# Shreyas911/MITgcm

Measured on AMD Instinct MI355X. Metric: model-days/wallclock-sec, higher is better.
Workload: dtype f64; 1 GPU; BASELINE config 2, verification/global_ocean.90x40x15 as verified: 90x40x15 global lat-lon ocean, 1 tile of 90x40 (OL=3) on 1 GPU, restarted from the committed pickup at nIter0=36000; r* coordinate with non-linear free surface (UPDATE_CG2D every step), JMD95P, GM/Redi gkw91, CD scheme, biharmonic + harmonic viscosity, quasi-hydrostatic + NH metric + 3-D Coriolis, implicit vertical diffusion, IVDC,; tiles_per_gpu=1, parallelism=replicas1, cg2d=single-GPU kernel

## Files before the change

mitgcm_amd/csrc/common.h:

```cpp
#pragma once
#include <hip/hip_runtime.h>
#include <stdint.h>
#include <stdlib.h>

namespace mgcm {

struct Dims {
  int sNx, sNy, OLx, OLy, Nr, nSx, nSy, nTiles;
  int t0, nT;
  int nx, ny;
  long n2, n3;
  long N2all, N3all;
};

#define MG_F2D_LIST(X) X(dxF) X(dyF) X(dxG) X(dyG) X(dxC) X(dyC) X(dxV) X(dyU) X(rA) X(rAw) X(rAs) X(recip_dxF) \
    X(recip_dyF) X(recip_dxC) X(recip_dyC) X(recip_dxV) X(recip_dyU) X(recip_rA) X(recip_rAw) X(recip_rAs) \
    X(fCori) X(Bo_surf) X(recip_Bo) X(tanPhiAtU) X(tanPhiAtV) X(maskInC) X(SST) X(lambdaThetaClimRelax) X(aW2d) \
    X(aS2d) X(aC2d) X(pW) X(pS) X(pC) X(etaN) X(fu) X(fv) X(etaH) X(surfaceForcingT) X(surfaceForcingS) \
    X(cg2d_b) X(cg2d_x) X(Qnet) X(EmPmR) X(SSS) X(lambdaSaltClimRelax) X(etaNm1) X(fCoriCos) X(recip_Rcol) \
    X(rSurfW) X(rSurfS) X(rLowW) X(rLowS) X(Ro_surf) X(R_low) X(rStarFacC) X(rStarFacW) X(rStarFacS) \
    X(rStarExpC) X(rStarExpW) X(rStarExpS) X(rStarDhCDt) X(rStarDhWDt) X(rStarDhSDt) X(PmEpR) X(dEtaHdt) \
    X(maskInW) X(maskInS) X(fCoriG) X(recip_rAz) X(recip_dxG) X(recip_dyG) X(etaHnm1) X(cg2d_r) X(cg2d_s) X(cg2d_q) \
    X(cg2d_min) X(cg2d_y) X(cg2d_v) X(EmPmRnext)
#define MG_F3D_LIST(X) X(hFacC) X(hFacW) X(hFacS) X(recip_hFacC) X(recip_hFacW) X(recip_hFacS) X(maskC) X(maskW) \
    X(maskS) X(uVel) X(vVel) X(wVel) X(theta) X(salt) X(gU) X(gV) X(guNm1) X(gvNm1) X(rhoInSitu) X(IVDConvCount) \
    X(gtNm1) X(thetaNext) X(gTscr) X(cpScr) X(phiHydC) X(saltNext) X(gsNm1) X(advScr1) X(advScr2) X(gAdv) \
    X(sigmaR) X(Kwx) X(Kwy) X(Kwz) X(Kux) X(Kvy) X(uVelD) X(vVelD) X(uNM1) X(vNM1) X(cdU) X(cdV) X(h0FacC) \
    X(h0FacW) X(h0FacS) X(totPhiHyd) X(alphaRho) X(del2u) X(del2v) X(dWtC) X(dWtU) X(dWtV) X(Kuz) X(Kvz) \
    X(GM_PsiX) X(GM_PsiY) X(gtNm2) X(gsNm2)
#define MG_ENUM2(n) F2_##n,
#define MG_ENUM3(n) F3_##n,
enum F2Id { MG_F2D_LIST(MG_ENUM2) F2_COUNT };
enum F3Id { MG_F3D_LIST(MG_ENUM3) F3_COUNT };
#undef MG_ENUM2
#undef MG_ENUM3

struct Params {
  double deltaTMom, deltaTFreeSurf, deltaTClock, abEps, rhoConst, gBaro;
  double viscAhD, viscAhZ, viscA4D, viscA4Z, viscAr, sideDragFactor;
  double freeSurfFac, implicSurfPress, implicDiv2DFlow, rkSign;
  double afFacMom, vfFacMom, pfFacMom, cfFacMom, foFacMom, mtFacMom;
  double cg2dNorm, cg2dTolerance_sq;
  int momAdvection, momViscosity, momForcing, useCoriolis, no_slip_sides, no_slip_bottom;
  int selectCoriScheme, momForcingOutAB, momDissip_In_AB, implicitViscosity;
  int cg2dMaxIters, cg2dUseMinResSol, cg2dNormaliseRHS, nIter0;
  int cg2dUseFMA;
  int useSRCGSolver;
  int cg2dRefOrder;
  double gravity, gravitySign, rhoNil, tAlpha, sBeta, ivdc_kappa, diffKhT, diffKrT, deltaTtracer;
  double recip_rSphere;
  int exactConserv, tempStepping, tempAdvection, tempForcing, implicitDiffusion, tempAdvScheme;
  int metricSphere;
  double diffKhS, diffKrS;
  int saltStepping, saltAdvection, saltForcing, saltAdvScheme, multiDimAdvection, momStepping;
  int multiDimCompressible;
  int eosType;
  int allowFreezing, useRealFreshWaterFlux, useCDscheme, useGMRedi, periodicExternalForcing, nForcRec;
  double HeatCapacity_Cp, convertFW2Salt, temp_EvPrRn, salt_EvPrRn, rCD, epsAB_CD;
  double externForcingPeriod, externForcingCycle;
  double GM_background_K, GM_isopycK, GM_skewflx, GM_maxSlope, GM_Kmin_horiz, GM_Small_Number, GM_slopeSqCutoff;
  int GM_AdvForm, GM_ExtraDiag;
  int nonlinFreeSurf, select_rStar, quasiHydrostatic, useNHMTerms, select3dCoriScheme, selectP_inEOS_Zc;
  int storePhiHyd4Phys;
  double hFacInf;
  int vectorInvariantMomentum, selectVortScheme, selectKEscheme, upwindShear, cubeCorners;
  int staggerTimeStep, tracForcingOutAB;
  double alph_AB, beta_AB;
  int useAB3;
};

struct Fields {
  const double *drF, *drC, *recip_drF, *recip_drC, *rF, *rC, *tRef, *sRef;
  const double *dxF, *dyF, *dxG, *dyG, *dxC, *dyC, *dxV, *dyU, *rA, *rAw, *rAs;
  const double *recip_dxF, *recip_dyF, *recip_dxC, *recip_dyC, *recip_dxV, *recip_dyU;
  const double *recip_rA, *recip_rAw, *recip_rAs, *fCori, *Bo_surf, *recip_Bo;
  const double *tanPhiAtU, *tanPhiAtV, *maskInC, *lambdaThetaClimRelax;
  double *SST;
  double *hFacC, *hFacW, *hFacS, *recip_hFacC, *recip_hFacW, *recip_hFacS;
  const double *maskC, *maskW, *maskS;
  double *aW2d, *aS2d, *aC2d, *pW, *pS, *pC;
  double *uVel, *vVel, *wVel, *theta, *salt, *etaN;
  double *gU, *gV, *guNm1, *gvNm1;
  double *fu, *fv;
  double *etaH, *surfaceForcingT, *rhoInSitu, *IVDConvCount, *gtNm1;
  double *thetaNext, *gTscr, *cpScr;
  double *phiHydC;
  double *saltNext, *gsNm1, *surfaceForcingS;
  double *gtNm2, *gsNm2;
  double *advScr1, *advScr2, *gAdv;
  const double *pRef4EOS;
  const double *forcRec;
  double *Qnet, *EmPmR, *SSS, *lambdaSaltClimRelax, *etaNm1;
  double *sigmaR, *Kwx, *Kwy, *Kwz, *Kux, *Kvy;
  double *Kuz, *Kvz, *GM_PsiX, *GM_PsiY;
  double *uVelD, *vVelD, *uNM1, *vNM1, *cdU, *cdV;
  const double *h0FacC, *h0FacW, *h0FacS;
  const double *fCoriCos, *recip_Rcol, *rSurfW, *rSurfS, *rLowW, *rLowS, *Ro_surf, *R_low;
  const double *phiRefC;
  double *totPhiHyd, *alphaRho, *del2u, *del2v;
  double *rStarFacC, *rStarFacW, *rStarFacS, *rStarExpC, *rStarExpW, *rStarExpS;
  double *rStarDhCDt, *rStarDhWDt, *rStarDhSDt, *PmEpR, *dEtaHdt;
  double *etaHnm1;
  const double *maskInW, *maskInS;
  double *dWtC, *dWtU, *dWtV;
  const double *fCoriG, *recip_rAz, *recip_dxG, *recip_dyG;
  const int *tileFace, *tileEdge;
  double *cg2d_b, *cg2d_x;
  double *cg2d_r, *cg2d_s, *cg2d_q;
  double *cg2d_min;
  double *cg2d_y, *cg2d_v;
  double *EmPmRnext;
  double *a2, *a3;
};
typedef __attribute__((address_space(1))) double mg_gdouble;
#define AR2(x, q) ((mg_gdouble *)f.a2)[(long)F2_##x * d.N2all + (q)]
#define AR3(x, q) ((mg_gdouble *)f.a3)[(long)F3_##x * d.N3all + (q)]

#define MG_I2(d, i, j, t) \
  ((long)((i) + (d).OLx - 1) + (long)((j) + (d).OLy - 1) * (d).nx + (long)(t) * (d).n2)
#define MG_I3(d, i, j, k, t)                                                                \
  ((long)((i) + (d).OLx - 1) + (long)((j) + (d).OLy - 1) * (d).nx + (long)((k) - 1) * (d).n2 + \
   (long)(t) * (d).n3)

#define MG_NXCD 8
__device__ __forceinline__ int mg_xcd_block() {
  const int b = (int)blockIdx.x, n = (int)gridDim.x;
  const int x = b % MG_NXCD, per = n / MG_NXCD, rem = n % MG_NXCD;
  return x * per + (x < rem ? x : rem) + b / MG_NXCD;
}
#define MG_PLANE(i0, ni, j0, nj, zvar)                                                  \
  int i, j, zvar;                                                                       \
  {                                                                                     \
    const int np_ = (ni) * (nj), nb_ = (np_ + (int)blockDim.x - 1) / (int)blockDim.x; \
    const int lb_ = mg_xcd_block();                                                     \
    const int q_ = (lb_ % nb_) * (int)blockDim.x + (int)threadIdx.x;                    \
    zvar = lb_ / nb_;                                                                   \
    if (q_ >= np_) return;                                                              \
    i = (i0) + q_ % (ni);                                                               \
    j = (j0) + q_ / (ni);                                                               \
  }
#define MG_PLANE_LB(i0, ni, j0, nj, zvar, LB)                                           \
  int i, j, zvar;                                                                       \
  {                                                                                     \
    const int np_ = (ni) * (nj), nb_ = (np_ + (int)blockDim.x - 1) / (int)blockDim.x; \
    const int lb_ = (LB);                                                               \
    const int q_ = (lb_ % nb_) * (int)blockDim.x + (int)threadIdx.x;                    \
    zvar = lb_ / nb_;                                                                   \
    if (q_ >= np_) return;                                                              \
    i = (i0) + q_ % (ni);                                                               \
    j = (j0) + q_ / (ni);                                                               \
  }
#define MG_PLANE_THREADS 256

__host__ __device__ inline int mg_col_kp(int Nr) { int kp = 1; while (kp < Nr) kp <<= 1; return kp; }
#define MG_COLS(i0, ni, j0, nj, Nr)                                                    \
  const int KP_ = mg_col_kp(Nr), NC_ = 256 / KP_;                                        \
  const int cc = (int)threadIdx.x % NC_, kk = (int)threadIdx.x / NC_;                   \
  const long col_ = (long)mg_xcd_block() * NC_ + cc;                                    \
  const long npl_ = (long)(ni) * (nj);                                                  \
  const bool valid = col_ < npl_ * d.nT;                                                \
  const int t = d.t0 + (int)(valid ? col_ / npl_ : 0);                                  \
  const int i = (i0) + (int)((valid ? col_ % npl_ : 0) % (ni));                         \
  const int j = (j0) + (int)((valid ? col_ % npl_ : 0) / (ni));
inline unsigned mg_col_blocks(int ni, int nj, int nT, int Nr) {
  const int nc = 256 / mg_col_kp(Nr);
  return (unsigned)(((long)ni * nj * nT + nc - 1) / nc);
}
#define MG_COLF(i0, ni, j0, nj, NCv)                                                   \
  const int NC_ = (NCv), KW_ = 256 / NC_;                                              \
  const int cc = (int)threadIdx.x % NC_, kk = (int)threadIdx.x / NC_;                  \
  const long col_ = (long)mg_xcd_block() * NC_ + cc;                                   \
  const long npl_ = (long)(ni) * (nj);                                                 \
  const bool valid = col_ < npl_ * d.nT;                                               \
  const int t = d.t0 + (int)(valid ? col_ / npl_ : 0);                                 \
  const int i = (i0) + (int)((valid ? col_ % npl_ : 0) % (ni));                        \
  const int j = (j0) + (int)((valid ? col_ % npl_ : 0) / (ni));
#define MG_COLF_LB(i0, ni, j0, nj, NCv, LB)                                            \
  const int NC_ = (NCv), KW_ = 256 / NC_;                                              \
  const int cc = (int)threadIdx.x % NC_, kk = (int)threadIdx.x / NC_;                  \
  const long col_ = (long)(LB) * NC_ + cc;                                             \
  const long npl_ = (long)(ni) * (nj);                                                 \
  const bool valid = col_ < npl_ * d.nT;                                               \
  const int t = d.t0 + (int)(valid ? col_ / npl_ : 0);                                 \
  const int i = (i0) + (int)((valid ? col_ % npl_ : 0) % (ni));                        \
  const int j = (j0) + (int)((valid ? col_ % npl_ : 0) / (ni));
#define MG_COLF_K(kvar) for (int kvar = kk + 1; kvar <= d.Nr; kvar += KW_)
inline int mg_colf_nc(long ncols, int Nr, int nArr) {
  (void)ncols; (void)Nr; (void)nArr;
  return 16;
}
inline size_t mg_colf_lds(int Nr, int nc, int nArr) { return (size_t)nArr * Nr * nc * sizeof(double); }
#define MG_ALLOW_LDS(kern)                                                                              \
  do {                                                                                                  \
    static const bool set_ = (hipFuncSetAttribute((const void *)(kern),                                 \
                                                  hipFuncAttributeMaxDynamicSharedMemorySize, 160 * 1024) == hipSuccess); \
    (void)set_;                                                                                         \
  } while (0)
inline unsigned mg_colf_blocks(long ncols, int nc) { return (unsigned)((ncols + nc - 1) / nc); }
enum { MG_FUSE_SFP = 1, MG_FUSE_ETA = 2, MG_FUSE_PHI = 4, MG_FUSE_END = 8, MG_FUSE_PHYS = 16, MG_FUSE_ETAA = 32,
       MG_FUSE_TREX = 64, MG_FUSE_DT = 128, MG_FUSE_ETAX = 256, MG_FUSE_TCG = 512, MG_FUSE_OPE = 1024,
       MG_FUSE_RING = 2048, MG_FUSE_RINGP = 4096, MG_FUSE_ENDS = 8192, MG_FUSE_PIPE = 16384 };
inline bool mg_fuse_on(int bit) {
  const int mask = getenv("MGCM_STEP_FUSE") ? atoi(getenv("MGCM_STEP_FUSE"))
                                            : MG_FUSE_SFP | MG_FUSE_PHI | MG_FUSE_END | MG_FUSE_DT | MG_FUSE_ETAX |
                                                MG_FUSE_OPE | MG_FUSE_RING | MG_FUSE_RINGP | MG_FUSE_ENDS | MG_FUSE_PIPE;
  return (mask & bit) != 0;
}
inline bool mg_hfuse(int bit, long nx, long ny, long nT, long Nr) {
  return mg_fuse_on(bit) && nx * ny * nT * Nr <= (1L << 21);
}
inline unsigned mg_plane_blocks(int ni, int nj, int nz) {
  return (unsigned)(((ni) * (nj) + MG_PLANE_THREADS - 1) / MG_PLANE_THREADS * (nz));
}

__device__ __forceinline__ void sfp_rhs_column(const Dims &d, const Params &p, const Fields &f, long q, bool inner,
                                               const double *sE, const double *sW, const double *sN, const double *sS,
                                               int NC_, int cc) {
  if (p.useCDscheme) f.etaNm1[q] = f.etaN[q];
  f.cg2d_x[q] = f.Bo_surf[q] * f.etaN[q];
  double b = 0.0;
  if (inner) {
    if (p.useRealFreshWaterFlux) {
      const double tmpFac = p.freeSurfFac * (1.0 / p.rhoConst) * p.implicDiv2DFlow;
      b = tmpFac * f.rA[q] * f.EmPmR[q] / p.deltaTMom * f.maskInC[q];
    }
    for (int k2 = d.Nr; k2 >= 1; k2--) {
      const int s2 = (k2 - 1) * NC_ + cc;
      b = b + sE[s2] - sW[s2];
      b = b + sN[s2] - sS[s2];
    }
    b = b - p.freeSurfFac * f.rA[q] / p.deltaTMom / p.deltaTFreeSurf * (p.exactConserv ? f.etaH[q] : f.etaN[q]);
  }
  f.cg2d_b[q] = b;
}

struct TracerArgs {
  const double *tr;
  double *trNext;
  double *gNm1;
  double *scr;
  double *cp;
  const double *sfc;
  double diffKh, diffKr, dT;
  int advection, multiDim, useAB, forcing;
  int limiter;
  int scheme;
  double *gNm2;
};

#define MG_XMAX 8
struct XFields {
  double *p[MG_XMAX];
  int nz[MG_XMAX];
  int n;
};

__device__ __forceinline__ void exchange_multi_body(const Dims &d, const XFields &x, const long *__restrict__ map,
                                                    int nHalo, int *ctr, int hb, int k, int fi) {
  const int h = hb * (int)blockDim.x + (int)threadIdx.x;
  if (ctr && h == 0 && k == 0 && fi == 0) { ctr[0] += 1; ctr[1] += 1; }
  if (h >= nHalo || fi >= x.n || k >= x.nz[fi]) return;
  const long dst = map[2 * h], src = map[2 * h + 1];
  const long dt = dst / d.n2, dl = dst % d.n2, st = src / d.n2, sl = src % d.n2;
  const long lvl = (long)d.n2 * x.nz[fi];
  double *a = x.p[fi];
  a[dt * lvl + (long)k * d.n2 + dl] = a[st * lvl + (long)k * d.n2 + sl];
}

__device__ __forceinline__ void exchange_mixed_body(const Dims &d, double *u, double *v, int nzUV,
                                                    const long *__restrict__ uvMap, int nU, int nV, const XFields &x,
                                                    const long *__restrict__ map, int nHalo, int *ctr, int hb, int k,
                                                    int z) {
  const int h = hb * (int)blockDim.x + (int)threadIdx.x;
  if (ctr && h == 0 && k == 0 && z == 0) { ctr[0] += 1; ctr[1] += 1; }
  if (z == 0) {
    if (h >= nU + nV || k >= nzUV) return;
    const long dst = uvMap[2 * h], code = uvMap[2 * h + 1];
    const long N2 = d.n2 * d.nTiles, s = (code > 0 ? code : -code) - 1;
    const long n3 = d.n2 * nzUV, lvl = (long)k * d.n2;
    auto at = [&](long g) -> long { return (g / d.n2) * n3 + lvl + g % d.n2; };
    const double val = s < N2 ? u[at(s)] : v[at(s - N2)];
    (h < nU ? u : v)[at(dst)] = code > 0 ? val : -val;
    return;
  }
  const int fi = z - 1;
  if (h >= nHalo || fi >= x.n || k >= x.nz[fi]) return;
  const long dst = map[2 * h], src = map[2 * h + 1];
  const long dt = dst / d.n2, dl = dst % d.n2, st = src / d.n2, sl = src % d.n2;
  const long lvl = (long)d.n2 * x.nz[fi];
  double *a = x.p[fi];
  a[dt * lvl + (long)k * d.n2 + dl] = a[st * lvl + (long)k * d.n2 + sl];
}

struct MwgTables {
  const int *ownG;
  const int *ownC;
  const unsigned *ownNb;
  const unsigned *ownExp;
  const int *ringG;
  const unsigned *ringNb;
  const int *impC;
  const int *impG;
  const int *nImp;
  int G, IMAX, SZ;
  int nExp;
  int pinned;
  int sys;
  int partsPerTile;
  int exclusive;
  unsigned *ctr;
  unsigned *epoch;
  unsigned long long *part;
  unsigned long long *xs;
  size_t hsBytes;
  int ref;
  int nTiles;
  const int *ownN;
  unsigned long long *refc;
};

struct MonSpec {
  const double *arr, *hfac, *mask, *area, *dr;
  int nz, arr3d, hf3d;
};
constexpr int MON_NF = 6, MON_NV = 6;
struct MonSpecs {
  MonSpec s[MON_NF];
  double mean[MON_NF];
};

struct SolveRecord {
  double firstResidual, lastResidual, minResidualSq, rhsMax, sumRHS;
  int numIters, nIterMin;
};

}
```

mitgcm_amd/csrc/kernels_dyn.hip:

```cpp
#include <cstdlib>

#include "common.h"
#include "phys.h"
#include <cstring>
#include <cstdio>
#include <type_traits>

namespace mgcm {

__device__ __forceinline__ double hfacz(const Dims &d, const Fields &f, int i, int j, int k, int t) {
  if (i < 2 - d.OLx || j < 2 - d.OLy) return 0.0;
  double h = fmin(f.hFacW[MG_I3(d, i, j, k, t)], f.hFacW[MG_I3(d, i, j - 1, k, t)]);
  h = fmin(f.hFacS[MG_I3(d, i, j, k, t)], h);
  h = fmin(f.hFacS[MG_I3(d, i - 1, j, k, t)], h);
  return h;
}

__device__ __forceinline__ double h0facz(const Dims &d, const Params &p, const Fields &f, int i, int j, int k, int t) {
  if (!(p.momViscosity && p.no_slip_sides && p.nonlinFreeSurf > 0)) return hfacz(d, f, i, j, k, t);
  if (i < 2 - d.OLx || j < 2 - d.OLy) return 0.0;
  return fmin(fmin(f.h0FacW[MG_I3(d, i, j, k, t)], f.h0FacW[MG_I3(d, i, j - 1, k, t)]),
              fmin(f.h0FacS[MG_I3(d, i, j, k, t)], f.h0FacS[MG_I3(d, i - 1, j, k, t)]));
}

__device__ __forceinline__ void del2uv_body(const Dims &d, const Params &p, const Fields &f, int lb) {
  MG_PLANE_LB(1 - d.OLx, d.nx, 1 - d.OLy, d.ny, z, lb)
  const int t = d.t0 + z / d.Nr, k = z % d.Nr + 1;
  const long q3 = MG_I3(d, i, j, k, t);
  if (i < 2 - d.OLx || i > d.sNx + d.OLx - 1 || j < 2 - d.OLy || j > d.sNy + d.OLy - 1) {
    f.del2u[q3] = 0.0;
    f.del2v[q3] = 0.0;
    return;
  }
  const double drF = f.drF[k - 1];
#define U(ii, jj) f.uVel[MG_I3(d, ii, jj, k, t)]
#define V(ii, jj) f.vVel[MG_I3(d, ii, jj, k, t)]
#define G2(a, ii, jj) f.a[MG_I2(d, ii, jj, t)]
#define G3(a, ii, jj) f.a[MG_I3(d, ii, jj, k, t)]
  {
    auto fz = [&](int ii) { return drF * G3(hFacC, ii, j) * G2(dyF, ii, j) * G2(recip_dxF, ii, j) * (U(ii + 1, j) - U(ii, j)) * 1.0; };
    auto fm = [&](int jj) {
      return drF * hfacz(d, f, i, jj, k, t) * G2(dxV, i, jj) * G2(recip_dyU, i, jj) * (U(i, jj) - U(i, jj - 1));
    };
    double v4 = f.recip_drF[k - 1] * G3(recip_hFacW, i, j) * G2(recip_rAw, i, j) *
                (fz(i) - fz(i - 1) + fm(j + 1) - fm(j)) * G3(maskW, i, j);
    if (p.no_slip_sides) {
      const double hS = G3(h0FacW, i, j) - h0facz(d, p, f, i, j, k, t);
      const double hN = G3(h0FacW, i, j) - h0facz(d, p, f, i, j + 1, k, t);
      v4 = v4 - G3(recip_hFacW, i, j) * G2(recip_rAw, i, j) *
                    (hS * G2(dxV, i, j) * G2(recip_dyU, i, j) + hN * G2(dxV, i, j + 1) * G2(recip_dyU, i, j + 1)) * U(i, j) *
                    p.sideDragFactor * G3(maskW, i, j);
    }
    f.del2u[q3] = v4;
  }
  {
    auto fz = [&](int ii) {
      return drF * hfacz(d, f, ii, j, k, t) * G2(dyU, ii, j) * G2(recip_dxV, ii, j) * (V(ii, j) - V(ii - 1, j)) * 1.0;
    };
    auto fm = [&](int jj) { return drF * G3(hFacC, i, jj) * G2(dxF, i, jj) * G2(recip_dyF, i, jj) * (V(i, jj + 1) - V(i, jj)); };
    double v4 = f.recip_drF[k - 1] * G3(recip_hFacS, i, j) * G2(recip_rAs, i, j) *
                (fz(i + 1) - fz(i) + fm(j) - fm(j - 1)) * G3(maskS, i, j);
    if (p.no_slip_sides) {
      const double hW = G3(h0FacS, i, j) - h0facz(d, p, f, i, j, k, t);
      const double hE = G3(h0FacS, i, j) - h0facz(d, p, f, i + 1, j, k, t);
      v4 = v4 - G3(recip_hFacS, i, j) * G2(recip_rAs, i, j) *
                    (hW * G2(dyU, i, j) * G2(recip_dxV, i, j) + hE * G2(dyU, i + 1, j) * G2(recip_dxV, i + 1, j)) * V(i, j) *
                    p.sideDragFactor * G3(maskS, i, j);
    }
    f.del2v[q3] = v4;
  }
#undef U
#undef V
#undef G2
#undef G3
}
__global__ void __launch_bounds__(256) k_del2uv(Dims d, Params p, Fields f) { del2uv_body(d, p, f, mg_xcd_block()); }

template <bool PHYS = false>
__device__ __forceinline__ void phi_hyd_body(const Dims &d, const Params &p, const Fields &f, int nc, int lb,
                                             const int *iterPtr = nullptr) {
  extern __shared__ __attribute__((aligned(16))) double lds[];
  MG_COLF_LB(PHYS ? 1 - d.OLx : -1, PHYS ? d.nx : d.sNx + 3, PHYS ? 1 - d.OLy : -1, PHYS ? d.ny : d.sNy + 3, nc, lb)
  const int Nr = d.Nr, NS = Nr * NC_;
  double *sM = lds, *sP = lds + NS, *sPh = lds + 2 * NS, *sC = lds + 3 * NS, *sU = lds + 4 * NS, *sV = lds + 5 * NS;
  const bool qh = p.quasiHydrostatic && (p.select3dCoriScheme >= 1 || p.useNHMTerms);
  const bool rstar = p.nonlinFreeSurf > 0 && p.select_rStar > 0;
  const bool inPhi = !PHYS || (i >= -1 && i <= d.sNx + 1 && j >= -1 && j <= d.sNy + 1);
  const bool ring = inPhi && i >= 0 && j >= 0;
  const double recip_rhoConst = 1.0 / p.rhoConst;
  const long q2 = MG_I2(d, i, j, t);
  if (valid) MG_COLF_K(k) {
    const int me = (k - 1) * NC_ + cc;
    double dRlocM = 0.5 * f.drC[k - 1];
    if (k == 1) dRlocM = f.rF[0] - f.rC[0];
    const double dRlocP = (k == Nr) ? (f.rC[k - 1] - f.rF[k]) : 0.5 * f.drC[k];
    const long q3 = MG_I3(d, i, j, k, t);
    double a;
    if constexpr (PHYS) a = oceanic_phys_point(d, p, f, iterPtr, i, j, k, t);
    else a = f.rhoInSitu[q3];
    if (qh) {
      const double scalingFactor = p.rhoConst * p.gravitySign * (1.0 / p.gravity);
      const double u0 = f.uVel[q3], u1 = f.uVel[MG_I3(d, i + 1, j, k, t)];
      const double v0 = f.vVel[q3], v1 = f.vVel[MG_I3(d, i, j + 1, k, t)];
      double gW = 0.0;
      if (p.select3dCoriScheme >= 1) gW = f.fCoriCos[q2] * (1.0 * 0.5 * (u0 + u1) - 0.0 * 0.5 * (v0 + v1));
      if (p.useNHMTerms) gW = gW + ((u0 * u0 + u1 * u1) + (v0 * v0 + v1 * v1)) * 0.5 * p.recip_rSphere;
      a = a + scalingFactor * gW;
    }
    if (rstar && inPhi) f.alphaRho[q3] = a;
    sM[me] = dRlocM * p.gravity * a * recip_rhoConst;
    sP[me] = dRlocP * p.gravity * a * recip_rhoConst;
    if (rstar) {
      const double drF = f.drF[k - 1];
      sC[me] = f.rStarDhCDt[q2] * drF * f.h0FacC[q3] * f.rA[q2];
      if (ring) {
        sU[me] = f.rStarDhWDt[q2] * drF * f.h0FacW[q3] * f.rAw[q2];
        sV[me] = f.rStarDhSDt[q2] * drF * f.h0FacS[q3] * f.rAs[q2];
      }
    }
  }
  __syncthreads();
  if (valid && kk == 0) {
    double phF = 0.0;
    for (int k2 = 1; k2 <= Nr; k2++) {
      const int s2 = (k2 - 1) * NC_ + cc;
      const double phC = phF + sM[s2];
      phF = phC + sP[s2];
      sPh[s2] = phC;
    }
    if (rstar) {
      auto d0 = [&](long r) { return f.rStarDhCDt[r] * (f.Ro_surf[r] - f.R_low[r]) * f.rA[r]; };
      double c = d0(q2);
      double u = ring ? 0.5 * (d0(q2 - 1) + c) : 0.0, v = ring ? 0.5 * (d0(q2 - d.nx) + c) : 0.0;
      for (int k2 = 1; k2 <= Nr; k2++) {
        const int s2 = (k2 - 1) * NC_ + cc;
        const double cc2 = sC[s2];
        sC[s2] = c;
        c = c - cc2;
        if (ring) {
          const double uu = sU[s2], vv = sV[s2];
          sU[s2] = u;
          sV[s2] = v;
          u = u - uu;
          v = v - vv;
        }
      }
    }
  }
  __syncthreads();
  if (valid) MG_COLF_K(k) {
    const int me = (k - 1) * NC_ + cc;
    const long q3 = MG_I3(d, i, j, k, t);
    if (rstar && inPhi) {
      f.dWtC[q3] = sC[me];
      if (ring) { f.dWtU[q3] = sU[me]; f.dWtV[q3] = sV[me]; }
    }
    if (ring) {
      const double phC = sPh[me];
      f.phiHydC[q3] = phC;
      if (p.storePhiHyd4Phys) {
        double tot;
        if (rstar && p.nonlinFreeSurf >= 4) {
          const double dPhiRef = (f.Ro_surf[q2] - f.rC[k - 1]) * p.gravity;
          tot = phC * f.rStarFacC[q2] + fmax(dPhiRef, 0.0) * (f.rStarFacC[q2] - 1.0) + 0.0;
        } else {
          tot = phC + f.Bo_surf[q2] * f.etaN[q2] + 0.0;
        }
        f.totPhiHyd[q3] = tot;
      }
    }
  }
}
__global__ void __launch_bounds__(256) k_phi_hyd(Dims d, Params p, Fields f, int nc) {
  phi_hyd_body(d, p, f, nc, mg_xcd_block());
}
constexpr int PHI_CH = 10;
template <bool RS, bool QH, int NRC = 0>
__device__ __forceinline__ void phi_flat_body(const Dims &d, const Params &p, const Fields &f, int lb) {
  constexpr int o = RS ? 1 : 0;
  const int W = d.sNx + 2 + o, H = d.sNy + 2 + o;
  const long col = (long)lb * 256 + threadIdx.x, npl = (long)W * H;
  if (col >= npl * d.nT) return;
  const int t = d.t0 + (int)(col / npl), r = (int)(col % npl);
  const int i = r % W - o, j = r / W - o;
  const bool ring = i >= 0 && j >= 0;
  const int Nr = NRC > 0 ? NRC : d.Nr;
  constexpr int CH = (RS || QH) ? 5 : PHI_CH;
  const double recip_rhoConst = 1.0 / p.rhoConst;
  const double scalingFactor = p.rhoConst * p.gravitySign * (1.0 / p.gravity);
  const long q2 = MG_I2(d, i, j, t);
  double c = 0.0, u = 0.0, v = 0.0, dCdt = 0.0, dWdt = 0.0, dSdt = 0.0, rA = 0.0, rAw = 0.0, rAs = 0.0;
  if (RS) {
    auto d0 = [&](long rr) { return f.rStarDhCDt[rr] * (f.Ro_surf[rr] - f.R_low[rr]) * f.rA[rr]; };
    c = d0(q2);
    u = ring ? 0.5 * (d0(q2 - 1) + c) : 0.0;
    v = ring ? 0.5 * (d0(q2 - d.nx) + c) : 0.0;
    dCdt = f.rStarDhCDt[q2]; rA = f.rA[q2];
    if (ring) { dWdt = f.rStarDhWDt[q2]; dSdt = f.rStarDhSDt[q2]; rAw = f.rAw[q2]; rAs = f.rAs[q2]; }
  }
  const bool tot = p.storePhiHyd4Phys && ring;
  const bool totR = RS && p.nonlinFreeSurf >= 4;
  const double bEta = tot && !totR ? f.Bo_surf[q2] * f.etaN[q2] : 0.0;
  const double fac = tot && totR ? f.rStarFacC[q2] : 0.0, roS = tot && totR ? f.Ro_surf[q2] : 0.0;
  const double fCos = QH ? f.fCoriCos[q2] : 0.0;
  double phF = 0.0;
  auto chunk = [&](const int k0) {
    double a[CH], u0[CH], u1[CH], v0[CH], v1[CH], hC[CH], hW[CH], hS[CH], dM[CH], dP[CH];
#pragma unroll
    for (int cc = 0; cc < CH; cc++) {
      const int k = k0 + cc <= Nr ? k0 + cc : Nr;
      const long q3 = MG_I3(d, i, j, k, t);
      a[cc] = f.rhoInSitu[q3];
      if constexpr (NRC > 0) {
        dM[cc] = (k == 1) ? f.rF[0] - f.rC[0] : 0.5 * f.drC[k - 1];
        dP[cc] = (k == Nr) ? (f.rC[k - 1] - f.rF[k]) : 0.5 * f.drC[k];
      }
      if (QH) {
        u0[cc] = f.uVel[q3]; u1[cc] = f.uVel[MG_I3(d, i + 1, j, k, t)];
        v0[cc] = f.vVel[q3]; v1[cc] = f.vVel[MG_I3(d, i, j + 1, k, t)];
      }
      if (RS) {
        hC[cc] = f.h0FacC[q3];
        if (ring) { hW[cc] = f.h0FacW[q3]; hS[cc] = f.h0FacS[q3]; }
      }
    }
#pragma unroll
    for (int cc = 0; cc < CH; cc++) {
      const int k = k0 + cc;
      if (k > Nr) continue;
      const long q3 = MG_I3(d, i, j, k, t);
      double dRlocM, dRlocP;
      if constexpr (NRC > 0) {
        dRlocM = dM[cc];
        dRlocP = dP[cc];
      } else {
        dRlocM = 0.5 * f.drC[k - 1];
        if (k == 1) dRlocM = f.rF[0] - f.rC[0];
        dRlocP = (k == Nr) ? (f.rC[k - 1] - f.rF[k]) : 0.5 * f.drC[k];
      }
      double al = a[cc];
      if (QH) {
        double gW = 0.0;
        if (p.select3dCoriScheme >= 1) gW = fCos * (1.0 * 0.5 * (u0[cc] + u1[cc]) - 0.0 * 0.5 * (v0[cc] + v1[cc]));
        if (p.useNHMTerms)
          gW = gW + ((u0[cc] * u0[cc] + u1[cc] * u1[cc]) + (v0[cc] * v0[cc] + v1[cc] * v1[cc])) * 0.5 * p.recip_rSphere;
        al = al + scalingFactor * gW;
      }
      if (RS) f.alphaRho[q3] = al;
      const double sM = dRlocM * p.gravity * al * recip_rhoConst;
      const double sP = dRlocP * p.gravity * al * recip_rhoConst;
      const double phC = phF + sM;
      phF = phC + sP;
      if (RS) {
        const double drF = f.drF[k - 1];
        const double cc2 = dCdt * drF * hC[cc] * rA;
        f.dWtC[q3] = c;
        c = c - cc2;
        if (ring) {
          const double uu = dWdt * drF * hW[cc] * rAw, vv = dSdt * drF * hS[cc] * rAs;
          f.dWtU[q3] = u;
          f.dWtV[q3] = v;
          u = u - uu;
          v = v - vv;
        }
      }
      if (ring) {
        f.phiHydC[q3] = phC;
        if (tot) {
          if (totR) {
            const double dPhiRef = (roS - f.rC[k - 1]) * p.gravity;
            f.totPhiHyd[q3] = phC * fac + fmax(dPhiRef, 0.0) * (fac - 1.0) + 0.0;
          } else {
            f.totPhiHyd[q3] = phC + bEta + 0.0;
          }
        }
      }
    }
  };
  if constexpr (NRC > 0) {
#pragma unroll
    for (int k0 = 1; k0 <= NRC; k0 += CH) chunk(k0);
  } else {
    for (int k0 = 1; k0 <= Nr; k0 += CH) chunk(k0);
  }
}
template <bool RS, bool QH, int NRC = 0>
__global__ void __launch_bounds__(256) k_phi_flat(Dims d, Params p, Fields f) {
  phi_flat_body<RS, QH, NRC>(d, p, f, mg_xcd_block());
}

inline bool phi_flat_on(const Params &p) {
  const char *e = getenv("MGCM_PHI_FLAT");
  const int v = e ? atoi(e) : 1;
  if (v == 0 || v == 2) return v == 2;
  const bool rs = p.nonlinFreeSurf > 0 && p.select_rStar > 0;
  const bool qh = p.quasiHydrostatic && (p.select3dCoriScheme >= 1 || p.useNHMTerms);
  return !rs && !qh;
}
inline int phi_flat_blocks(const Dims &d, const Params &p) {
  const int o = (p.nonlinFreeSurf > 0 && p.select_rStar > 0) ? 1 : 0;
  return (int)(((long)(d.sNx + 2 + o) * (d.sNy + 2 + o) * d.nT + 255) / 256);
}
__global__ void __launch_bounds__(256) k_phys_phi(Dims d, Params p, Fields f, int nc, const int *iterPtr) {
  phi_hyd_body<true>(d, p, f, nc, mg_xcd_block(), iterPtr);
}
__global__ void __launch_bounds__(256) k_phi_del2(Dims d, Params p, Fields f, int nc, int nbPhi) {
  const int lb = mg_xcd_block();
  if (lb < nbPhi) phi_hyd_body(d, p, f, nc, lb);
  else del2uv_body(d, p, f, lb - nbPhi);
}


template <class A> __device__ __forceinline__ int vi_tile_face(const A &, const Fields &f, int t) { return f.tileFace[t]; }
template <class A> __device__ __forceinline__ int vi_tile_edge(const A &, const Fields &f, int t) { return f.tileEdge[t]; }
template <class A> __device__ __forceinline__ double vi_rdrC(const A &, const Fields &f, int kk) { return f.recip_drC[kk - 1]; }
template <class A> __device__ __forceinline__ double vi_rdrF(const A &, const Fields &f, int kk) { return f.recip_drF[kk - 1]; }
template <class A> __device__ __forceinline__ double vi_drF(const A &, const Fields &f, int kk) { return f.drF[kk - 1]; }
// ... 2028 lines not shown
```

mitgcm_amd/csrc/kernels_rstar.hip:

```cpp
#include "common.h"
#include "phys.h"
#include "ucg2d.h"

namespace mgcm {

__device__ __forceinline__ double eta_exch(const Dims &d, const Fields &f, const long *srcOf, long q, int fromX) {
  const long sq = srcOf[q];
  if (sq >= 0) return f.cg2d_b[sq];
  const long l = q % d.n2;
  const int i = (int)(l % d.nx) - d.OLx + 1, j = (int)(l / d.nx) - d.OLy + 1;
  if (i >= 1 && i <= d.sNx && j >= 1 && j <= d.sNy) return f.cg2d_b[q];
  return fromX ? f.recip_Bo[q] * f.cg2d_x[q] : f.etaN[q];
}

template <bool FUSE>
__device__ __forceinline__ void calc_r_star_body(const Dims &d, const Params &p, const Fields &f,
                                                 const long *__restrict__ srcOf, int lb, int fromX, int empNext = 0) {
  const long q = (long)lb * blockDim.x + threadIdx.x;
  if (q >= d.n2 * d.nTiles) return;
  const int t = (int)(q / d.n2);
  if (t < d.t0 || t >= d.t0 + d.nT) return;
  if constexpr (FUSE) {
    if (p.nonlinFreeSurf > 0 && p.useRealFreshWaterFlux) f.PmEpR[q] = -f.EmPmR[q];
    if (empNext) f.EmPmR[q] = f.EmPmRnext[q];
    const double x = eta_exch(d, f, srcOf, q, fromX);
    f.etaHnm1[q] = f.etaH[q];
    f.etaN[q] = x;
    f.etaH[q] = x;
  }
  const long sq = srcOf[q], r = sq >= 0 ? sq : q;
  const long l = r % d.n2;
  const int i = (int)(l % d.nx) - d.OLx + 1, j = (int)(l / d.nx) - d.OLy + 1;
  auto eta = [&](long qq) { return FUSE ? eta_exch(d, f, srcOf, qq, fromX) : f.etaH[qq]; };
  const double oc = f.rStarFacC[q], ow = f.rStarFacW[q], os = f.rStarFacS[q];
  double fc = oc, fw = ow, fs = os;
  if (i >= 0 && i <= d.sNx + 1 && j >= 0 && j <= d.sNy + 1)
    fc = (f.maskInC[r] != 0.0) ? (eta(r) + f.Ro_surf[r] - f.R_low[r]) * f.recip_Rcol[r] : 1.0;
  const long rv = p.cubeCorners ? q : r;
  const long lv = rv % d.n2;
  const int iv = (int)(lv % d.nx) - d.OLx + 1, jv = (int)(lv / d.nx) - d.OLy + 1;
  if (iv >= 1 && iv <= d.sNx + 1 && jv >= 1 && jv <= d.sNy) {
    if (f.maskInW[rv] != 0.0) {
      const double tmp = f.rSurfW[rv] - f.rLowW[rv];
      fw = (0.5 * (eta(rv - 1) * f.rA[rv - 1] + eta(rv) * f.rA[rv]) * f.recip_rAw[rv] + tmp) / tmp;
    } else {
      fw = 1.0;
    }
  }
  if (iv >= 1 && iv <= d.sNx && jv >= 1 && jv <= d.sNy + 1) {
    if (f.maskInS[rv] != 0.0) {
      const double tmp = f.rSurfS[rv] - f.rLowS[rv];
      fs = (0.5 * (eta(rv - d.nx) * f.rA[rv - d.nx] + eta(rv) * f.rA[rv]) * f.recip_rAs[rv] + tmp) / tmp;
    } else {
      fs = 1.0;
    }
  }
  f.rStarFacC[q] = fc;
  f.rStarFacW[q] = fw;
  f.rStarFacS[q] = fs;
  f.rStarDhCDt[q] = (fc - oc) / p.deltaTFreeSurf;
  f.rStarDhWDt[q] = (fw - ow) / p.deltaTFreeSurf;
  f.rStarDhSDt[q] = (fs - os) / p.deltaTFreeSurf;
  f.rStarExpC[q] = fc / oc;
  f.rStarExpW[q] = fw / ow;
  f.rStarExpS[q] = fs / os;
}
template <bool FUSE>
__global__ void __launch_bounds__(256) k_calc_r_star(Dims d, Params p, Fields f, const long *__restrict__ srcOf, int fromX) {
  calc_r_star_body<FUSE>(d, p, f, srcOf, (int)blockIdx.x, fromX);
}
template <bool FUSE>
__global__ void __launch_bounds__(256) k_rstar_exch(Dims d, Params p, Fields f, const long *__restrict__ srcOf, int nbR,
                                                    XFields x, const long *__restrict__ map, int nHalo, int *ctr, int nbX,
                                                    int nzMax, int fromX, int empNext) {
  const int b = (int)blockIdx.x;
  if (b < nbR) { calc_r_star_body<FUSE>(d, p, f, srcOf, b, fromX, empNext); return; }
  const int r = b - nbR;
  exchange_multi_body(d, x, map, nHalo, ctr, r % nbX, (r / nbX) % nzMax, r / (nbX * nzMax));
}

template <bool FUSE>
__global__ void __launch_bounds__(256) k_rstar_exmix(Dims d, Params p, Fields f, const long *__restrict__ srcOf, int nbR,
                                                     int fromX, double *u, double *v, int nzUV,
                                                     const long *__restrict__ uvMap, int nU, int nV, XFields x,
                                                     const long *__restrict__ map, int nHalo, int nbH, int nzMax) {
  const int b = (int)blockIdx.x;
  if (b < nbR) { calc_r_star_body<FUSE>(d, p, f, srcOf, b, fromX); return; }
  const int r = b - nbR;
  exchange_mixed_body(d, u, v, nzUV, uvMap, nU, nV, x, map, nHalo, nullptr, r % nbH, (r / nbH) % nzMax, r / (nbH * nzMax));
}

template <bool SFP, bool PH>
__global__ void __launch_bounds__(256) k_update_r_star_cg2d_a(Dims d, Params p, Fields f, int nc, int opIn,
                                                              const long *__restrict__ srcOf, int nbPc,
                                                              const int *iterPtr, int nbPh) {
  extern __shared__ __attribute__((aligned(16))) double lds[];
  int lb = mg_xcd_block();
  if constexpr (PH) {
    if (lb < nbPh) { phys_hoist_body(d, p, f, iterPtr, srcOf, lb); return; }
    lb -= nbPh;
  }
  if (lb < nbPc) { ucg2d_p_point(d, p, f, srcOf, lb); return; }
  lb -= nbPc;
  MG_COLF_LB(1 - d.OLx, d.nx, 1 - d.OLy, d.ny, nc, lb)
  const int NS = d.Nr * NC_;
  double *sW = lds, *sS = lds + NS;
  double *fE = lds + 2 * NS, *fW = lds + 3 * NS, *fN = lds + 4 * NS, *fS = lds + 5 * NS;
  const long q = MG_I2(d, i, j, t);
  const bool op = opIn && p.nonlinFreeSurf > 2 && i >= 1 && i <= d.sNx + 1 && j >= 1 && j <= d.sNy + 1;
  const bool inner = i >= 1 && i <= d.sNx && j >= 1 && j <= d.sNy;
  if (valid) {
    const double fc = f.rStarFacC[q], fw = f.rStarFacW[q], fs = f.rStarFacS[q];
    double fwE = 0.0, fsN = 0.0;
    if (SFP && inner) { fwE = f.rStarFacW[MG_I2(d, i + 1, j, t)]; fsN = f.rStarFacS[MG_I2(d, i, j + 1, t)]; }
    MG_COLF_K(k) {
      const long q3 = MG_I3(d, i, j, k, t);
      const double hC = f.h0FacC[q3] * fc, hW = f.h0FacW[q3] * fw, hS = f.h0FacS[q3] * fs;
      f.hFacC[q3] = hC;
      f.hFacW[q3] = hW;
      f.hFacS[q3] = hS;
      if (f.maskC[q3] != 0.0) f.recip_hFacC[q3] = 1.0 / hC;
      if (f.maskW[q3] != 0.0) f.recip_hFacW[q3] = 1.0 / hW;
      if (f.maskS[q3] != 0.0) f.recip_hFacS[q3] = 1.0 / hS;
      const int me = (k - 1) * NC_ + cc;
      if (op) {
        double faceArea = f.dyG[q] * f.drF[k - 1] * hW;
        sW[me] = faceArea * f.recip_dxC[q];
        faceArea = f.dxG[q] * f.drF[k - 1] * hS;
        sS[me] = faceArea * f.recip_dyC[q];
      }
      if (SFP) {
        if (p.useCDscheme) {
          f.uNM1[q3] = f.uVel[q3];
          f.vNM1[q3] = f.vVel[q3];
        }
        if (inner) {
          const double drF = f.drF[k - 1];
          const long qE = MG_I3(d, i + 1, j, k, t), qN = MG_I3(d, i, j + 1, k, t);
          fE[me] = f.dyG[MG_I2(d, i + 1, j, t)] * drF * (f.h0FacW[qE] * fwE) * f.gU[qE] / p.deltaTMom;
          fW[me] = f.dyG[q] * drF * hW * f.gU[q3] / p.deltaTMom;
          fN[me] = f.dxG[MG_I2(d, i, j + 1, t)] * drF * (f.h0FacS[qN] * fsN) * f.gV[qN] / p.deltaTMom;
          fS[me] = f.dxG[q] * drF * hS * f.gV[q3] / p.deltaTMom;
        }
      }
    }
  }
  __syncthreads();
  if (!valid || kk != 0) return;
  if (opIn && p.nonlinFreeSurf > 2) {
    double aW = 0.0, aS = 0.0;
    if (op) {
      for (int k = 1; k <= d.Nr; k++) {
        const int me = (k - 1) * NC_ + cc;
        aW = aW + sW[me];
        aS = aS + sS[me];
      }
      aW = aW * p.cg2dNorm * p.implicSurfPress * p.implicDiv2DFlow;
      aS = aS * p.cg2dNorm * p.implicSurfPress * p.implicDiv2DFlow;
    }
    f.aW2d[q] = aW;
    f.aS2d[q] = aS;
  }
  if (SFP) sfp_rhs_column(d, p, f, q, inner, fE, fW, fN, fS, NC_, cc);
}

__global__ void __launch_bounds__(256) k_update_cg2d_p(Dims d, Params p, Fields f, const long *__restrict__ srcOf) {
  ucg2d_p_point(d, p, f, srcOf, (int)blockIdx.x);
}

hipError_t launch_calc_r_star(const Dims &d, const Params &p, const Fields &f, const long *srcOf, hipStream_t s,
                              bool fuseEtaH, int fromX) {
  const long n = d.n2 * d.nTiles;
  hipLaunchKernelGGL(fuseEtaH ? k_calc_r_star<true> : k_calc_r_star<false>, dim3((unsigned)((n + 255) / 256)), dim3(256),
                     0, s, d, p, f, srcOf, fromX);
  return hipGetLastError();
}

hipError_t launch_rstar_exch(const Dims &d, const Params &p, const Fields &f, const long *srcOf, bool fuseEtaH,
                             const XFields &x, const long *map, int nHalo, int *ctr, hipStream_t s, int fromX, int empNext) {
  const long n = d.n2 * d.nTiles;
  const int nbR = (int)((n + 255) / 256);
  int nzMax = 1;
  for (int q = 0; q < x.n; q++) nzMax = x.nz[q] > nzMax ? x.nz[q] : nzMax;
  const int nbX = ((nHalo > 0 ? nHalo : 1) + 255) / 256;
  const unsigned nb = (unsigned)(nbR + nbX * nzMax * (x.n > 0 ? x.n : 1));
  hipLaunchKernelGGL(fuseEtaH ? k_rstar_exch<true> : k_rstar_exch<false>, dim3(nb), dim3(256), 0, s, d, p, f, srcOf, nbR, x,
                     map, nHalo, ctr, nbX, nzMax, fromX, fuseEtaH ? empNext : 0);
  return hipGetLastError();
}

hipError_t launch_rstar_exmix(const Dims &d, const Params &p, const Fields &f, const long *srcOf, bool fuseEtaH, int fromX,
                              double *u, double *v, int nzUV, const long *uvMap, int nU, int nV, const XFields &x,
                              const long *map, int nHalo, hipStream_t s) {
  const long n = d.n2 * d.nTiles;
  const int nbR = (int)((n + 255) / 256);
  int nzMax = nzUV;
  for (int q = 0; q < x.n; q++) nzMax = x.nz[q] > nzMax ? x.nz[q] : nzMax;
  const int nh = (nU + nV) > nHalo ? nU + nV : nHalo;
  const int nbH = ((nh > 0 ? nh : 1) + 255) / 256;
  const unsigned nb = (unsigned)(nbR + nbH * nzMax * (1 + x.n));
  hipLaunchKernelGGL(fuseEtaH ? k_rstar_exmix<true> : k_rstar_exmix<false>, dim3(nb), dim3(256), 0, s, d, p, f, srcOf, nbR,
                     fromX, u, v, nzUV, uvMap, nU, nV, x, map, nHalo, nbH, nzMax);
  return hipGetLastError();
}

hipError_t launch_update_r_star_cg2d(const Dims &d, const Params &p, const Fields &f, const long *srcOf, hipStream_t s,
                                     bool sfp, bool opEarly, bool pcHere, const int *iterPtr) {
  const long n = d.n2 * d.nTiles;
  const unsigned nb = (unsigned)((n + 255) / 256);
  const long ncol = (long)d.nx * d.ny * d.nT;
  const int nArr = sfp ? 6 : 2;
  const int nc = mg_colf_nc(ncol, d.Nr, nArr);
  auto kPlain = k_update_r_star_cg2d_a<false, false>, kSfp = k_update_r_star_cg2d_a<true, false>,
       kSfpPhys = k_update_r_star_cg2d_a<true, true>;
  MG_ALLOW_LDS(kPlain);
  MG_ALLOW_LDS(kSfp);
  const int nbPc = (opEarly && pcHere && p.nonlinFreeSurf > 2) ? (int)nb : 0;
  if (iterPtr) {
    if (!sfp) return hipErrorInvalidValue;
    MG_ALLOW_LDS(kSfpPhys);
    const int nbPh = phys_hoist_blocks(d);
    hipLaunchKernelGGL(kSfpPhys, dim3(mg_colf_blocks(ncol, nc) + (unsigned)(nbPc + nbPh)), dim3(256),
                       mg_colf_lds(d.Nr, nc, nArr), s, d, p, f, nc, opEarly ? 0 : 1, srcOf, nbPc, iterPtr, nbPh);
  } else
    hipLaunchKernelGGL(sfp ? kSfp : kPlain, dim3(mg_colf_blocks(ncol, nc) + (unsigned)nbPc), dim3(256),
                       mg_colf_lds(d.Nr, nc, nArr), s, d, p, f, nc, opEarly ? 0 : 1, srcOf, nbPc, (const int *)nullptr, 0);
  if (p.nonlinFreeSurf > 2 && !opEarly) hipLaunchKernelGGL(k_update_cg2d_p, dim3(nb), dim3(256), 0, s, d, p, f, srcOf);
  return hipGetLastError();
}

}
```

mitgcm_amd/csrc/kernels_step.hip:

```cpp
#include "kernels_dyn.hip"
#include "kernels_thermo.hip"
#include "ucg2d.h"

namespace mgcm {

template <bool GM>
__global__ void __launch_bounds__(256) k_dt_front(Dims d, Params p, Fields f, TracerArgs aT, TracerArgs aS,
                                                  const int *iterPtr, int nc, int nbPhi, int nbDel, int nbTr) {
  int lb = mg_xcd_block();
  if (lb < nbPhi) { phi_hyd_body(d, p, f, nc, lb); return; }
  lb -= nbPhi;
  if (lb < nbDel) { del2uv_body(d, p, f, lb); return; }
  lb -= nbDel;
  if (lb < nbTr) tracer_rhs_body_br<GM>(d, p, f, aT, iterPtr, lb);
  else tracer_rhs_body_br<GM>(d, p, f, aS, iterPtr, lb - nbTr);
}

__global__ void __launch_bounds__(256) k_dt_back(Dims d, Params p, Fields f, TracerArgs aT, TracerArgs aS,
                                                 const int *iterPtr, int nc, int nbMom, int nbImp) {
  int lb = mg_xcd_block();
  if (lb < nbMom) {
    if (lb & 1) mom_step_point<false, 2>(d, p, f, iterPtr, lb >> 1);
    else mom_step_point<false, 1>(d, p, f, iterPtr, lb >> 1);
    return;
  }
  lb -= nbMom;
  if (lb < nbImp) tracer_impl_body<false>(d, p, f, aT, nc, lb);
  else tracer_impl_body<false>(d, p, f, aS, nc, lb - nbImp);
}

static int dt_long_first() {
  const char *e = getenv("MGCM_DT_LAYOUT");
  return !(e && atoi(e) == 4);
}
__global__ void __launch_bounds__(256) k_dt_l1(Dims d, Params p, Fields f, int nc, int nbGm, int nbPhi, int nbOp, int lf) {
  int lb = mg_xcd_block();
  if (lf) {
    if (lb < nbPhi) { phi_hyd_body(d, p, f, nc, lb); return; }
    lb -= nbPhi;
    if (lb < nbOp) { ucg2d_op_point(d, p, f, lb); return; }
    lb -= nbOp;
    if (lb < nbGm) { gm_tensor_body(d, p, f, lb); return; }
    del2uv_body(d, p, f, lb - nbGm);
    return;
  }
  if (lb < nbOp) { ucg2d_op_point(d, p, f, lb); return; }
  lb -= nbOp;
  if (lb < nbGm) { gm_tensor_body(d, p, f, lb); return; }
  lb -= nbGm;
  if (lb < nbPhi) { phi_hyd_body(d, p, f, nc, lb); return; }
  del2uv_body(d, p, f, lb - nbPhi);
}
static void phi_frame(const Dims &d, const Params &p, int &nc, int &nArr, int &nb);
template <bool RS, bool QH>
__global__ void __launch_bounds__(256) k_dt_l1f(Dims d, Params p, Fields f, int nbGm, int nbPhi, int nbOp) {
  int lb = mg_xcd_block();
  if (lb < nbOp) { ucg2d_op_point(d, p, f, lb); return; }
  lb -= nbOp;
  if (lb < nbGm) { gm_tensor_body(d, p, f, lb); return; }
  lb -= nbGm;
  if (lb < nbPhi) { phi_flat_body<RS, QH>(d, p, f, lb); return; }
  del2uv_body(d, p, f, lb - nbPhi);
}
static void launch_l1(const Dims &d, const Params &p, const Fields &f, int nbDel, hipStream_t s, int nbOp = 0,
                      bool gm = true) {
  const int nbGm = gm ? (int)mg_plane_blocks(d.nx - 2, d.ny - 2, d.nT * d.Nr) : 0;
  if (phi_flat_on(p)) {
    const bool rs = p.nonlinFreeSurf > 0 && p.select_rStar > 0;
    const bool qh = p.quasiHydrostatic && (p.select3dCoriScheme >= 1 || p.useNHMTerms);
    auto kern = rs ? (qh ? k_dt_l1f<true, true> : k_dt_l1f<true, false>)
                   : (qh ? k_dt_l1f<false, true> : k_dt_l1f<false, false>);
    const int nbPhi = phi_flat_blocks(d, p);
    hipLaunchKernelGGL(kern, dim3((unsigned)(nbOp + nbGm + nbPhi + nbDel)), dim3(256), 0, s, d, p, f, nbGm, nbPhi,
                       nbOp);
    return;
  }
  int nc, nArr, nbPhi;
  phi_frame(d, p, nc, nArr, nbPhi);
  MG_ALLOW_LDS(k_dt_l1);
  hipLaunchKernelGGL(k_dt_l1, dim3((unsigned)(nbOp + nbGm + nbPhi + nbDel)), dim3(256), mg_colf_lds(d.Nr, nc, nArr), s, d, p,
                     f, nc, nbGm, nbPhi, nbOp, dt_long_first());
}
template <bool GM, bool FF4>
__global__ void __launch_bounds__(256) k_dt_l2(Dims d, Params p, Fields f, TracerArgs aT, TracerArgs aS,
                                               const int *iterPtr, int nbMom, int nbTr, const long *__restrict__ srcOf,
                                               int nbPc, int nbOp, int lf) {
  int lb = mg_xcd_block();
  if (lf) {
    if (lb < 2 * nbTr) {
      if (lb < nbTr) tracer_rhs_body_br<GM>(d, p, f, aT, iterPtr, lb);
      else tracer_rhs_body_br<GM>(d, p, f, aS, iterPtr, lb - nbTr);
      return;
    }
    lb -= 2 * nbTr;
  }
  if (lb < nbPc) { ucg2d_p_point(d, p, f, srcOf, lb); return; }
  lb -= nbPc;
  if (lb < nbOp) { ucg2d_op_point(d, p, f, lb); return; }
  lb -= nbOp;
  if (lb < nbMom) {
    if constexpr (FF4) mom_ff4_body(d, p, f, iterPtr, lb);
    else if (lb & 1) mom_step_point<false, 2>(d, p, f, iterPtr, lb >> 1);
    else mom_step_point<false, 1>(d, p, f, iterPtr, lb >> 1);
    return;
  }
  lb -= nbMom;
  if (lb < nbTr) tracer_rhs_body_br<GM>(d, p, f, aT, iterPtr, lb);
  else tracer_rhs_body_br<GM>(d, p, f, aS, iterPtr, lb - nbTr);
}
__global__ void __launch_bounds__(256) k_dt_l3(Dims d, Params p, Fields f, TracerArgs aT, TracerArgs aS,
                                               const int *iterPtr, int nc, int nbCd, int nbImp, const long *__restrict__ srcOf,
                                               int nbPc, int lf) {
  int lb = mg_xcd_block();
  if (lf) {
    if (lb < 2 * nbImp) {
      if (lb < nbImp) tracer_impl_body<false>(d, p, f, aT, nc, lb);
      else tracer_impl_body<false>(d, p, f, aS, nc, lb - nbImp);
      return;
    }
    lb -= 2 * nbImp;
    if (lb < nbPc) { ucg2d_p_point(d, p, f, srcOf, lb); return; }
    cd_scheme_body(d, p, f, iterPtr, lb - nbPc);
    return;
  }
  if (lb < nbPc) { ucg2d_p_point(d, p, f, srcOf, lb); return; }
  lb -= nbPc;
  if (lb < nbCd) { cd_scheme_body(d, p, f, iterPtr, lb); return; }
  lb -= nbCd;
  if (lb < nbImp) tracer_impl_body<false>(d, p, f, aT, nc, lb);
  else tracer_impl_body<false>(d, p, f, aS, nc, lb - nbImp);
}
bool dyn_thermo_takes_gm(const Params &p) {
  const char *e = getenv("MGCM_DT_LAYOUT");
  return p.useGMRedi && p.useCDscheme && !(p.implicitViscosity) && !(e && atoi(e) == 2);
}

bool dyn_thermo_fusable(const Dims &d, const Params &p, const TracerArgs &aT, const TracerArgs &aS) {
  return mg_hfuse(MG_FUSE_DT, d.nx, d.ny, d.nT, d.Nr) && p.momStepping && p.tempStepping && p.saltStepping &&
         p.useGMRedi && p.implicitDiffusion && !aT.multiDim && !aS.multiDim && !p.vectorInvariantMomentum &&
         aT.scr != aS.scr && aT.scheme == 2 && aS.scheme == 2 && !p.useAB3;
}

static void phi_frame(const Dims &d, const Params &p, int &nc, int &nArr, int &nb) {
  const long ncol = (long)(d.sNx + 3) * (d.sNy + 3) * d.nT;
  nArr = (p.nonlinFreeSurf > 0 && p.select_rStar > 0) ? 6 : 3;
  nc = mg_colf_nc(ncol, d.Nr, nArr);
  nb = (int)mg_colf_blocks(ncol, nc);
}

bool gm_phi_fusable(const Dims &d, const Params &p) {
  return mg_hfuse(MG_FUSE_DT, d.nx, d.ny, d.nT, d.Nr) && p.useGMRedi && p.momStepping;
}
hipError_t launch_gm_phi(const Dims &d, const Params &p, const Fields &f, hipStream_t s, bool op) {
  launch_l1(d, p, f, phi_del2_fused(d, p) ? (int)mg_plane_blocks(d.nx, d.ny, d.nT * d.Nr) : 0, s, op ? ucg2d_blocks(d) : 0);
  return hipGetLastError();
}

template <bool GM>
__global__ void __launch_bounds__(256) k_tr_rhs_pair(Dims d, Params p, Fields f, TracerArgs aT, TracerArgs aS,
                                                     const int *iterPtr, int nbTr) {
  const int lb = mg_xcd_block();
  if (lb < nbTr) tracer_rhs_body<GM>(d, p, f, aT, iterPtr, lb);
  else tracer_rhs_body<GM>(d, p, f, aS, iterPtr, lb - nbTr);
}
__global__ void __launch_bounds__(256) k_tr_impl_pair(Dims d, Params p, Fields f, TracerArgs aT, TracerArgs aS, int nc,
                                                      int nbImp) {
  const int lb = mg_xcd_block();
  if (lb < nbImp) tracer_impl_body<false>(d, p, f, aT, nc, lb);
  else tracer_impl_body<false>(d, p, f, aS, nc, lb - nbImp);
}
bool tracer_hpair_ok(const Dims &d, const Params &p, const TracerArgs &aT, const TracerArgs &aS) {
  return mg_hfuse(MG_FUSE_DT, d.nx, d.ny, d.nT, d.Nr) && p.tempStepping && p.saltStepping && p.implicitDiffusion &&
         !aT.multiDim && !aS.multiDim && aT.scr != aS.scr && !tracer_march_on(d);
}
hipError_t launch_tracer_hpair(const Dims &d, const Params &p, const Fields &f, const TracerArgs &aT, const TracerArgs &aS,
                               const int *iterPtr, hipStream_t s) {
  const int nbTr = (int)mg_plane_blocks(d.sNx, d.sNy, d.nT * d.Nr);
  if (p.useGMRedi) hipLaunchKernelGGL(k_tr_rhs_pair<true>, dim3((unsigned)(2 * nbTr)), dim3(256), 0, s, d, p, f, aT, aS,
                                      iterPtr, nbTr);
  else hipLaunchKernelGGL(k_tr_rhs_pair<false>, dim3((unsigned)(2 * nbTr)), dim3(256), 0, s, d, p, f, aT, aS, iterPtr, nbTr);
  const long ncol = (long)d.sNx * d.sNy * d.nT;
  const int nc = mg_colf_nc(ncol, d.Nr, 3);
  const int nbImp = (int)mg_colf_blocks(ncol, nc);
  MG_ALLOW_LDS(k_tr_impl_pair);
  hipLaunchKernelGGL(k_tr_impl_pair, dim3((unsigned)(2 * nbImp)), dim3(256), mg_colf_lds(d.Nr, nc, 3), s, d, p, f, aT, aS, nc,
                     nbImp);
  return hipGetLastError();
}

hipError_t launch_dyn_thermo(const Dims &d, const Params &p, const Fields &f, const TracerArgs &aT, const TracerArgs &aS,
                             const int *iterPtr, hipStream_t s, const long *srcOf, bool gmHere) {
  const dim3 blk(256);
  int ncPhi, nArrPhi, nbPhi;
  phi_frame(d, p, ncPhi, nArrPhi, nbPhi);
  const int nbDel = del2_needed(p) ? (int)mg_plane_blocks(d.nx, d.ny, d.nT * d.Nr) : 0;
  const int nbTr = (int)mg_plane_blocks(d.sNx, d.sNy, d.nT * d.Nr);
  if (dyn_thermo_takes_gm(p)) {
    const int nbU = srcOf ? ucg2d_blocks(d) : 0;
    const int nbOp1 = 0, nbPc2 = 0, nbOp2 = nbU, nbPc3 = nbU;
    launch_l1(d, p, f, nbDel, s, nbOp1, gmHere);
    const bool ff4 = mom_ff4_on(true);
    const int nbMom = ff4 ? mom_ff4_blocks(d) : 2 * (int)mg_plane_blocks(d.nx, d.ny, d.nT * d.Nr);
    auto l2 = ff4 ? k_dt_l2<true, true> : k_dt_l2<true, false>;
    hipLaunchKernelGGL(l2, dim3((unsigned)(nbPc2 + nbOp2 + nbMom + 2 * nbTr)), blk, 0, s, d, p, f, aT, aS, iterPtr, nbMom, nbTr,
                       srcOf, nbPc2, nbOp2, dt_long_first());
    const long ncolTr = (long)d.sNx * d.sNy * d.nT;
    const int ncTr = mg_colf_nc(ncolTr, d.Nr, 3);
    const int nbImp = (int)mg_colf_blocks(ncolTr, ncTr);
    const int nbCd = (int)mg_plane_blocks(d.nx - 2, d.ny - 2, d.nT * d.Nr);
    MG_ALLOW_LDS(k_dt_l3);
    hipLaunchKernelGGL(k_dt_l3, dim3((unsigned)(nbPc3 + nbCd + 2 * nbImp)), blk, mg_colf_lds(d.Nr, ncTr, 3), s, d, p, f, aT,
                       aS, iterPtr, ncTr, nbCd, nbImp, srcOf, nbPc3, dt_long_first());
    return hipGetLastError();
  }
  if (srcOf || !gmHere) return hipErrorInvalidValue;
  MG_ALLOW_LDS(k_dt_front<true>);
  hipLaunchKernelGGL(k_dt_front<true>, dim3((unsigned)(nbPhi + nbDel + 2 * nbTr)), blk,
                     mg_colf_lds(d.Nr, ncPhi, nArrPhi), s, d, p, f, aT, aS, iterPtr, ncPhi, nbPhi, nbDel, nbTr);
  const int nbMom = 2 * (int)mg_plane_blocks(d.nx, d.ny, d.nT * d.Nr);
  const long ncolTr = (long)d.sNx * d.sNy * d.nT;
  const int ncTr = mg_colf_nc(ncolTr, d.Nr, 3);
  const int nbImp = (int)mg_colf_blocks(ncolTr, ncTr);
  MG_ALLOW_LDS(k_dt_back);
  hipLaunchKernelGGL(k_dt_back, dim3((unsigned)(nbMom + 2 * nbImp)), blk, mg_colf_lds(d.Nr, ncTr, 3), s, d, p, f, aT, aS,
                     iterPtr, ncTr, nbMom, nbImp);
  const hipError_t e = hipGetLastError();
  if (e != hipSuccess) return e;
  return launch_mom_tail(d, p, f, iterPtr, s);
}

}
```

mitgcm_amd/csrc/model.hip:

```cpp
#include <hip/hip_runtime.h>

#include <cmath>
#include <cstdarg>
#include <cstdio>
#include <cstdlib>
#include <cstring>
#include <algorithm>
#include <map>
#include <utility>
#include <string>
#include <vector>

#include "../../include/mitgcm_amd.h"
#include "cg2d.h"

namespace mgcm {
static std::vector<std::pair<uintptr_t, uintptr_t>> g_hostReg;
void mg_host_ranges_set(const uintptr_t *lo, const uintptr_t *hi, size_t n) {
  g_hostReg.clear();
  for (size_t i = 0; i < n; i++) g_hostReg.push_back({lo[i], hi[i]});
  std::sort(g_hostReg.begin(), g_hostReg.end());
}
hipError_t mg_host_copy(void *dst, const void *src, size_t bytes, hipMemcpyKind kind, hipStream_t s) {
  if (g_hostReg.empty() || bytes == 0) return hipMemcpyAsync(dst, src, bytes, kind, s);
  const uintptr_t h = (uintptr_t)(kind == hipMemcpyHostToDevice ? src : dst), end = h + bytes;
  size_t off = 0;
  while (h + off < end) {
    const uintptr_t cur = h + off;
    uintptr_t cut = end;
    for (const auto &r : g_hostReg) {
      if (r.first > cur && r.first < cut) cut = r.first;
      if (r.second > cur && r.second < cut) cut = r.second;
    }
    const hipError_t e = hipMemcpyAsync((char *)dst + off, (const char *)src + off, cut - cur, kind, s);
    if (e != hipSuccess) return e;
    off += cut - cur;
  }
  return hipSuccess;
}
}

namespace mgcm {
hipError_t launch_mom_step(const Dims &, const Params &, const Fields &, const int *, hipStream_t, bool ring = true);
bool mom_ring_separable(const Dims &, const Params &);
hipError_t launch_mom_ring(const Dims &, const Params &, const Fields &, const int *, hipStream_t);
hipError_t launch_phi_hyd(const Dims &, const Params &, const Fields &, hipStream_t);
bool phys_phi_fusable(const Dims &, const Params &);
hipError_t launch_phys_phi(const Dims &, const Params &, const Fields &, const int *, hipStream_t);
hipError_t launch_sfp_rhs(const Dims &, const Params &, const Fields &, hipStream_t);
hipError_t launch_exchange(const Dims &, double *, const long *, int, int, hipStream_t);
hipError_t launch_cgd(const Dims &, const Params &, const Fields &, int, double, double *, hipStream_t);
hipError_t launch_cgd_record(SolveRecord *, const int *, double, double, double, double, int, double, int, hipStream_t);
hipError_t launch_field_pack(double *, const long *, long, double *, int, hipStream_t);
hipError_t launch_correction(const Dims &, const Params &, const Fields &, hipStream_t);
hipError_t launch_bump_counter(int *, int, hipStream_t);
hipError_t launch_exchange_multi(const Dims &, const XFields &, const long *, int, int *, hipStream_t);
hipError_t launch_exchange_uv(const Dims &, double *, double *, const long *, int, int, int, hipStream_t);
hipError_t launch_exchange_mixed(const Dims &, double *, double *, int, const long *, int, int, const XFields &,
                                 const long *, int, int *, hipStream_t);
hipError_t launch_exchange_uv_pairs(const Dims &, double *const *, double *const *, int, const long *, int, int,
                                   hipStream_t);
hipError_t launch_exch_eta(const Dims &, const Params &, const Fields &, const long *, bool, int, hipStream_t,
                           int fromX = 0);
hipError_t launch_corr_cont(const Dims &, const Params &, const Fields &, int, hipStream_t, const long *etaSrc = nullptr,
                            bool gmNext = false);
hipError_t launch_calc_r_star(const Dims &, const Params &, const Fields &, const long *, hipStream_t, bool fuseEtaH = false,
                              int fromX = 0);
hipError_t launch_rstar_exmix(const Dims &, const Params &, const Fields &, const long *, bool, int, double *, double *, int,
                              const long *, int, int, const XFields &, const long *, int, hipStream_t);
hipError_t launch_rstar_exch(const Dims &, const Params &, const Fields &, const long *, bool, const XFields &, const long *,
                             int, int *, hipStream_t, int fromX = 0, int empNext = 0);
hipError_t launch_update_r_star_cg2d(const Dims &, const Params &, const Fields &, const long *, hipStream_t, bool sfp = false,
                                     bool opEarly = false, bool pcHere = false, const int *iterPtr = nullptr);
hipError_t launch_halo_pack(const Dims &, const XFields &, const long *, long, double *, int, hipStream_t);
hipError_t launch_oceanic_phys(const Dims &, const Params &, const Fields &, const int *, hipStream_t, bool gm = true,
                               bool *ringDone = nullptr);
hipError_t launch_tracer_step(const Dims &, const Params &, const Fields &, const TracerArgs &, const int *, hipStream_t,
                              bool impl = true);
bool dyn_thermo_fusable(const Dims &, const Params &, const TracerArgs &, const TracerArgs &);
hipError_t launch_dyn_thermo(const Dims &, const Params &, const Fields &, const TracerArgs &, const TracerArgs &, const int *,
                             hipStream_t, const long *srcOf = nullptr, bool gmHere = true);
bool dyn_thermo_takes_gm(const Params &);
hipError_t launch_gm_tensor(const Dims &, const Params &, const Fields &, hipStream_t);
hipError_t launch_hfac_snapshot(const Dims &, const Fields &, double *, hipStream_t);
Fields hfac_snapshot_fields(const Dims &, const Fields &, double *);
bool gm_phi_fusable(const Dims &, const Params &);
hipError_t launch_gm_phi(const Dims &, const Params &, const Fields &, hipStream_t, bool op = false);
bool tracer_hpair_ok(const Dims &, const Params &, const TracerArgs &, const TracerArgs &);
hipError_t launch_tracer_hpair(const Dims &, const Params &, const Fields &, const TracerArgs &, const TracerArgs &,
                               const int *, hipStream_t);
hipError_t launch_mon_stats(const Dims &, const MonSpecs &, int, double *, int, hipStream_t);
}

using namespace mgcm;

static thread_local std::string g_err;
static int set_err(const char *fmt, ...) {
  char buf[1024];
  va_list ap;
  va_start(ap, fmt);
  vsnprintf(buf, sizeof buf, fmt, ap);
  va_end(ap);
  g_err = buf;
  return -1;
}
#define HIPCHK(x)                                                                              \
  do {                                                                                         \
    hipError_t e_ = (x);                                                                       \
    if (e_ != hipSuccess) return set_err("%s:%d %s: %s", __FILE__, __LINE__, #x, hipGetErrorString(e_)); \
  } while (0)

enum FieldKind { F1D, F2D, F3D, FREC };
#define MG_MAXREC 12
struct FieldDesc {
  const char *name;
  FieldKind kind;
  size_t off;
};

#define FD(n, k) {#n, k, offsetof(Fields, n)}
static const FieldDesc FIELDS[] = {
    FD(drF, F1D), FD(drC, F1D), FD(recip_drF, F1D), FD(recip_drC, F1D), FD(rF, F1D), FD(rC, F1D), FD(tRef, F1D), FD(sRef, F1D), FD(pRef4EOS, F1D), FD(phiRefC, F1D),
#define FD2(n) FD(n, F2D),
#define FD3(n) FD(n, F3D),
    MG_F2D_LIST(FD2)
    MG_F3D_LIST(FD3)
#undef FD2
#undef FD3
    FD(forcRec, FREC),
};
#undef FD

struct PDesc {
  const char *name;
  size_t off;
  bool isint;
};
#define PD(n) {#n, offsetof(Params, n), false}
#define PI_(n) {#n, offsetof(Params, n), true}
static const PDesc PARAMS[] = {
    PD(deltaTMom), PD(deltaTFreeSurf), PD(deltaTClock), PD(abEps), PD(alph_AB), PD(beta_AB), PI_(useAB3), PD(rhoConst), PD(gBaro), PD(viscAhD), PD(viscAhZ),
    PD(viscA4D), PD(viscA4Z), PD(viscAr), PD(sideDragFactor), PD(freeSurfFac), PD(implicSurfPress),
    PD(implicDiv2DFlow), PD(rkSign), PD(afFacMom), PD(vfFacMom), PD(pfFacMom), PD(cfFacMom), PD(foFacMom),
    PD(mtFacMom), PD(cg2dNorm), PD(cg2dTolerance_sq),
    PI_(momAdvection), PI_(momViscosity), PI_(momForcing), PI_(useCoriolis), PI_(no_slip_sides),
    PI_(no_slip_bottom), PI_(selectCoriScheme), PI_(momForcingOutAB), PI_(momDissip_In_AB),
    PI_(implicitViscosity), PI_(cg2dMaxIters), PI_(cg2dUseMinResSol), PI_(cg2dNormaliseRHS), PI_(nIter0), PI_(cg2dUseFMA), PI_(useSRCGSolver), PI_(cg2dRefOrder),
    PD(gravity), PD(gravitySign), PD(rhoNil), PD(tAlpha), PD(sBeta), PD(ivdc_kappa), PD(diffKhT), PD(diffKrT),
    PD(deltaTtracer), PI_(exactConserv), PI_(tempStepping), PI_(tempAdvection), PI_(tempForcing),
    PI_(implicitDiffusion), PI_(tempAdvScheme), PI_(saltStepping), PI_(saltAdvection), PI_(saltForcing),
    PI_(saltAdvScheme), PD(diffKhS), PD(diffKrS), PI_(multiDimAdvection), PI_(multiDimCompressible), PI_(momStepping),
    PI_(eosType), PI_(allowFreezing), PI_(useRealFreshWaterFlux), PI_(useCDscheme), PI_(useGMRedi),
    PI_(periodicExternalForcing), PI_(nForcRec), PD(HeatCapacity_Cp), PD(convertFW2Salt), PD(temp_EvPrRn),
    PD(salt_EvPrRn), PD(rCD), PD(epsAB_CD), PD(externForcingPeriod), PD(externForcingCycle), PD(GM_background_K),
    PD(GM_isopycK), PD(GM_skewflx), PD(GM_maxSlope), PD(GM_Kmin_horiz), PD(GM_Small_Number), PD(GM_slopeSqCutoff),
    PI_(GM_AdvForm), PI_(GM_ExtraDiag),
    PI_(nonlinFreeSurf), PI_(select_rStar), PI_(quasiHydrostatic), PI_(useNHMTerms), PI_(select3dCoriScheme),
    PI_(selectP_inEOS_Zc), PI_(storePhiHyd4Phys), PD(hFacInf),
    PI_(vectorInvariantMomentum), PI_(selectVortScheme), PI_(selectKEscheme), PI_(upwindShear),
    PI_(staggerTimeStep), PI_(tracForcingOutAB),
};
#undef PD
#undef PI_

enum Kern { K_MOM, K_RHS, K_CG2D, K_EXCH, K_ETA, K_CORR, K_CONT, K_PHYS, K_TEMP, K_RSTAR, K_PHI, K_N };
static const char *KNAMES[K_N] = {"mom_step",   "sfp_rhs",    "cg2d",         "exchange",  "eta_update",
                                  "correction", "continuity", "oceanic_phys", "temp_step", "r_star", "phi_hyd"};

struct mgcm_model {
  Dims d{};
  Params p{};
  Fields f{};
  int device = 0;
  hipStream_t stream = nullptr;
  hipStream_t ownStream = nullptr;
  hipStream_t stream2 = nullptr;
  hipEvent_t evFork = nullptr, evJoin = nullptr;
  hipEvent_t evSnap = nullptr;
  double *snapH = nullptr;
  hipStream_t stream3 = nullptr;
  hipEvent_t evEta0 = nullptr, evEta1 = nullptr;
  hipEvent_t evHand = nullptr;
  bool overlap = true;
  std::vector<void *> allocs;
  std::map<std::string, double> extra;
  long *d_halo = nullptr;
  long *d_srcOf = nullptr;
  int nHalo = 0;
  long *d_haloAll = nullptr;
  int nHaloAll = 0;
  std::vector<long> h_halo;
  enum class Cg2dSolver { Bxy = 3, Mwg = 4, BlockRef = 5, MwgRef = 6 };
  Cg2dSolver solver = Cg2dSolver::Bxy;
  bool useMwg() const { return solver == Cg2dSolver::Mwg || solver == Cg2dSolver::MwgRef; }
  int nPts = 0;
  unsigned *d_nbr = nullptr;
  int *d_gofs = nullptr;
  unsigned *d_nbx = nullptr;
  int *d_blkx = nullptr;
  int nBlkX = 0;
  int bxyVar = -1;
  int *d_slot2 = nullptr;
  std::vector<int> h_dropG;
  int *d_dropG = nullptr;
  int nDropBlk = 0;
  bool noCompact = false;
  int *h_guard = nullptr;
  int *d_guard = nullptr;
  bool latlonTopology = true;
  MwgTables mwg{};
  std::vector<void *> mwgAllocs;
  void *mwgShared = nullptr;
  void *mwgBlock = nullptr;
  std::vector<int> mwgPlan;
  bool uvMap = false;
  std::vector<long> h_uv[2];
  long *d_uv[2] = {nullptr, nullptr};
  int nUvU[2] = {0, 0}, nUvV[2] = {0, 0};
  long *d_uvAll[2] = {nullptr, nullptr};
  int nUvUAll[2] = {0, 0}, nUvVAll[2] = {0, 0};
  struct UvPre { const long *map = nullptr; int nU = 0, nV = 0; } uvPre[2][2];
  int *d_tileInfo = nullptr;
  double *exchBuf[2] = {nullptr, nullptr};
  long exchCap = 0;
  bool useGraph = true;
  hipGraphExec_t graphExec[2][4][3] = {};
  hipGraphExec_t graph1Exec[2][4][2] = {};
  double *graph1Tr[2][4][2][4] = {};
  bool ovlAuto = false, ovlDecided = false;
  float ovlMs[2] = {0.f, 0.f};
  hipEvent_t ovlEv[2] = {nullptr, nullptr};
  double *thetaA = nullptr, *saltA = nullptr;
  int stepLayout = 0;
  int shardFork = 0;
// ... 811 lines not shown
    dst[i] = field_ptr(m, fd);
    total += counts[i];
    maxc = std::max(maxc, counts[i]);
  }
  HIPCHK(hipSetDevice(m->device));
  const size_t bytes = (size_t)(2 + 2 * n + total) * sizeof(double);
  if (m->stCap < bytes) {
    HIPCHK(hipStreamSynchronize(m->stream));
    if (m->stCopy) HIPCHK(hipStreamSynchronize(m->stCopy));
    else HIPCHK(hipStreamCreateWithFlags(&m->stCopy, hipStreamNonBlocking));
    for (int q = 0; q < 2; q++) {
      if (m->stHost[q]) HIPCHK(hipHostFree(m->stHost[q]));
      if (m->stDev[q]) HIPCHK(hipFree(m->stDev[q]));
      m->stHost[q] = nullptr;
      m->stDev[q] = nullptr;
      HIPCHK(hipHostMalloc((void **)&m->stHost[q], bytes, hipHostMallocDefault));
      HIPCHK(hipMalloc((void **)&m->stDev[q], bytes));
      if (!m->stEv[q]) HIPCHK(hipEventCreateWithFlags(&m->stEv[q], hipEventDisableTiming));
      if (!m->stCopied[q]) HIPCHK(hipEventCreateWithFlags(&m->stCopied[q], hipEventDisableTiming));
    }
    m->stCap = bytes;
  }
  const int q = m->stNext;
  m->stNext ^= 1;
  HIPCHK(hipEventSynchronize(m->stEv[q]));
  long *hdr = reinterpret_cast<long *>(m->stHost[q]);
  double *vals = reinterpret_cast<double *>(m->stHost[q]) + 2 + 2 * n;
  hdr[0] = n;
  long o = 0;
  for (int i = 0; i < n; i++) {
    hdr[1 + i] = reinterpret_cast<long>(dst[i]);
    hdr[1 + n + i] = o;
    memcpy(vals + o, hosts[i], counts[i] * sizeof(double));
    o += counts[i];
  }
  hdr[1 + 2 * n] = o;
  HIPCHK(hipMemcpyAsync(m->stDev[q], m->stHost[q], bytes, hipMemcpyHostToDevice, m->stCopy));
  HIPCHK(hipEventRecord(m->stCopied[q], m->stCopy));
  HIPCHK(hipStreamWaitEvent(m->stream, m->stCopied[q], 0));
  const unsigned gx = (unsigned)std::min<long>(64, (maxc + 255) / 256);
  hipLaunchKernelGGL(mgcm::k_put_scatter, dim3(gx, n), dim3(256), 0, m->stream, m->stDev[q]);
  HIPCHK(hipGetLastError());
  HIPCHK(hipEventRecord(m->stEv[q], m->stream));
  return 0;
}

int mgcm_put_async(mgcm_model *m, const char *name, const double *host, long count) {
  return mgcm_put_batch_async(m, 1, &name, &host, &count);
}

int mgcm_get(mgcm_model *m, const char *name, double *host, long count) {
  const FieldDesc *fd = find_field(name);
  if (!fd) return set_err("mgcm_get: unknown field %s", name);
  const long n = field_count(m, fd->kind);
  if (count > n || count <= 0) return set_err("mgcm_get: %s count %ld > %ld", name, count, n);
  HIPCHK(hipSetDevice(m->device));
  HIPCHK(mg_host_copy(host, field_ptr(m, fd), count * sizeof(double), hipMemcpyDeviceToHost, m->stream));
  HIPCHK(hipStreamSynchronize(m->stream));
  return 0;
}

double *mgcm_device_ptr(mgcm_model *m, const char *name) {
  const FieldDesc *fd = find_field(name);
  if (!fd) { set_err("mgcm_device_ptr: unknown field %s", name); return nullptr; }
  return field_ptr(m, fd);
}

int mgcm_set_halo_map(mgcm_model *m, const long *src_of_point, long count) {
  const long N2 = m->d.n2 * m->d.nTiles;
  if (count != N2) return set_err("mgcm_set_halo_map: count %ld != %ld", count, N2);
  m->h_halo.clear();
  build_latlon_halo(m);
  std::vector<long> ll = m->h_halo;
  m->h_halo.clear();
  for (long q = 0; q < N2; q++)
    if (src_of_point[q] >= 0 && src_of_point[q] != q) {
      m->h_halo.push_back(q);
      m->h_halo.push_back(src_of_point[q]);
    }
  m->latlonTopology = (ll == m->h_halo);
  m->ready = false;
  return 0;
}

int mgcm_set_uv_map(mgcm_model *m, const long *u1, const long *v1, const long *u0, const long *v0,
                    const int *tileFace, const int *tileEdge, long count) {
  const long N2 = m->d.n2 * m->d.nTiles;
  if (count != N2) return set_err("mgcm_set_uv_map: count %ld != %ld", count, N2);
  const long *src[2][2] = {{u0, v0}, {u1, v1}};
  for (int w = 0; w < 2; w++) {
    m->h_uv[w].assign((size_t)2 * N2, 0);
    for (int c = 0; c < 2; c++)
      for (long q = 0; q < N2; q++) {
        const long code = src[w][c][q];
        const long s = (code > 0 ? code : -code) - 1;
        if (code != 0 && (s < 0 || s >= 2 * N2)) return set_err("mgcm_set_uv_map: bad code %ld at %ld", code, q);
        m->h_uv[w][(size_t)c * N2 + q] = code;
      }
  }
  std::vector<int> info(2 * (size_t)m->d.nTiles);
  for (int t = 0; t < m->d.nTiles; t++) { info[t] = tileFace[t]; info[m->d.nTiles + t] = tileEdge[t]; }
  HIPCHK(hipSetDevice(m->device));
  if (m->d_tileInfo) (void)hipFree(m->d_tileInfo);
  HIPCHK(hipMalloc(&m->d_tileInfo, info.size() * sizeof(int)));
  HIPCHK(hipMemcpy(m->d_tileInfo, info.data(), info.size() * sizeof(int), hipMemcpyHostToDevice));
  m->f.tileFace = m->d_tileInfo;
  m->f.tileEdge = m->d_tileInfo + m->d.nTiles;
  m->p.cubeCorners = 1;
  m->uvMap = true;
  m->ready = false;
  drop_graphs(m);
  return 0;
}

static hipError_t uv_pre(mgcm_model *m, const Dims &d, double *u, double *v, int nz, int w, bool all = false) {
  const mgcm_model::UvPre &p = m->uvPre[all ? 1 : 0][w];
  return launch_exchange_uv(d, u, v, p.map, p.nU, p.nV, nz, m->stream);
}

static int exchange_uv(mgcm_model *m, double *u, double *v, int nz, bool withSigns) {
  if (!m->uvMap) {
    HIPCHK(launch_exchange(m->d, u, m->d_halo, m->nHalo, nz, m->stream));
    HIPCHK(launch_exchange(m->d, v, m->d_halo, m->nHalo, nz, m->stream));
    return 0;
  }
  const int w = withSigns ? 1 : 0;
  HIPCHK(uv_pre(m, m->d, u, v, nz, w));
  HIPCHK(launch_exchange_uv(m->d, u, v, m->d_uv[w], m->nUvU[w], m->nUvV[w], nz, m->stream));
  return 0;
}

static Dims all_tiles(const Dims &d) { Dims a = d; a.t0 = 0; a.nT = d.nTiles; return a; }

static hipError_t calc_r_star(mgcm_model *m, bool fuseEtaH = false, int fromX = 0, bool stagEx = false) {
  const Dims da = all_tiles(m->d);
  hipError_t e;
  if (stagEx) {
    XFields xw{};
    xw.p[0] = m->f.wVel; xw.nz[0] = m->d.Nr; xw.n = 1;
    e = uv_pre(m, m->d, m->f.uVel, m->f.vVel, m->d.Nr, 1);
    if (e != hipSuccess) return e;
    e = launch_rstar_exmix(da, m->p, m->f, m->d_srcOf, fuseEtaH, fromX, m->f.uVel, m->f.vVel, m->d.Nr, m->d_uv[1],
                           m->nUvU[1], m->nUvV[1], xw, m->d_halo, m->nHalo, m->stream);
  } else
    e = launch_calc_r_star(da, m->p, m->f, m->d_srcOf, m->stream, fuseEtaH, fromX);
  if (e != hipSuccess || !m->uvMap) return e;
  double *us[3] = {m->f.rStarFacW, m->f.rStarDhWDt, m->f.rStarExpW}, *vs[3] = {m->f.rStarFacS, m->f.rStarDhSDt,
                                                                                 m->f.rStarExpS};
  for (int q = 0; q < 3; q++)
    if ((e = uv_pre(m, da, us[q], vs[q], 1, 0, true)) != hipSuccess) return e;
  return launch_exchange_uv_pairs(da, us, vs, 3, m->d_uvAll[0], m->nUvUAll[0], m->nUvVAll[0], m->stream);
}
static hipError_t update_r_star_cg2d(mgcm_model *m, bool sfp = false, bool opEarly = false, bool pcHere = false,
                                     const int *physNext = nullptr) {
  return launch_update_r_star_cg2d(all_tiles(m->d), m->p, m->f, m->d_srcOf, m->stream, sfp, opEarly, pcHere, physNext);
}

int mgcm_init(mgcm_model *m) {
  auto ext = [&](const char *n, double dflt) { auto it = m->extra.find(n); return it == m->extra.end() ? dflt : it->second; };
  HIPCHK(hipSetDevice(m->device));
  if (!m->snapH && m->p.nonlinFreeSurf > 0 && m->p.select_rStar > 0 && (m->p.tempStepping || m->p.saltStepping)) {
    HIPCHK(hipMalloc(&m->snapH, 6 * (size_t)m->d.N3all * sizeof(double)));
    m->allocs.push_back(m->snapH);
  }
  if (upload_halo(m)) return -1;
  m->noCompact = false;
  m->nPts = m->d.nTiles * m->d.sNx * m->d.sNy;
  BxyChoice bxy;
  if (choose_bxy(m, bxy)) return -1;
  if (m->p.cg2dRefOrder) {
    if (m->p.useSRCGSolver) return set_err("mgcm_init: cg2dRefOrder with useSRCGSolver not implemented");
    m->solver = m->nPts > cg2d_ref_max_points() ? Cg2dSolver::MwgRef : Cg2dSolver::BlockRef;
  } else
    m->solver = (bxy.var < 0 || ext("cg2dForceMwg", 0.0) != 0.0) ? Cg2dSolver::Mwg : Cg2dSolver::Bxy;
  if (m->p.useSRCGSolver && m->solver == Cg2dSolver::BlockRef)
    return set_err("mgcm_init: useSRCGSolver (CG2D_SR) is implemented in the blocked single-workgroup and the "
                   "multi-workgroup CG2D only");
  clear_bxy(m);
  if (m->solver == Cg2dSolver::Bxy ? build_bxy(m, bxy) : m->solver == Cg2dSolver::BlockRef ? build_block(m) : build_mwg(m))
    return -1;
  if (!m->h_dropG.empty()) {
    const long n2a = m->d.n2 * m->d.nTiles;
    std::vector<double> eta((size_t)n2a);
    for (const char *nm : {"etaN", "etaH"}) {
      if (!strcmp(nm, "etaH") && m->p.nIter0 == 0) continue;
      HIPCHK(hipMemcpy(eta.data(), !strcmp(nm, "etaN") ? m->f.etaN : m->f.etaH, n2a * sizeof(double), hipMemcpyDeviceToHost));
      if (land_eta_check(m, nm, eta.data(), n2a)) return -1;
    }
  }
  if ((m->p.viscA4D != 0.0 || m->p.viscA4Z != 0.0) && (m->d.OLx < 3 || m->d.OLy < 3))
    return set_err("mgcm_init: biharmonic viscosity needs OLx, OLy >= 3 (del2u of the halo ring)");
  const bool rstar = m->p.nonlinFreeSurf > 0;
  if (rstar) {
    if (m->p.nonlinFreeSurf != 4 || m->p.select_rStar != 2)
      return set_err("mgcm_init: the non-linear free surface is implemented for nonlinFreeSurf=4, select_rStar=2 only");
    if (!m->p.exactConserv) return set_err("mgcm_init: nonlinFreeSurf needs exactConserv");
  }
  if (m->p.selectP_inEOS_Zc > 2) return set_err("mgcm_init: selectP_inEOS_Zc = 3 needs the non-hydrostatic pressure");
  if (m->p.selectP_inEOS_Zc == 2 && !m->p.storePhiHyd4Phys)
    return set_err("mgcm_init: selectP_inEOS_Zc = 2 needs storePhiHyd4Phys (set_parms.F:297)");
  if (m->p.implicitViscosity && (ext("momImplVertAdv", 0.0) != 0.0 || ext("selectImplicitDrag", 0.0) != 0.0))
    return set_err("mgcm_init: momImplVertAdv / selectImplicitDrag not implemented on the device");
  if (m->p.vectorInvariantMomentum) {
    if (m->d.OLx < 2 || m->d.OLy < 2) return set_err("mgcm_init: vector-invariant momentum needs OLx, OLy >= 2");
    if (m->p.viscA4D != 0.0 || m->p.viscA4Z != 0.0)
      return set_err("mgcm_init: biharmonic viscosity with vectorInvariantMomentum not implemented on the device");
    if (m->p.useNHMTerms || m->p.select3dCoriScheme > 0 || m->p.useCDscheme)
      return set_err("mgcm_init: NH metric / 3-D Coriolis / CD scheme with vectorInvariantMomentum not implemented");
    if (m->p.selectVortScheme < 0 || m->p.selectVortScheme > 3 || m->p.selectKEscheme < 0 || m->p.selectKEscheme > 3 ||
        m->p.selectCoriScheme < 0 || m->p.selectCoriScheme > 3)
      return set_err("mgcm_init: selectVortScheme/selectKEscheme/selectCoriScheme outside 0..3");
    auto e = m->extra.find("useAbsVorticity");
    if (e != m->extra.end() && e->second != 0.0) return set_err("mgcm_init: useAbsVorticity not implemented");
  }
  if (m->uvMap && m->p.useCDscheme) return set_err("mgcm_init: CD scheme on an EXCH2 topology not implemented");
  if (m->p.implicSurfPress != 1.0 || m->p.implicDiv2DFlow != 1.0)
    return set_err("mgcm_init: implicSurfPress/implicDiv2DFlow != 1 not supported yet");
  const bool sph = ext("usingSphericalPolarGrid", 0.0) != 0.0;
  m->p.metricSphere = sph && ext("selectMetricTerms", 1.0) >= 1.0;
  m->p.recip_rSphere = sph ? 1.0 / ext("rSphere", 6370.0e3) : 0.0;
  if (ext("integr_GeoPot", 2.0) != 2.0) return set_err("mgcm_init: only integr_GeoPot = 2 is implemented");
  auto okScheme = [&](int s, const char *vname) {
    return (s == 2 || s == 3 || s == 4 || ((s == 30 || s == 33) && m->p.multiDimAdvection)) &&
           ext(vname, (double)s) == (double)s;
  };
  auto wideScheme = [&](int s) { return s == 3 || s == 4; };
  if (((m->p.tempStepping && wideScheme(m->p.tempAdvScheme)) || (m->p.saltStepping && wideScheme(m->p.saltAdvScheme))) &&
      (m->uvMap || m->d.OLx < 2 || m->d.OLy < 2))
    return set_err("mgcm_init: advection schemes 3 / 4 need OLx, OLy >= 2 and a lat-lon topology on the device");
  if (m->p.useAB3 && (m->p.momStepping || (m->p.nonlinFreeSurf > 0 && m->p.select_rStar > 0) || m->p.staggerTimeStep))
    return set_err("mgcm_init: ADAMS_BASHFORTH3 only for the tracers (momStepping off, no r*, not staggered)");
  if (m->p.useAB3 && m->p.nIter0 != 0) return set_err("mgcm_init: ADAMS_BASHFORTH3 from a pickup (nIter0 != 0) not supported");
  auto mdScheme = [&](int s) { return s == 30 || s == 33; };
  if (m->uvMap && ((m->p.tempStepping && mdScheme(m->p.tempAdvScheme)) || (m->p.saltStepping && mdScheme(m->p.saltAdvScheme)))) {
    if (!m->f.tileFace) return set_err("mgcm_init: multi-dimensional advection on EXCH2 needs the tile face table");
    if (m->d.OLx != m->d.OLy) return set_err("mgcm_init: cube multi-dimensional advection needs OLx = OLy");
    if (m->d.OLx < 4 || m->d.OLy < 4)
      return set_err("mgcm_init: multi-dimensional advection on the cube needs OLx, OLy >= 4 (GAD_CHECK: Overlap Size too small)");
  }
  if (m->p.tempStepping && !okScheme(m->p.tempAdvScheme, "tempVertAdvScheme"))
    return set_err("mgcm_init: tempAdvScheme %d not implemented on the device", m->p.tempAdvScheme);
  if (m->p.saltStepping && !okScheme(m->p.saltAdvScheme, "saltVertAdvScheme"))
    return set_err("mgcm_init: saltAdvScheme %d not implemented on the device", m->p.saltAdvScheme);
  if (m->p.useGMRedi && m->p.GM_AdvForm && m->p.multiDimAdvection &&
      ((m->p.tempStepping && mdScheme(m->p.tempAdvScheme)) || (m->p.saltStepping && mdScheme(m->p.saltAdvScheme))))
    return set_err("mgcm_init: GM_AdvForm with multi-dimensional advection is not implemented on the device");
  if (m->p.useGMRedi && m->p.GM_AdvForm && m->p.GM_skewflx != 0.0)
    return set_err("mgcm_init: GM_AdvForm needs GM_skewflx = 0 (gmredi_readparms.F:243-244)");
  if (m->p.eosType != 0 && m->p.eosType != 1) return set_err("mgcm_init: eosType %d not implemented", m->p.eosType);
  if (m->d.Nr > 64) return set_err("mgcm_init: Nr = %d > 64 (column kernels hold a column in one workgroup)", m->d.Nr);
  if (m->p.periodicExternalForcing && (m->p.nForcRec < 1 || m->p.nForcRec > MG_MAXREC))
    return set_err("mgcm_init: nForcRec %d outside 1..%d", m->p.nForcRec, MG_MAXREC);
  drop_graphs(m);
  m->thetaA = m->f.theta;
  m->saltA = m->f.salt;
  m->useGraph = true;
  int it0 = m->p.nIter0;
  HIPCHK(hipMemcpyAsync(m->d_ctr, &it0, sizeof(int), hipMemcpyHostToDevice, m->stream));
  if (m->p.nIter0 == 0)
    HIPCHK(hipMemcpyAsync(m->f.etaH, m->f.etaN, m->d.n2 * m->d.nTiles * sizeof(double), hipMemcpyDeviceToDevice,
                          m->stream));
  if (rstar) {
    HIPCHK(calc_r_star(m));
    HIPCHK(update_r_star_cg2d(m));
    HIPCHK(launch_corr_cont(m->d, m->p, m->f, 1, m->stream));
    HIPCHK(launch_exch_eta(m->d, m->p, m->f, m->d_srcOf, true, 1, m->stream));
    HIPCHK(launch_exchange(m->d, m->f.wVel, m->d_halo, m->nHalo, m->d.Nr, m->stream));
    HIPCHK(calc_r_star(m));
    HIPCHK(hipStreamSynchronize(m->stream));
  }
  m->ready = true;
  return 0;
}

static bool cg2d_fuses_eta(const mgcm_model *m) {
  return m->solver == Cg2dSolver::Bxy && m->d.nT == m->d.nTiles;
}

static hipError_t launch_cg2d(mgcm_model *m, int maxIters, int nIterMin, bool fuseEta = false) {
  switch (m->solver) {
    case Cg2dSolver::Bxy:
      return launch_cg2d_bxy(m->bxyVar, m->d, m->p, m->f, m->d_nbx, m->d_blkx, m->nBlkX, maxIters, nIterMin, m->d_rec,
                             m->d_ctr + 1, fuseEta ? m->d_slot2 : nullptr, m->d_srcOf, m->d_dropG, (int)m->h_dropG.size(),
                             m->h_dropG.empty() ? nullptr : m->d_guard, m->stream);
    case Cg2dSolver::BlockRef:
      return launch_cg2d_block(m->d, m->p, m->f, m->d_nbr, m->d_gofs, m->nPts, maxIters, nIterMin, m->d_rec, m->d_ctr + 1,
                               m->stream);
    case Cg2dSolver::Mwg:
    case Cg2dSolver::MwgRef:
      return launch_cg2d_mwg(m->d, m->p, m->f, m->mwg, maxIters, nIterMin, m->d_rec, m->d_ctr + 1, m->stream);
  }
  return hipErrorInvalidValue;
}

static int land_uncompact(mgcm_model *m) {
  HIPCHK(hipSetDevice(m->device));
  HIPCHK(hipStreamSynchronize(m->stream));
  drop_graphs(m);
  m->noCompact = true;
  BxyChoice bxy;
  if (choose_bxy(m, bxy)) return -1;
  if (m->h_guard) *m->h_guard = 0;
  if (bxy.var < 0) {
    clear_bxy(m);
    return set_err("land_uncompact: no single-workgroup CG2D fits this grid without leaving the all-land blocks out");
  }
  return build_bxy(m, bxy);
}
static int land_eta_check(mgcm_model *m, const char *name, const double *host, long n) {
  if (m->h_dropG.empty() || (strcmp(name, "etaN") && strcmp(name, "etaH"))) return 0;
  for (int g : m->h_dropG)
    if (g < n && !(host[g] == 0.0)) return land_uncompact(m);
  return 0;
}
static int land_guard_check(mgcm_model *m, const char *who) {
  if (m->h_guard && *(volatile int *)m->h_guard)
    return set_err("%s: a CG2D solve of an earlier step found a non-zero cg2d_b or cg2d_x on a land point of a block left "
                   "out of the solver's tables (recorded as numIters = -1); its results are invalid -- load the state "
                   "through mgcm_put / mgcm_init, which check eta on those points, or set MGCM_CG2D_COMPACT=0", who);
  return 0;
}

static int check_ready(mgcm_model *m) {
  if (!m->ready) return set_err("model not initialised: call mgcm_init() after loading the fields");
  return 0;
}

#define TIMED(K, CALL)                      \
  do {                                      \
    int ev_ = ev_begin(m, K);               \
    hipError_t e_ = (CALL);                 \
    ev_end(m, K, ev_);                      \
    if (e_ != hipSuccess) return set_err("%s: %s", KNAMES[K], hipGetErrorString(e_)); \
  } while (0)

static int dynamics_on(mgcm_model *m, bool ring) {
  TIMED(K_PHI, launch_phi_hyd(m->d, m->p, m->f, m->stream));
  TIMED(K_MOM, launch_mom_step(m->d, m->p, m->f, m->d_ctr, m->stream, ring));
  return 0;
}
int mgcm_dynamics(mgcm_model *m) {
  if (check_ready(m)) return -1;
  return dynamics_on(m, true);
}

static TracerArgs tracer_args(mgcm_model *m, bool salt) {
  const Params &p = m->p;
  TracerArgs a{};
  const int scheme = salt ? p.saltAdvScheme : p.tempAdvScheme;
  a.tr = salt ? m->f.salt : m->f.theta;
  a.trNext = salt ? m->f.saltNext : m->f.thetaNext;
  a.gNm1 = salt ? m->f.gsNm1 : m->f.gtNm1;
  a.scr = salt ? m->f.cpScr : m->f.gTscr;
  a.cp = salt ? m->f.advScr2 : m->f.advScr1;
  a.sfc = salt ? m->f.surfaceForcingS : m->f.surfaceForcingT;
  a.diffKh = salt ? p.diffKhS : p.diffKhT;
  a.diffKr = salt ? p.diffKrS : p.diffKrT;
  a.dT = p.deltaTtracer;
  a.advection = salt ? p.saltAdvection : p.tempAdvection;
  a.forcing = salt ? p.saltForcing : p.tempForcing;
  const bool abScheme = scheme == 2 || scheme == 3 || scheme == 4;
  a.multiDim = p.multiDimAdvection && a.advection && !abScheme;
  a.useAB = abScheme;
  a.limiter = scheme == 33;
  a.scheme = scheme;
  a.gNm2 = salt ? m->f.gsNm2 : m->f.gtNm2;
  return a;
}

static int tracers_on(mgcm_model *m, hipStream_t st, const Fields *fo = nullptr) {
  const TracerArgs aT = tracer_args(m, false), aS = tracer_args(m, true);
  const Fields &F = fo ? *fo : m->f;
  if (tracer_hpair_ok(m->d, m->p, aT, aS)) {
    TIMED(K_TEMP, launch_tracer_hpair(m->d, m->p, F, aT, aS, m->d_ctr, st));
    std::swap(m->f.theta, m->f.thetaNext);
    std::swap(m->f.salt, m->f.saltNext);
    return 0;
  }
  if (m->p.tempStepping) {
    TIMED(K_TEMP, launch_tracer_step(m->d, m->p, F, tracer_args(m, false), m->d_ctr, st));
    std::swap(m->f.theta, m->f.thetaNext);
  }
  if (m->p.saltStepping) {
    TIMED(K_TEMP, launch_tracer_step(m->d, m->p, F, tracer_args(m, true), m->d_ctr, st));
    std::swap(m->f.salt, m->f.saltNext);
  }
  return 0;
}

int mgcm_thermodynamics(mgcm_model *m) {
  if (check_ready(m)) return -1;
  TIMED(K_PHYS, launch_oceanic_phys(m->d, m->p, m->f, m->d_ctr, m->stream));
  return tracers_on(m, m->stream);
}

static int solve_impl(mgcm_model *m) {
  TIMED(K_RHS, launch_sfp_rhs(m->d, m->p, m->f, m->stream));
  const int nIterMin = m->p.cg2dUseMinResSol - 1;
  TIMED(K_CG2D, launch_cg2d(m, m->p.cg2dMaxIters, nIterMin));
  TIMED(K_ETA, launch_exch_eta(m->d, m->p, m->f, m->d_srcOf, false, 0, m->stream));
  return 0;
}

int mgcm_solve_for_pressure(mgcm_model *m) {
  if (check_ready(m)) return -1;
  return solve_impl(m);
}

int mgcm_momentum_correction_step(mgcm_model *m) {
  if (check_ready(m)) return -1;
  TIMED(K_CORR, launch_correction(m->d, m->p, m->f, m->stream));
  return 0;
}

int mgcm_integr_continuity(mgcm_model *m) {
  if (check_ready(m)) return -1;
  TIMED(K_CONT, launch_corr_cont(m->d, m->p, m->f, 2, m->stream));
  if (m->p.exactConserv) TIMED(K_ETA, launch_exch_eta(m->d, m->p, m->f, m->d_srcOf, true, 0, m->stream));
  return 0;
}

int mgcm_update_r_star(mgcm_model *m) {
  if (check_ready(m)) return -1;
  if (m->p.nonlinFreeSurf > 0) TIMED(K_RSTAR, update_r_star_cg2d(m));
  return 0;
}

int mgcm_calc_r_star(mgcm_model *m) {
  if (check_ready(m)) return -1;
  if (m->p.nonlinFreeSurf > 0) TIMED(K_RSTAR, calc_r_star(m));
  return 0;
}

static XFields blocking_fields(const mgcm_model *m, int tracers = 1);

int mgcm_blocking_exchanges(mgcm_model *m) {
  if (check_ready(m)) return -1;
  if (m->uvMap) TIMED(K_EXCH, exchange_uv(m, m->f.uVel, m->f.vVel, m->d.Nr, true) ? hipErrorUnknown : hipSuccess);
  TIMED(K_EXCH, launch_exchange_multi(m->d, blocking_fields(m), m->d_halo, m->nHalo, nullptr, m->stream));
  return 0;
}

int mgcm_stagger_exchanges(mgcm_model *m) {
  if (check_ready(m)) return -1;
  if (m->uvMap) {
    XFields xw{};
    xw.p[0] = m->f.wVel; xw.nz[0] = m->d.Nr; xw.n = 1;
    HIPCHK(uv_pre(m, m->d, m->f.uVel, m->f.vVel, m->d.Nr, 1));
    TIMED(K_EXCH, launch_exchange_mixed(m->d, m->f.uVel, m->f.vVel, m->d.Nr, m->d_uv[1], m->nUvU[1], m->nUvV[1], xw,
                                        m->d_halo, m->nHalo, nullptr, m->stream));
  } else {
    TIMED(K_EXCH, exchange_uv(m, m->f.uVel, m->f.vVel, m->d.Nr, true) ? hipErrorUnknown : hipSuccess);
    TIMED(K_EXCH, launch_exchange(m->d, m->f.wVel, m->d_halo, m->nHalo, m->d.Nr, m->stream));
  }
  return 0;
}

int mgcm_oceanic_phys(mgcm_model *m) {
  if (check_ready(m)) return -1;
  TIMED(K_PHYS, launch_oceanic_phys(m->d, m->p, m->f, m->d_ctr, m->stream));
  return 0;
}

int mgcm_tracer_step(mgcm_model *m) {
  if (check_ready(m)) return -1;
  return tracers_on(m, m->stream);
}

static int exch_scratch(mgcm_model *m, int nz) {
  const long need = (long)nz * m->d.n2 * m->d.nTiles;
  if (need <= m->exchCap) return 0;
  for (auto &q : m->exchBuf)
    if (q) { hipFree(q); q = nullptr; }
  HIPCHK(hipMalloc(&m->exchBuf[0], need * sizeof(double)));
  HIPCHK(hipMalloc(&m->exchBuf[1], need * sizeof(double)));
  m->exchCap = need;
  return 0;
}

int mgcm_exchange_host(mgcm_model *m, double *u, double *v, int nz, int vector, int withSigns) {
  if (!m->d_srcOf && upload_halo(m)) return -1;
  if (nz < 1 || nz > m->d.Nr) return set_err("mgcm_exchange_host: nz = %d outside 1..%d", nz, m->d.Nr);
  if (vector && !v) return set_err("mgcm_exchange_host: a vector exchange needs both components");
  if (exch_scratch(m, nz)) return -1;
  HIPCHK(hipSetDevice(m->device));
  const size_t bytes = (size_t)nz * m->d.n2 * m->d.nTiles * sizeof(double);
  double *host[2] = {u, v};
  for (int c = 0; c < 2; c++)
    if (host[c]) HIPCHK(mg_host_copy(m->exchBuf[c], host[c], bytes, hipMemcpyHostToDevice, m->stream));
  const long *hmap = m->d_haloAll ? m->d_haloAll : m->d_halo;
  const int nh = m->d_haloAll ? m->nHaloAll : m->nHalo;
  if (vector && m->uvMap) {
    const int w = withSigns ? 1 : 0;
    HIPCHK(uv_pre(m, m->d, m->exchBuf[0], m->exchBuf[1], nz, w, true));
    HIPCHK(launch_exchange_uv(m->d, m->exchBuf[0], m->exchBuf[1], m->d_uvAll[w], m->nUvUAll[w], m->nUvVAll[w], nz,
                              m->stream));
  } else {
    for (int c = 0; c < 2; c++)
      if (host[c]) HIPCHK(launch_exchange(m->d, m->exchBuf[c], hmap, nh, nz, m->stream));
  }
  for (int c = 0; c < 2; c++)
    if (host[c]) HIPCHK(mg_host_copy(host[c], m->exchBuf[c], bytes, hipMemcpyDeviceToHost, m->stream));
  HIPCHK(hipStreamSynchronize(m->stream));
  return 0;
}

const char *mgcm_param_name(int i) {
  const int n = (int)(sizeof(PARAMS) / sizeof(PARAMS[0]));
  return (i >= 0 && i < n) ? PARAMS[i].name : nullptr;
}

long mgcm_field_count(mgcm_model *m, const char *name) {
  const FieldDesc *fd = find_field(name);
  if (!fd) { set_err("mgcm_field_count: unknown field %s", name); return -1; }
  return field_count(m, fd->kind);
}

static XFields blocking_fields(const mgcm_model *m, int tracers) {
  XFields x{};
  double *fl[] = {m->f.uVel, m->f.vVel, m->f.wVel, m->f.theta, m->f.salt, m->f.uVelD, m->f.vVelD, m->f.totPhiHyd};
  const bool use[] = {!m->uvMap, !m->uvMap, true, m->p.tempStepping != 0, m->p.saltStepping != 0, m->p.useCDscheme != 0,
                      m->p.useCDscheme != 0, m->p.storePhiHyd4Phys != 0};
  for (int q = 0; q < 8; q++) {
    const bool tr = q == 3 || q == 4;
    if (use[q] && (tracers == 1 || (tracers == 2) == tr)) { x.p[x.n] = fl[q]; x.nz[x.n] = m->d.Nr; x.n++; }
  }
  return x;
}

enum StepMode {
  STEP_PLAIN = 0,
  STEP_HOIST = 1,
  STEP_LAST = 2
};
#define MG_PIPE_MIN_STEPS 4
static bool step_pipelinable(mgcm_model *m) {
  const Params &p = m->p;
  const bool tracers = p.tempStepping && p.saltStepping;
  const bool stagger = p.staggerTimeStep != 0 && p.momStepping;
  if (stagger || !m->overlap || !p.momStepping || !tracers || !mg_fuse_on(MG_FUSE_PIPE)) return false;
  if (p.nonlinFreeSurf <= 0 || p.select_rStar <= 0 || !p.useRealFreshWaterFlux || !p.exactConserv) return false;
  if (m->d.nT != m->d.nTiles || m->uvMap || !m->d_srcOf) return false;
  if (p.nonlinFreeSurf > 0 && p.select_rStar > 0 && m->snapH && mg_fuse_on(MG_FUSE_TCG)) return false;
  const TracerArgs aT = tracer_args(m, false), aS = tracer_args(m, true);
  if (!dyn_thermo_fusable(m->d, p, aT, aS) || !dyn_thermo_takes_gm(p) || phys_phi_fusable(m->d, p)) return false;
  if (!mg_fuse_on(MG_FUSE_SFP) || !mg_hfuse(MG_FUSE_END, m->d.nx, m->d.ny, m->d.nT, m->d.Nr)) return false;
  if (p.eosType == 1 && p.selectP_inEOS_Zc == 2 && !p.storePhiHyd4Phys) return false;
  return true;
}
static int one_step(mgcm_model *m, StepMode mode = STEP_PLAIN) {
  const bool pipe = mode != STEP_PLAIN, hoist = mode == STEP_HOIST;
  if (pipe && !step_pipelinable(m)) return set_err("one_step: the pipelined step does not apply to this model");
  const bool stagger = m->p.staggerTimeStep != 0 && m->p.momStepping;
  const bool tracers = m->p.tempStepping || m->p.saltStepping;
  const bool fork = !stagger && m->overlap && !m->timing && m->p.momStepping && tracers;
  bool endFused = false;
  bool stagEx = false;
  const bool lateJoin = fork && m->p.nonlinFreeSurf <= 0;
  const bool thermoLate = lateJoin;
  const bool trEx = lateJoin && mg_fuse_on(MG_FUSE_TREX);
  const bool ringAside = thermoLate && mom_ring_separable(m->d, m->p) && mg_fuse_on(MG_FUSE_RING);
  auto fork_thermo = [&]() -> int {
    HIPCHK(hipEventRecord(m->evFork, m->stream));
    HIPCHK(hipStreamWaitEvent(m->stream2, m->evFork, 0));
    if (ringAside) HIPCHK(launch_mom_ring(m->d, m->p, m->f, m->d_ctr, m->stream2));
    if (tracers_on(m, m->stream2)) return -1;
    if (trEx) {
      const XFields xt = blocking_fields(m, 2);
      if (xt.n > 0) HIPCHK(launch_exchange_multi(m->d, xt, m->d_halo, m->nHalo, nullptr, m->stream2));
    }
    HIPCHK(hipEventRecord(m->evJoin, m->stream2));
    return 0;
  };
  const TracerArgs aT = tracer_args(m, false), aS = tracer_args(m, true);
  const bool forkable = !stagger && m->overlap && m->p.momStepping && tracers;
  const bool tcg = forkable && m->p.nonlinFreeSurf > 0 && m->p.select_rStar > 0 && m->snapH &&
                   mg_fuse_on(MG_FUSE_TCG);
  const bool tcgFork = tcg && fork;
  const bool dtFused = forkable && !tcg && m->p.nonlinFreeSurf > 0 &&
                       dyn_thermo_fusable(m->d, m->p, aT, aS);
  auto fork_tcg = [&]() -> int {
    HIPCHK(hipEventRecord(m->evFork, m->stream));
    HIPCHK(hipStreamWaitEvent(m->stream2, m->evFork, 0));
    HIPCHK(launch_hfac_snapshot(m->d, m->f, m->snapH, m->stream2));
    HIPCHK(hipEventRecord(m->evSnap, m->stream2));
    HIPCHK(launch_gm_tensor(m->d, m->p, m->f, m->stream2));
    const Fields fT = hfac_snapshot_fields(m->d, m->f, m->snapH);
    if (tracers_on(m, m->stream2, &fT)) return -1;
    HIPCHK(hipEventRecord(m->evJoin, m->stream2));
    return 0;
  };
  m->mwg.exclusive = thermoLate ? 1 : 0;
  const bool physPhi = !stagger && m->p.momStepping && phys_phi_fusable(m->d, m->p);
  m->stepLayout = (dtFused ? 1 : 0) | (physPhi ? 2 : 0) | (forkable && !dtFused ? 4 : 0) |
                  ((forkable && m->p.nonlinFreeSurf <= 0) || tcg ? 8 : 0) | (pipe ? 16 : 0);
  const bool gmPhi = (stagger || thermoLate) && !dtFused && !physPhi && !m->timing && gm_phi_fusable(m->d, m->p);
  bool ringPhys = false;
  const bool ringPhysOk = !ringAside && !physPhi && mom_ring_separable(m->d, m->p) && mg_fuse_on(MG_FUSE_RINGP);
  auto phys = [&]() -> int {
    if (pipe) return 0;
    if (physPhi) TIMED(K_PHYS, launch_phys_phi(m->d, m->p, m->f, m->d_ctr, m->stream));
    else TIMED(K_PHYS, launch_oceanic_phys(m->d, m->p, m->f, m->d_ctr, m->stream,
                                           !(dtFused && dyn_thermo_takes_gm(m->p)) && !gmPhi && !tcgFork,
                                           ringPhysOk ? &ringPhys : nullptr));
    return 0;
  };
  if (stagger || fork || dtFused) {
    if (phys()) return -1;
    if (tcgFork) {
      if (fork_tcg()) return -1;
    } else if (fork && !thermoLate && !dtFused && fork_thermo()) return -1;
  } else {
    if (phys() || tracers_on(m, m->stream)) return -1;
  }
  const bool opEarly = dtFused && m->p.nonlinFreeSurf > 2 && dyn_thermo_takes_gm(m->p) && m->d.nT == m->d.nTiles &&
                       mg_fuse_on(MG_FUSE_OPE);
  if (m->p.momStepping) {
    if (dtFused) {
      TIMED(K_MOM, launch_dyn_thermo(m->d, m->p, m->f, aT, aS, m->d_ctr, m->stream, opEarly ? m->d_srcOf : nullptr,
                                     !pipe));
      std::swap(m->f.theta, m->f.thetaNext);
      std::swap(m->f.salt, m->f.saltNext);
    } else if (physPhi) TIMED(K_MOM, launch_mom_step(m->d, m->p, m->f, m->d_ctr, m->stream, !ringAside && !ringPhys));
    else if (gmPhi) {
      TIMED(K_PHI, launch_gm_phi(m->d, m->p, m->f, m->stream));
      TIMED(K_MOM, launch_mom_step(m->d, m->p, m->f, m->d_ctr, m->stream, !ringAside && !ringPhys));
    } else if (dynamics_on(m, !ringAside && !ringPhys)) return -1;
    if (tcgFork) HIPCHK(hipStreamWaitEvent(m->stream, m->evSnap, 0));
    else if (fork && !lateJoin && !dtFused) HIPCHK(hipStreamWaitEvent(m->stream, m->evJoin, 0));
    const bool sfpFused = mg_fuse_on(MG_FUSE_SFP) && m->p.nonlinFreeSurf > 0 && m->d.nT == m->d.nTiles;
    if (m->p.nonlinFreeSurf > 0)
      TIMED(K_RSTAR, update_r_star_cg2d(m, sfpFused, opEarly, false, hoist ? m->d_ctr : nullptr));
    if (!sfpFused) TIMED(K_RHS, launch_sfp_rhs(m->d, m->p, m->f, m->stream));
    if (thermoLate && fork_thermo()) return -1;
    const bool etaFused = mg_fuse_on(MG_FUSE_ETA) && cg2d_fuses_eta(m);
    TIMED(K_CG2D, launch_cg2d(m, m->p.cg2dMaxIters, m->p.cg2dUseMinResSol - 1, etaFused));
    const bool etaX = !etaFused && m->p.exactConserv && mg_fuse_on(MG_FUSE_ETAX) && m->d.nT == m->d.nTiles;
    const bool etaAside = !etaX && !etaFused && m->p.exactConserv && !m->timing && mg_fuse_on(MG_FUSE_ETAA) &&
                          m->d.nT == m->d.nTiles;
    if (etaX) {
    } else if (etaAside) {
      HIPCHK(hipEventRecord(m->evEta0, m->stream));
      HIPCHK(hipStreamWaitEvent(m->stream3, m->evEta0, 0));
      HIPCHK(launch_exch_eta(m->d, m->p, m->f, m->d_srcOf, false, 0, m->stream3));
      HIPCHK(hipEventRecord(m->evEta1, m->stream3));
    } else if (!etaFused) {
      TIMED(K_ETA, launch_exch_eta(m->d, m->p, m->f, m->d_srcOf, false, 0, m->stream));
    }
    if (lateJoin || tcgFork) HIPCHK(hipStreamWaitEvent(m->stream, m->evJoin, 0));
    TIMED(K_CONT, launch_corr_cont(m->d, m->p, m->f, 0, m->stream, (etaAside || etaX) ? m->d_srcOf : nullptr, hoist));
    if (etaAside) HIPCHK(hipStreamWaitEvent(m->stream, m->evEta1, 0));
    const bool fuseEtaH = m->p.exactConserv && m->p.nonlinFreeSurf > 0;
    if (m->p.exactConserv && !fuseEtaH)
      TIMED(K_ETA, launch_exch_eta(m->d, m->p, m->f, m->d_srcOf, true, 0, m->stream, etaX ? 1 : 0));
    endFused = m->p.nonlinFreeSurf > 0 && !stagger && !m->uvMap && m->d.nT == m->d.nTiles &&
               mg_hfuse(MG_FUSE_END, m->d.nx, m->d.ny, m->d.nT, m->d.Nr);
    if (endFused)
      TIMED(K_RSTAR, launch_rstar_exch(m->d, m->p, m->f, m->d_srcOf, fuseEtaH, blocking_fields(m), m->d_halo, m->nHalo,
                                       m->d_ctr, m->stream, etaX ? 1 : 0,
                                       hoist && m->p.periodicExternalForcing ? 1 : 0));
    else if (m->p.nonlinFreeSurf > 0) {
      stagEx = stagger && tracers && m->uvMap && m->d.nT == m->d.nTiles &&
               mg_hfuse(MG_FUSE_ENDS, m->d.nx, m->d.ny, m->d.nT, m->d.Nr);
      TIMED(K_RSTAR, calc_r_star(m, fuseEtaH, etaX ? 1 : 0, stagEx));
    }
  } else {
    if (mgcm_integr_continuity(m)) return -1;
  }
  if (stagger && tracers) {
    if (stagEx) {
    } else if (m->uvMap) {
      XFields xw{};
      xw.p[0] = m->f.wVel; xw.nz[0] = m->d.Nr; xw.n = 1;
      HIPCHK(uv_pre(m, m->d, m->f.uVel, m->f.vVel, m->d.Nr, 1));
      TIMED(K_EXCH, launch_exchange_mixed(m->d, m->f.uVel, m->f.vVel, m->d.Nr, m->d_uv[1], m->nUvU[1], m->nUvV[1], xw,
                                          m->d_halo, m->nHalo, nullptr, m->stream));
    } else {
      TIMED(K_EXCH, exchange_uv(m, m->f.uVel, m->f.vVel, m->d.Nr, true) ? hipErrorUnknown : hipSuccess);
      TIMED(K_EXCH, launch_exchange(m->d, m->f.wVel, m->d_halo, m->nHalo, m->d.Nr, m->stream));
    }
    if (tracers_on(m, m->stream)) return -1;
  }
  if (endFused) return 0;
  const XFields xEnd = blocking_fields(m, trEx ? 0 : 1);
  if (m->uvMap) {
    HIPCHK(uv_pre(m, m->d, m->f.uVel, m->f.vVel, m->d.Nr, 1));
    TIMED(K_EXCH, launch_exchange_mixed(m->d, m->f.uVel, m->f.vVel, m->d.Nr, m->d_uv[1], m->nUvU[1], m->nUvV[1], xEnd,
                                        m->d_halo, m->nHalo, m->d_ctr, m->stream));
  } else
    TIMED(K_EXCH, launch_exchange_multi(m->d, xEnd, m->d_halo, m->nHalo, m->d_ctr, m->stream));
  return 0;
}

static void drop_graphs(mgcm_model *m) {
  for (auto &row : m->graphExec)
    for (auto &col : row)
      for (auto &ge : col)
        if (ge) { (void)hipGraphExecDestroy(ge); ge = nullptr; }
  for (auto &row : m->graph1Exec)
    for (auto &col : row)
      for (auto &ge : col)
        if (ge) { (void)hipGraphExecDestroy(ge); ge = nullptr; }
}

static int buffer_parity(const mgcm_model *m) {
  return (m->f.theta == m->thetaA ? 0 : 1) + (m->f.salt == m->saltA ? 0 : 2);
}

static int two_step_graph(mgcm_model *m, hipGraphExec_t *out, int v = 0) {
  const int q = buffer_parity(m), o = m->overlap ? 1 : 0;
  if (!m->graphExec[o][q][v]) {
    hipGraph_t g = nullptr;
    HIPCHK(hipStreamBeginCapture(m->stream, hipStreamCaptureModeThreadLocal));
    int rc = one_step(m, v ? STEP_HOIST : STEP_PLAIN);
    if (!rc) rc = one_step(m, v == 1 ? STEP_HOIST : v == 2 ? STEP_LAST : STEP_PLAIN);
    hipError_t e = hipStreamEndCapture(m->stream, &g);
    if (rc) { if (g) (void)hipGraphDestroy(g); return -1; }
    HIPCHK(e);
    e = hipGraphInstantiate(&m->graphExec[o][q][v], g, nullptr, nullptr, 0);
    (void)hipGraphDestroy(g);
    HIPCHK(e);
  }
  *out = m->graphExec[o][q][v];
  return 0;
}

static int one_step_graph(mgcm_model *m, hipGraphExec_t *out, int v = 0) {
  const int q = buffer_parity(m), o = m->overlap ? 1 : 0;
  if (!m->graph1Exec[o][q][v]) {
    double *pre[4] = {m->f.theta, m->f.thetaNext, m->f.salt, m->f.saltNext};
    hipGraph_t g = nullptr;
    HIPCHK(hipStreamBeginCapture(m->stream, hipStreamCaptureModeThreadLocal));
    const int rc = one_step(m, v ? STEP_LAST : STEP_PLAIN);
    hipError_t e = hipStreamEndCapture(m->stream, &g);
    if (rc) { if (g) (void)hipGraphDestroy(g); return -1; }
    HIPCHK(e);
    e = hipGraphInstantiate(&m->graph1Exec[o][q][v], g, nullptr, nullptr, 0);
    (void)hipGraphDestroy(g);
    HIPCHK(e);
    double **tr[4] = {&m->f.theta, &m->f.thetaNext, &m->f.salt, &m->f.saltNext};
    for (int k = 0; k < 4; k++) m->graph1Tr[o][q][v][k] = *tr[k];
    m->f.theta = pre[0]; m->f.thetaNext = pre[1]; m->f.salt = pre[2]; m->f.saltNext = pre[3];
  }
  *out = m->graph1Exec[o][q][v];
  return 0;
}
int mgcm_tracer_parity(mgcm_model *m, int set) {
  if (set < 0) return buffer_parity(m);
  if (set > 3) return set_err("mgcm_tracer_parity: parity %d outside 0..3", set);
  double *tB = m->f.theta == m->thetaA ? m->f.thetaNext : m->f.theta;
  double *sB = m->f.salt == m->saltA ? m->f.saltNext : m->f.salt;
  m->f.theta = (set & 1) ? tB : m->thetaA;
  m->f.thetaNext = (set & 1) ? m->thetaA : tB;
  m->f.salt = (set & 2) ? sB : m->saltA;
  m->f.saltNext = (set & 2) ? m->saltA : sB;
  return set;
}

static void one_step_graph_done(mgcm_model *m, int o, int q, int v) {
  m->f.theta = m->graph1Tr[o][q][v][0]; m->f.thetaNext = m->graph1Tr[o][q][v][1];
  m->f.salt = m->graph1Tr[o][q][v][2]; m->f.saltNext = m->graph1Tr[o][q][v][3];
}

static int ovl_trial(mgcm_model *m);

int mgcm_prepare(mgcm_model *m) {
  if (check_ready(m)) return -1;
  if (!m->useGraph) return 0;
  HIPCHK(hipSetDevice(m->device));
  if (m->ovlAuto && !m->ovlDecided && ovl_trial(m)) return -1;
  hipGraphExec_t ge;
  if (step_pipelinable(m) && (two_step_graph(m, &ge, 1) || two_step_graph(m, &ge, 2))) return -1;
  return two_step_graph(m, &ge);
}

static int ovl_trial(mgcm_model *m) {
  const bool forkable = !m->p.staggerTimeStep && m->p.momStepping && (m->p.tempStepping || m->p.saltStepping);
  if (!forkable) { m->ovlDecided = true; return 0; }
  std::vector<std::pair<void *, size_t>> parts = {
      {m->f.a2, (size_t)F2_COUNT * m->d.N2all * sizeof(double)},
      {m->f.a3, (size_t)F3_COUNT * m->d.N3all * sizeof(double)},
      {m->d_ctr, 2 * sizeof(int)},
      {m->d_rec, (size_t)m->maxRec * sizeof(SolveRecord)}};
  for (auto &fd : FIELDS)
    if (fd.kind != F2D && fd.kind != F3D && field_ptr(m, &fd))
      parts.push_back({field_ptr(m, &fd), (size_t)field_count(m, fd.kind) * sizeof(double)});
  size_t total = 0;
  for (auto &pr : parts) total += (pr.second + 255) & ~(size_t)255;
  char *save = nullptr;
  if (hipMalloc(&save, total) != hipSuccess) {
    (void)hipGetLastError();
    m->ovlDecided = true;
    return 0;
  }
  const bool ovl0 = m->overlap;
  int rc = 0;
  size_t off = 0;
  for (auto &pr : parts) {
    if (!rc && hipMemcpyAsync(save + off, pr.first, pr.second, hipMemcpyDeviceToDevice, m->stream) != hipSuccess) rc = -1;
    off += (pr.second + 255) & ~(size_t)255;
  }
  for (int ph = 0; ph < 6 && !rc; ph++) {
    const int pairs = ph < 2 ? 1 : 2, mode = (ph & 1) ? 0 : 1;
    m->overlap = mode != 0;
    hipGraphExec_t ge;
    if (two_step_graph(m, &ge)) { rc = -1; break; }
    if (hipEventRecord(m->ovlEv[0], m->stream) != hipSuccess) { rc = -1; break; }
    for (int r = 0; r < pairs && !rc; r++)
      if (two_step_graph(m, &ge) || hipGraphLaunch(ge, m->stream) != hipSuccess) rc = -1;
    float ms = 0.f;
    if (rc || hipEventRecord(m->ovlEv[1], m->stream) != hipSuccess || hipEventSynchronize(m->ovlEv[1]) != hipSuccess ||
        hipEventElapsedTime(&ms, m->ovlEv[0], m->ovlEv[1]) != hipSuccess) { rc = -1; break; }
    if (ph >= 2) m->ovlMs[mode] += ms;
  }
  int rs = 0;
  off = 0;
  for (auto &pr : parts) {
    if (hipMemcpyAsync(pr.first, save + off, pr.second, hipMemcpyDeviceToDevice, m->stream) != hipSuccess) rs = -1;
    off += (pr.second + 255) & ~(size_t)255;
  }
  if (hipStreamSynchronize(m->stream) != hipSuccess) rs = -1;
  (void)hipFree(save);
  if (rc || rs) {
    m->overlap = ovl0;
    return set_err(rs ? "ovl_trial: restoring the saved state failed" : "ovl_trial: graph replay failed");
  }
  m->ovlDecided = true;
  m->overlap = m->ovlMs[1] <= m->ovlMs[0];
  return 0;
}

int mgcm_forward_step(mgcm_model *m, int nsteps) {
  if (check_ready(m)) return -1;
  if (land_guard_check(m, "mgcm_forward_step")) return -1;
  if (nsteps <= 0 || nsteps > m->maxRec) return set_err("mgcm_forward_step: nsteps %d out of range", nsteps);
  HIPCHK(hipSetDevice(m->device));
  HIPCHK(hipMemsetAsync(m->d_ctr + 1, 0, sizeof(int), m->stream));
  int s = 0;
  if (m->useGraph && !m->timing && m->ovlAuto && !m->ovlDecided && nsteps >= 2 && ovl_trial(m)) return -1;
  const bool pipe = nsteps >= MG_PIPE_MIN_STEPS && step_pipelinable(m);
  if (pipe) TIMED(K_PHYS, launch_oceanic_phys(m->d, m->p, m->f, m->d_ctr, m->stream));
  if (m->useGraph && !m->timing) {
    for (; s + 2 <= nsteps; s += 2) {
      hipGraphExec_t ge;
      if (two_step_graph(m, &ge, pipe ? (s + 2 == nsteps ? 2 : 1) : 0)) return -1;
      HIPCHK(hipGraphLaunch(ge, m->stream));
    }
  }
  if (s < nsteps && m->useGraph && !m->timing) {
    const int q = buffer_parity(m), o = m->overlap ? 1 : 0;
    hipGraphExec_t ge;
    if (one_step_graph(m, &ge, pipe ? 1 : 0)) return -1;
    HIPCHK(hipGraphLaunch(ge, m->stream));
    one_step_graph_done(m, o, q, pipe ? 1 : 0);
    s++;
  }
  for (; s < nsteps; s++)
    if (one_step(m, pipe ? (s == nsteps - 1 ? STEP_LAST : STEP_HOIST) : STEP_PLAIN)) return -1;
  m->stepLayout = (m->stepLayout & ~16) | (pipe ? 16 : 0);
  m->lastBatch = nsteps;
  return 0;
}

int mgcm_set_tile_range(mgcm_model *m, int t0, int nT) {
  if (t0 < 0 || nT < 1 || t0 + nT > m->d.nTiles)
    return set_err("mgcm_set_tile_range: tiles [%d, %d) outside [0, %d)", t0, t0 + nT, m->d.nTiles);
  if (m->solver == Cg2dSolver::MwgRef && nT < m->d.nTiles)
    return set_err("mgcm_set_tile_range: cg2dRefOrder in the multi-workgroup CG2D needs the whole domain's tiles, not the "
                   "tile range [%d, %d) of %d", t0, t0 + nT, m->d.nTiles);
  m->d.t0 = t0;
  m->d.nT = nT;
  drop_graphs(m);
  if (m->ready) {
    HIPCHK(hipSetDevice(m->device));
    HIPCHK(hipStreamSynchronize(m->stream));
    if (upload_halo(m)) return -1;
  }
  return 0;
}

int mgcm_set_stream(mgcm_model *m, void *stream) {
  HIPCHK(hipSetDevice(m->device));
  HIPCHK(hipStreamSynchronize(m->stream));
  drop_graphs(m);
  m->stream = stream ? (hipStream_t)stream : m->ownStream;
  return 0;
}

static XFields transfer_fields(const mgcm_model *m, int group = 0) {
  XFields x{};
  double *fl[] = {m->f.uVel, m->f.vVel, m->f.wVel, m->f.theta, m->f.salt, m->f.uVelD, m->f.vVelD, m->f.totPhiHyd};
  const bool use[] = {true, true, true, m->p.tempStepping != 0, m->p.saltStepping != 0, m->p.useCDscheme != 0,
                      m->p.useCDscheme != 0, m->p.storePhiHyd4Phys != 0};
  const bool tracer[] = {false, false, false, true, true, false, false, false};
  for (int q = 0; q < 8; q++)
    if (use[q] && (group == 0 || (group == 1) == tracer[q])) { x.p[x.n] = fl[q]; x.nz[x.n] = m->d.Nr; x.n++; }
  return x;
}

int mgcm_exchange_nfields(mgcm_model *m) { return transfer_fields(m).n; }
int mgcm_exchange_nfields_group(mgcm_model *m, int group) {
  if (group < 0 || group > 2) return -1;
  return transfer_fields(m, group).n;
}

int mgcm_halo_pack(mgcm_model *m, const long *idx, long n, double *buf, int unpack) {
  return mgcm_halo_pack_group(m, 0, idx, n, buf, unpack);
}

int mgcm_halo_pack_group(mgcm_model *m, int group, const long *idx, long n, double *buf, int unpack) {
  if (check_ready(m)) return -1;
  if (group < 0 || group > 2) return set_err("mgcm_halo_pack_group: no group %d", group);
  HIPCHK(launch_halo_pack(m->d, transfer_fields(m, group), idx, n, buf, unpack, m->stream));
  return 0;
}

int mgcm_stream_handoff(mgcm_model *m, void *other, int direction) {
  hipStream_t o = (hipStream_t)other;
  if (o == m->stream) return 0;
  HIPCHK(hipSetDevice(m->device));
  if (direction == 0) {
    HIPCHK(hipEventRecord(m->evHand, m->stream));
    HIPCHK(hipStreamWaitEvent(o, m->evHand, 0));
  } else {
    HIPCHK(hipEventRecord(m->evHand, o));
    HIPCHK(hipStreamWaitEvent(m->stream, m->evHand, 0));
  }
  return 0;
}

int mgcm_tile_copy(mgcm_model *m, const char *name, int t0, int nT, void *buf, int toField) {
  const FieldDesc *fd = find_field(name);
  if (!fd || fd->kind == F1D) return set_err("mgcm_tile_copy: no 2-D/3-D field '%s'", name);
  if (t0 < 0 || nT < 0 || t0 + nT > m->d.nTiles) return set_err("mgcm_tile_copy: bad tile range");
  const long per = fd->kind == F2D ? m->d.n2 : m->d.n3;
  double *f = field_ptr(m, fd) + t0 * per;
  const size_t bytes = (size_t)nT * per * sizeof(double);
  HIPCHK(hipMemcpyAsync(toField ? f : buf, toField ? buf : f, bytes, hipMemcpyDeviceToDevice, m->stream));
  return 0;
}

static int mwg_block_uncached(mgcm_model *m);

static int mwg_ref_refuse(const mgcm_model *m, const char *who) {
  if (m->solver != Cg2dSolver::MwgRef) return 0;
  return set_err("%s: cg2dRefOrder in the multi-workgroup CG2D runs the whole domain in one launch of one model "
                 "(no tile ranges, no shared hand-off block)", who);
}

static int mwg_restart_epoch(mgcm_model *m, bool zeroBlock) {
  if (zeroBlock) HIPCHK(hipMemset(m->mwg.ctr, 0, m->mwg.hsBytes));
  HIPCHK(hipMemset(m->mwg.epoch, 0, 64));
  HIPCHK(hipDeviceSynchronize());
  return 0;
}

int mgcm_cg2d_shared_export(mgcm_model *m, void *handle) {
  if (!m->useMwg() || m->mwg.partsPerTile <= 0)
    return set_err("mgcm_cg2d_shared_export: needs the multi-workgroup CG2D on whole-domain tables (cg2dForceMwg)");
  if (mwg_ref_refuse(m, "mgcm_cg2d_shared_export")) return -1;
  HIPCHK(hipSetDevice(m->device));
  HIPCHK(hipStreamSynchronize(m->stream));
  if (mwg_block_uncached(m) || mwg_restart_epoch(m, true)) return -1;
  hipIpcMemHandle_t h;
  HIPCHK(hipIpcGetMemHandle(&h, (void *)m->mwg.ctr));
  memcpy(handle, &h, sizeof h);
  return 0;
}

int mgcm_cg2d_shared_import(mgcm_model *m, const void *handle) {
  if (!m->useMwg() || m->mwg.partsPerTile <= 0)
    return set_err("mgcm_cg2d_shared_import: needs the multi-workgroup CG2D on whole-domain tables (cg2dForceMwg)");
  if (mwg_ref_refuse(m, "mgcm_cg2d_shared_import")) return -1;
  HIPCHK(hipSetDevice(m->device));
  HIPCHK(hipStreamSynchronize(m->stream));
  if (m->mwgShared) { (void)hipIpcCloseMemHandle(m->mwgShared); m->mwgShared = nullptr; }
  hipIpcMemHandle_t h;
  memcpy(&h, handle, sizeof h);
  void *p = nullptr;
  HIPCHK(hipIpcOpenMemHandle(&p, h, hipIpcMemLazyEnablePeerAccess));
  m->mwgShared = p;
  const size_t partGr = (size_t)2 * 3 * m->mwg.G * 2;
  m->mwg.ctr = (unsigned *)p;
  m->mwg.part = (unsigned long long *)((char *)p + 64);
  m->mwg.xs = m->mwg.part + partGr;
  m->mwg.sys = 1;
  if (mwg_restart_epoch(m, false)) return -1;
  drop_graphs(m);
  return 0;
}

int mgcm_cg2d_shared_bytes(mgcm_model *m) { return m->useMwg() ? (int)sizeof(hipIpcMemHandle_t) : -1; }

int mgcm_end_steps(mgcm_model *m, int nsteps) {
  if (nsteps < 0 || nsteps > m->maxRec) return set_err("mgcm_end_steps: nsteps %d out of range", nsteps);
  m->lastBatch = nsteps;
  return 0;
}

int mgcm_begin_steps(mgcm_model *m) {
  if (check_ready(m)) return -1;
  HIPCHK(hipSetDevice(m->device));
  HIPCHK(hipMemsetAsync(m->d_ctr + 1, 0, sizeof(int), m->stream));
  m->lastBatch = 0;
  return 0;
}

static int shard_fork_thermo(mgcm_model *m, bool ring = false) {
  HIPCHK(hipEventRecord(m->evFork, m->stream));
  HIPCHK(hipStreamWaitEvent(m->stream2, m->evFork, 0));
  if (ring) HIPCHK(launch_mom_ring(m->d, m->p, m->f, m->d_ctr, m->stream2));
  if (tracers_on(m, m->stream2)) return -1;
// ... 478 lines not shown
```

mitgcm_amd/model.py:

```python
import ctypes

import numpy as np

from ._lib import check, lib, MgcmError

GRID_2D = ("dxF", "dyF", "dxG", "dyG", "dxC", "dyC", "dxV", "dyU", "rA", "rAw", "rAs",
           "recip_dxF", "recip_dyF", "recip_dxC", "recip_dyC", "recip_dxV", "recip_dyU",
           "recip_rA", "recip_rAw", "recip_rAs", "fCori", "Bo_surf", "recip_Bo",
           "aW2d", "aS2d", "aC2d", "pW", "pS", "pC", "maskInC", "tanPhiAtU", "tanPhiAtV",
           "fCoriCos", "recip_Rcol", "rSurfW", "rSurfS", "rLowW", "rLowS", "Ro_surf", "R_low", "maskInW", "maskInS",
           "fCoriG", "recip_rAz", "recip_dxG", "recip_dyG")
GRID_3D = ("hFacC", "hFacW", "hFacS", "recip_hFacC", "recip_hFacW", "recip_hFacS", "maskC", "maskW", "maskS",
           "h0FacC", "h0FacW", "h0FacS")
GRID_1D = ("drF", "drC", "recip_drF", "recip_drC", "rF", "rC")
STATE_1D = ("tRef", "sRef", "pRef4EOS", "phiRefC")
STATE_3D = ("uVel", "vVel", "wVel", "theta", "salt", "gU", "gV", "guNm1", "gvNm1", "gtNm1", "gsNm1", "rhoInSitu",
            "IVDConvCount", "sigmaR", "Kwx", "Kwy", "Kwz", "Kux", "Kvy", "uVelD", "vVelD", "uNM1", "vNM1",
            "totPhiHyd", "alphaRho", "del2u", "del2v", "Kuz", "Kvz", "GM_PsiX", "GM_PsiY")
STATE_2D = ("etaN", "etaH", "fu", "fv", "SST", "lambdaThetaClimRelax", "surfaceForcingT", "surfaceForcingS",
            "Qnet", "EmPmR", "SSS", "lambdaSaltClimRelax", "etaNm1", "rStarFacC", "rStarFacW", "rStarFacS",
            "rStarExpC", "rStarExpW", "rStarExpS", "rStarDhCDt", "rStarDhWDt", "rStarDhSDt", "PmEpR", "dEtaHdt")
FORCING_ORDER = ("SST", "SSS", "taux", "tauy", "Qnet", "EmPmR")

DEVICE_PARAMS = ("deltaTMom", "deltaTFreeSurf", "deltaTClock", "abEps", "rhoConst", "gBaro", "viscAhD",
                 "viscAhZ", "viscA4D", "viscA4Z", "viscAr", "sideDragFactor", "freeSurfFac", "implicSurfPress",
                 "implicDiv2DFlow", "rkSign", "afFacMom", "vfFacMom", "pfFacMom", "cfFacMom", "foFacMom",
                 "mtFacMom", "momAdvection", "momViscosity", "momForcing", "useCoriolis", "no_slip_sides",
                 "no_slip_bottom", "selectCoriScheme", "momForcingOutAB", "momDissip_In_AB", "implicitViscosity",
                 "cg2dMaxIters", "cg2dUseMinResSol", "nIter0", "vectorInvariantMomentum", "selectVortScheme",
                 "selectKEscheme", "upwindShear")


def _dp(a):
    return a.ctypes.data_as(ctypes.POINTER(ctypes.c_double))


class Model:
    def __init__(self, grid, params, device=0):
        self.g = grid
        self.params = dict(params)
        L = lib()
        g = grid
        self.h = L.mgcm_create(g.sNx, g.sNy, g.OLx, g.OLy, g.Nr, g.nSx, g.nSy, device)
        if not self.h:
            raise MgcmError("mgcm_create failed: " + L.mgcm_last_error().decode())
        for k, v in self.params.items():
            check(L.mgcm_set_param(self.h, k.encode(), float(v)), "mgcm_set_param(%s)" % k)
        check(L.mgcm_set_param(self.h, b"cg2dNorm", g.cg2dNorm), "cg2dNorm")
        check(L.mgcm_set_param(self.h, b"cg2dTolerance_sq", g.cg2dTolerance_sq), "cg2dTolerance_sq")
        check(L.mgcm_set_param(self.h, b"cg2dNormaliseRHS", float(g.cg2dNormaliseRHS)), "cg2dNormaliseRHS")
        for n in GRID_1D:
            a = np.zeros(g.Nr + 1)
            v = g.f[n]
            a[:len(v)] = v
            self.put(n, a)
        for n in GRID_2D + GRID_3D:
            if n in g.f:
                self.put(n, g.f[n])
        for n in ("rStarFacC", "rStarFacW", "rStarFacS", "rStarExpC", "rStarExpW", "rStarExpS"):
            self.put(n, np.ones((g.nTiles, g.ny, g.nx)))
        src = np.ascontiguousarray(g.topo.src_of_point(), dtype=np.int64)
        check(L.mgcm_set_halo_map(self.h, src.ctypes.data_as(ctypes.POINTER(ctypes.c_long)), src.size),
              "mgcm_set_halo_map")
        if hasattr(g.topo, "uv_codes"):
            topo = g.topo
            LP = lambda a: a.ctypes.data_as(ctypes.POINTER(ctypes.c_long))
            IP = lambda a: a.ctypes.data_as(ctypes.POINTER(ctypes.c_int))
            u1, v1 = (np.ascontiguousarray(x, dtype=np.int64) for x in topo.uv_codes(True))
            u0, v0 = (np.ascontiguousarray(x, dtype=np.int64) for x in topo.uv_codes(False))
            face = np.ascontiguousarray(topo.face[1:], dtype=np.int32)
            edge = np.ascontiguousarray([topo.isN[t] | 2 * topo.isS[t] | 4 * topo.isE[t] | 8 * topo.isW[t]
                                         for t in range(1, topo.nTiles + 1)], dtype=np.int32)
            check(L.mgcm_set_uv_map(self.h, LP(u1), LP(v1), LP(u0), LP(v0), IP(face), IP(edge), u1.size),
                  "mgcm_set_uv_map")

    def init(self):
        check(lib().mgcm_init(self.h), "mgcm_init")

    def close(self):
        if getattr(self, "h", None):
            lib().mgcm_destroy(self.h)
            self.h = None

    def __del__(self):
        try:
            self.close()
        except Exception:
            pass

    def _shape(self, name):
        g = self.g
        if name in GRID_1D or name in STATE_1D:
            return (g.Nr + 1,)
        if name in GRID_3D or name in STATE_3D:
            return (g.nTiles, g.Nr, g.ny, g.nx)
        if name == "forcRec":
            n = lib().mgcm_field_count(self.h, b"forcRec")
            return (6, n // (6 * g.nTiles * g.ny * g.nx), g.nTiles, g.ny, g.nx)
        return (g.nTiles, g.ny, g.nx)

    def put_forcing(self, forcing):
        recs = np.stack([np.asarray(forcing[n], dtype=np.float64) for n in FORCING_ORDER])
        check(lib().mgcm_set_param(self.h, b"nForcRec", float(recs.shape[1])), "nForcRec")
        self.put("forcRec", recs)

    def put(self, name, arr):
        if name == "phiRef":
            v = np.zeros(self.g.Nr + 1)
            v[:self.g.Nr] = np.asarray(arr)[1:2 * self.g.Nr:2]
            name, arr = "phiRefC", v
        a = np.ascontiguousarray(arr, dtype=np.float64)
        check(lib().mgcm_put(self.h, name.encode(), _dp(a), a.size), "mgcm_put(%s)" % name)

    def set(self, name, arr):
        self.put(name, arr)

    def get(self, name):
        a = np.zeros(self._shape(name))
        check(lib().mgcm_get(self.h, name.encode(), _dp(a), a.size), "mgcm_get(%s)" % name)
        return a

    def prepare(self):
        check(lib().mgcm_prepare(self.h), "mgcm_prepare")

    def forward_step(self, nsteps=1):
        check(lib().mgcm_forward_step(self.h, int(nsteps)), "mgcm_forward_step")

    def thermodynamics(self):
        check(lib().mgcm_thermodynamics(self.h), "mgcm_thermodynamics")

    def dynamics(self):
        check(lib().mgcm_dynamics(self.h), "mgcm_dynamics")

    def solve_for_pressure(self):
        check(lib().mgcm_solve_for_pressure(self.h), "mgcm_solve_for_pressure")

    def my_iter(self):
        return int(lib().mgcm_get_param(self.h, b"myIter"))

    def sync(self):
        check(lib().mgcm_sync(self.h), "mgcm_sync")

    def solve_stats(self, back=0):
        f, la, rm = ctypes.c_double(), ctypes.c_double(), ctypes.c_double()
        it = ctypes.c_int()
        check(lib().mgcm_solve_stats(self.h, back, ctypes.byref(f), ctypes.byref(la), ctypes.byref(it),
                                     ctypes.byref(rm)), "mgcm_solve_stats")
        return {"cg2d_init_res": f.value, "cg2d_last_res": la.value, "cg2d_iters": it.value,
                "cg2d_rhs_max": rm.value}

    def solve_minres(self, back=0):
        r, n = ctypes.c_double(), ctypes.c_int()
        check(lib().mgcm_solve_minres(self.h, back, ctypes.byref(r), ctypes.byref(n)), "mgcm_solve_minres")
        return r.value, n.value

    def solve_history(self, n):
        it = np.zeros(n, dtype=np.int32)
        fr = np.zeros(n)
        lr = np.zeros(n)
        check(lib().mgcm_solve_history(self.h, n, it.ctypes.data_as(ctypes.POINTER(ctypes.c_int)), _dp(fr), _dp(lr)),
              "mgcm_solve_history")
        return it, fr, lr

    def cg2d(self, b, x, maxIters, nIterMin=-1):
        b = np.ascontiguousarray(b, dtype=np.float64).copy()
        x = np.ascontiguousarray(x, dtype=np.float64).copy()
        f, mn, la = ctypes.c_double(), ctypes.c_double(), ctypes.c_double()
        it, itm = ctypes.c_int(maxIters), ctypes.c_int(nIterMin)
        check(lib().mgcm_cg2d(self.h, _dp(b), _dp(x), ctypes.byref(f), ctypes.byref(mn), ctypes.byref(la),
                              ctypes.byref(it), ctypes.byref(itm)), "mgcm_cg2d")
        return x, f.value, mn.value, la.value, it.value, itm.value

    def cg2d_sum_plan(self):
        cap = 1 << 24
        plan = np.zeros(cap, dtype=np.int32)
        nt, ppt, ng = ctypes.c_int(), ctypes.c_int(), ctypes.c_int()
        check(lib().mgcm_cg2d_sum_plan(self.h, plan.ctypes.data_as(ctypes.POINTER(ctypes.c_int)), cap,
                                       ctypes.byref(nt), ctypes.byref(ppt), ctypes.byref(ng)), "mgcm_cg2d_sum_plan")
        return plan[:nt.value * ppt.value * ng.value].copy(), nt.value, ppt.value, ng.value

    def cg2d_kernel(self):
        k = lib().mgcm_get_param(self.h, b"cg2dKernel")
        names = {3.0: "bxy", 4.0: "mwg", 5.0: "block_ref", 6.0: "mwg_ref"}
        if k not in names:
            raise RuntimeError("cg2dKernel = %r names no CG2D solver" % (k,))
        return names[k]

    def step_layout(self):
        b = int(lib().mgcm_get_param(self.h, b"stepLayout"))
        return {"dyn_thermo_fused": bool(b & 1), "phys_phi_fused": bool(b & 2), "thermo_second_stream": bool(b & 4),
                "late_join": bool(b & 8), "pipelined": bool(b & 16)}

    def cg2d_fma(self):
        return lib().mgcm_get_param(self.h, b"cg2dFMA") != 0.0

    def cg2d_parts(self):
        return int(lib().mgcm_get_param(self.h, b"cg2dParts"))

    def kernel_timing(self, enable):
        lib().mgcm_kernel_timing(self.h, 1 if enable else 0)

    def kernel_ms(self, name):
        n = ctypes.c_int()
        ms = lib().mgcm_kernel_ms(self.h, name.encode(), ctypes.byref(n))
        return ms, n.value


MON_FIELDS = ("eta", "uvel", "vvel", "wvel", "theta", "salt")
MON_STATS = ("max", "min", "mean", "sd", "del2")


def monitor(model):
    out = np.zeros(len(MON_FIELDS) * len(MON_STATS))
    check(lib().mgcm_monitor(model.h, _dp(out)), "mgcm_monitor")
    return {"dynstat_%s_%s" % (f, s): float(out[i * 5 + j]) for i, f in enumerate(MON_FIELDS)
            for j, s in enumerate(MON_STATS)}


def mon_stats(g, arr, hfac, mask, area, dr):
    OLx, OLy, sNx, sNy = g.OLx, g.OLy, g.sNx, g.sNy
    nz = arr.shape[1]
    theMin = theMax = 0.0
    noPnts = True
    tNb, tDel2, tVol, tMean = [], [], [], []
    for t in range(arr.shape[0]):
        nb = d2 = vol = mean = 0.0
        for k in range(nz):
            for j in range(1, sNy + 1):
                J = j + OLy - 1
                for i in range(1, sNx + 1):
                    I = i + OLx - 1
                    v = arr[t, k, J, I]
                    msk = mask[t, J, I] * hfac[t, k, J, I]
                    if msk > 0.0:
                        if noPnts:
                            theMin = theMax = v
                            noPnts = False
                        theMin = min(theMin, v)
                        theMax = max(theMax, v)
                        ddx = hfac[t, k, J, I + 1] * hfac[t, k, J, I - 1]
                        if ddx > 0.0:
                            ddx = (arr[t, k, J, I + 1] - v) + (arr[t, k, J, I - 1] - v)
                        ddy = hfac[t, k, J + 1, I] * hfac[t, k, J - 1, I]
                        if ddy > 0.0:
                            ddy = (arr[t, k, J + 1, I] - v) + (arr[t, k, J - 1, I] - v)
                        d2 = d2 + ddx * ddx + ddy * ddy
                        nb = nb + 1.0
                        tv = area[t, J, I] * dr[k] * msk
                        vol = vol + tv
                        mean = mean + tv * v
        tNb.append(nb); tDel2.append(d2); tVol.append(vol); tMean.append(mean)
    gs = lambda xs: sum(xs, 0.0)
    theNb, theDel2, theVol, theMean = gs(tNb), gs(tDel2), gs(tVol), gs(tMean)
    theSD = 0.0
    if theNb > 0.0:
        theDel2 = np.sqrt(theDel2) / theNb
    if theVol > 0.0:
        theMean = theMean / theVol
        sds = []
        for t in range(arr.shape[0]):
            sd = 0.0
            for k in range(nz):
                for j in range(1, sNy + 1):
                    J = j + OLy - 1
                    for i in range(1, sNx + 1):
                        I = i + OLx - 1
                        msk = mask[t, J, I] * hfac[t, k, J, I]
                        if msk > 0.0:
                            tv = area[t, J, I] * dr[k] * msk
                            sd = sd + tv * (arr[t, k, J, I] - theMean) * (arr[t, k, J, I] - theMean)
            sds.append(sd)
        theSD = np.sqrt(gs(sds) / theVol)
    return {"min": theMin, "max": theMax, "mean": theMean, "sd": theSD, "del2": theDel2}


def dynstat(model):
    g = model.g
    f = g.f
    out = {}
    eta = model.get("etaN")[:, None]
    hC, hW, hS = model.get("hFacC"), model.get("hFacW"), model.get("hFacS")
    for name, arr, hf, mask, area, dr in (
            ("eta", eta, f["maskInC"][:, None], f["maskInC"], f["rA"], f["drF"]),
            ("uvel", model.get("uVel"), hW, f["maskInW"], f["rAw"], f["drF"]),
            ("vvel", model.get("vVel"), hS, f["maskInS"], f["rAs"], f["drF"]),
            ("wvel", model.get("wVel"), f["maskC"], f["maskInC"], f["rA"], f["drC"]),
            ("theta", model.get("theta"), hC, f["maskInC"], f["rA"], f["drF"]),
            ("salt", model.get("salt"), hC, f["maskInC"], f["rA"], f["drF"])):
        st = mon_stats(g, arr, hf, mask, area, dr)
        for k, v in st.items():
            out["dynstat_%s_%s" % (name, k)] = float(v)
    return out
```

Before: 3899 model-days/s.

## Hoist CALC_PHI_HYD into the previous step's r* pass with on-the-fly r* factors

Adds a pipelined path, on by default through a new fuse bit, that computes the hydrostatic pressure and del2uv for the next step inside the r*-exchange pass of the current step. It does this by recomputing the r* factors and their time derivatives per point from saved previous factors and by reading halo values through the exchange source map, so no separate exchange or launch is needed. The aim is to remove a kernel launch and a serial dependency from each step. The cost is extra redundant arithmetic, more gathered reads, new saved-factor arrays and added code complexity.

```diff
diff --git a/mitgcm_amd/csrc/common.h b/mitgcm_amd/csrc/common.h
--- a/mitgcm_amd/csrc/common.h
+++ b/mitgcm_amd/csrc/common.h
@@ -21,7 +21,7 @@
     X(rSurfW) X(rSurfS) X(rLowW) X(rLowS) X(Ro_surf) X(R_low) X(rStarFacC) X(rStarFacW) X(rStarFacS) \
     X(rStarExpC) X(rStarExpW) X(rStarExpS) X(rStarDhCDt) X(rStarDhWDt) X(rStarDhSDt) X(PmEpR) X(dEtaHdt) \
     X(maskInW) X(maskInS) X(fCoriG) X(recip_rAz) X(recip_dxG) X(recip_dyG) X(etaHnm1) X(cg2d_r) X(cg2d_s) X(cg2d_q) \
-    X(cg2d_min) X(cg2d_y) X(cg2d_v) X(EmPmRnext)
+    X(cg2d_min) X(cg2d_y) X(cg2d_v) X(EmPmRnext) X(rStarFacCPrev) X(rStarFacWPrev) X(rStarFacSPrev)
 #define MG_F3D_LIST(X) X(hFacC) X(hFacW) X(hFacS) X(recip_hFacC) X(recip_hFacW) X(recip_hFacS) X(maskC) X(maskW) \
     X(maskS) X(uVel) X(vVel) X(wVel) X(theta) X(salt) X(gU) X(gV) X(guNm1) X(gvNm1) X(rhoInSitu) X(IVDConvCount) \
     X(gtNm1) X(thetaNext) X(gTscr) X(cpScr) X(phiHydC) X(saltNext) X(gsNm1) X(advScr1) X(advScr2) X(gAdv) \
@@ -110,6 +110,7 @@
   double *cg2d_min;
   double *cg2d_y, *cg2d_v;
   double *EmPmRnext;
+  double *rStarFacCPrev, *rStarFacWPrev, *rStarFacSPrev;
   double *a2, *a3;
 };
 typedef __attribute__((address_space(1))) double mg_gdouble;
@@ -199,11 +200,12 @@
 inline unsigned mg_colf_blocks(long ncols, int nc) { return (unsigned)((ncols + nc - 1) / nc); }
 enum { MG_FUSE_SFP = 1, MG_FUSE_ETA = 2, MG_FUSE_PHI = 4, MG_FUSE_END = 8, MG_FUSE_PHYS = 16, MG_FUSE_ETAA = 32,
        MG_FUSE_TREX = 64, MG_FUSE_DT = 128, MG_FUSE_ETAX = 256, MG_FUSE_TCG = 512, MG_FUSE_OPE = 1024,
-       MG_FUSE_RING = 2048, MG_FUSE_RINGP = 4096, MG_FUSE_ENDS = 8192, MG_FUSE_PIPE = 16384 };
+       MG_FUSE_RING = 2048, MG_FUSE_RINGP = 4096, MG_FUSE_ENDS = 8192, MG_FUSE_PIPE = 16384, MG_FUSE_PHIP = 32768 };
 inline bool mg_fuse_on(int bit) {
   const int mask = getenv("MGCM_STEP_FUSE") ? atoi(getenv("MGCM_STEP_FUSE"))
                                             : MG_FUSE_SFP | MG_FUSE_PHI | MG_FUSE_END | MG_FUSE_DT | MG_FUSE_ETAX |
-                                                MG_FUSE_OPE | MG_FUSE_RING | MG_FUSE_RINGP | MG_FUSE_ENDS | MG_FUSE_PIPE;
+                                                MG_FUSE_OPE | MG_FUSE_RING | MG_FUSE_RINGP | MG_FUSE_ENDS | MG_FUSE_PIPE |
+                                                MG_FUSE_PHIP;
   return (mask & bit) != 0;
 }
 inline bool mg_hfuse(int bit, long nx, long ny, long nT, long Nr) {
diff --git a/mitgcm_amd/csrc/kernels_dyn.hip b/mitgcm_amd/csrc/kernels_dyn.hip
--- a/mitgcm_amd/csrc/kernels_dyn.hip
+++ b/mitgcm_amd/csrc/kernels_dyn.hip
@@ -2,6 +2,7 @@
 
 #include "common.h"
 #include "phys.h"
+#include "rstar.h"
 #include <cstring>
 #include <cstdio>
 #include <type_traits>
@@ -23,7 +24,9 @@
               fmin(f.h0FacS[MG_I3(d, i, j, k, t)], f.h0FacS[MG_I3(d, i - 1, j, k, t)]));
 }
 
-__device__ __forceinline__ void del2uv_body(const Dims &d, const Params &p, const Fields &f, int lb) {
+template <bool HO = false>
+__device__ __forceinline__ void del2uv_body(const Dims &d, const Params &p, const Fields &f, int lb,
+                                            const long *__restrict__ srcOf = nullptr) {
   MG_PLANE_LB(1 - d.OLx, d.nx, 1 - d.OLy, d.ny, z, lb)
   const int t = d.t0 + z / d.Nr, k = z % d.Nr + 1;
   const long q3 = MG_I3(d, i, j, k, t);
@@ -33,8 +36,11 @@
     return;
   }
   const double drF = f.drF[k - 1];
-#define U(ii, jj) f.uVel[MG_I3(d, ii, jj, k, t)]
-#define V(ii, jj) f.vVel[MG_I3(d, ii, jj, k, t)]
+  auto uv3 = [&](int ii, int jj) { return HO ? mg_at_source3(d, srcOf, ii, jj, k, t) : MG_I3(d, ii, jj, k, t); };
+  const long qv[5] = {uv3(i, j), uv3(i - 1, j), uv3(i + 1, j), uv3(i, j - 1), uv3(i, j + 1)};
+  auto qvAt = [&](int ii, int jj) { return qv[jj == j ? (ii == i ? 0 : ii < i ? 1 : 2) : (jj < j ? 3 : 4)]; };
+#define U(ii, jj) f.uVel[HO ? qvAt(ii, jj) : MG_I3(d, ii, jj, k, t)]
+#define V(ii, jj) f.vVel[HO ? qvAt(ii, jj) : MG_I3(d, ii, jj, k, t)]
 #define G2(a, ii, jj) f.a[MG_I2(d, ii, jj, t)]
 #define G3(a, ii, jj) f.a[MG_I3(d, ii, jj, k, t)]
   {
@@ -76,9 +82,10 @@
 }
 __global__ void __launch_bounds__(256) k_del2uv(Dims d, Params p, Fields f) { del2uv_body(d, p, f, mg_xcd_block()); }
 
-template <bool PHYS = false>
+template <bool PHYS = false, bool HO = false>
 __device__ __forceinline__ void phi_hyd_body(const Dims &d, const Params &p, const Fields &f, int nc, int lb,
-                                             const int *iterPtr = nullptr) {
+                                             const int *iterPtr = nullptr, const long *__restrict__ srcOf = nullptr,
+                                             int fromX = 0) {
   extern __shared__ __attribute__((aligned(16))) double lds[];
   MG_COLF_LB(PHYS ? 1 - d.OLx : -1, PHYS ? d.nx : d.sNx + 3, PHYS ? 1 - d.OLy : -1, PHYS ? d.ny : d.sNy + 3, nc, lb)
   const int Nr = d.Nr, NS = Nr * NC_;
@@ -89,19 +96,37 @@
   const bool ring = inPhi && i >= 0 && j >= 0;
   const double recip_rhoConst = 1.0 / p.rhoConst;
   const long q2 = MG_I2(d, i, j, t);
+  double hoFacC = 0.0, hoDhC = 0.0, hoDhW = 0.0, hoDhS = 0.0;
+  const bool hoStash = HO && Nr >= 2 && KW_ >= 4;
+  auto hoD0 = [&](long r) {
+    double fc_ = 0.0, c_ = 0.0, w_ = 0.0, s_ = 0.0;
+    if constexpr (HO) r_star_next_point<false>(d, p, f, srcOf, r, fromX, fc_, c_, w_, s_);
+    return c_ * (f.Ro_surf[r] - f.R_low[r]) * f.rA[r];
+  };
+  bool hoHave = false;
   if (valid) MG_COLF_K(k) {
     const int me = (k - 1) * NC_ + cc;
     double dRlocM = 0.5 * f.drC[k - 1];
     if (k == 1) dRlocM = f.rF[0] - f.rC[0];
     const double dRlocP = (k == Nr) ? (f.rC[k - 1] - f.rF[k]) : 0.5 * f.drC[k];
     const long q3 = MG_I3(d, i, j, k, t);
+    double hoOp[7] = {0.0, 0.0, 0.0, 0.0, 0.0, 0.0, 0.0};
+    if constexpr (HO) {
+      if (rstar) {
+        hoOp[0] = f.drF[k - 1]; hoOp[1] = f.h0FacC[q3]; hoOp[2] = f.rA[q2];
+        if (ring) { hoOp[3] = f.h0FacW[q3]; hoOp[4] = f.rAw[q2]; hoOp[5] = f.h0FacS[q3]; hoOp[6] = f.rAs[q2]; }
+      }
+    }
     double a;
     if constexpr (PHYS) a = oceanic_phys_point(d, p, f, iterPtr, i, j, k, t);
     else a = f.rhoInSitu[q3];
     if (qh) {
       const double scalingFactor = p.rhoConst * p.gravitySign * (1.0 / p.gravity);
-      const double u0 = f.uVel[q3], u1 = f.uVel[MG_I3(d, i + 1, j, k, t)];
-      const double v0 = f.vVel[q3], v1 = f.vVel[MG_I3(d, i, j + 1, k, t)];
+      const long qc = HO ? mg_at_source3(d, srcOf, i, j, k, t) : q3;
+      const long qe = HO ? mg_at_source3(d, srcOf, i + 1, j, k, t) : MG_I3(d, i + 1, j, k, t);
+      const long qn = HO ? mg_at_source3(d, srcOf, i, j + 1, k, t) : MG_I3(d, i, j + 1, k, t);
+      const double u0 = f.uVel[qc], u1 = f.uVel[qe];
+      const double v0 = f.vVel[qc], v1 = f.vVel[qn];
       double gW = 0.0;
       if (p.select3dCoriScheme >= 1) gW = f.fCoriCos[q2] * (1.0 * 0.5 * (u0 + u1) - 0.0 * 0.5 * (v0 + v1));
       if (p.useNHMTerms) gW = gW + ((u0 * u0 + u1 * u1) + (v0 * v0 + v1 * v1)) * 0.5 * p.recip_rSphere;
@@ -111,16 +136,41 @@
     sM[me] = dRlocM * p.gravity * a * recip_rhoConst;
     sP[me] = dRlocP * p.gravity * a * recip_rhoConst;
     if (rstar) {
-      const double drF = f.drF[k - 1];
-      sC[me] = f.rStarDhCDt[q2] * drF * f.h0FacC[q3] * f.rA[q2];
-      if (ring) {
-        sU[me] = f.rStarDhWDt[q2] * drF * f.h0FacW[q3] * f.rAw[q2];
-        sV[me] = f.rStarDhSDt[q2] * drF * f.h0FacS[q3] * f.rAs[q2];
+      if constexpr (HO) {
+        if (!hoHave) {
+          r_star_next_point<true>(d, p, f, srcOf, q2, fromX, hoFacC, hoDhC, hoDhW, hoDhS);
+          hoHave = true;
+        }
+        sC[me] = hoDhC * hoOp[0] * hoOp[1] * hoOp[2];
+        if (ring) {
+          sU[me] = hoDhW * hoOp[0] * hoOp[3] * hoOp[4];
+          sV[me] = hoDhS * hoOp[0] * hoOp[5] * hoOp[6];
+        }
+      } else {
+        const double drF = f.drF[k - 1];
+        sC[me] = f.rStarDhCDt[q2] * drF * f.h0FacC[q3] * f.rA[q2];
+        if (ring) {
+          sU[me] = f.rStarDhWDt[q2] * drF * f.h0FacW[q3] * f.rAw[q2];
+          sV[me] = f.rStarDhSDt[q2] * drF * f.h0FacS[q3] * f.rAs[q2];
+        }
+      }
+    }
+  }
+  if constexpr (HO) {
+    if (valid && rstar) {
+      if (!hoHave && kk == 0) r_star_next_point<true>(d, p, f, srcOf, q2, fromX, hoFacC, hoDhC, hoDhW, hoDhS);
+      if (hoStash && ring) {
+        if (kk == KW_ / 4) sPh[cc] = hoD0(q2 - 1);
+        if (kk == KW_ / 2) sPh[NC_ + cc] = hoD0(q2 - d.nx);
       }
     }
   }
   __syncthreads();
   if (valid && kk == 0) {
+    double hoW = 0.0, hoS = 0.0;
+    if constexpr (HO) {
+      if (rstar && hoStash && ring) { hoW = sPh[cc]; hoS = sPh[NC_ + cc]; }
+    }
     double phF = 0.0;
     for (int k2 = 1; k2 <= Nr; k2++) {
       const int s2 = (k2 - 1) * NC_ + cc;
@@ -129,7 +179,15 @@
       sPh[s2] = phC;
     }
     if (rstar) {
-      auto d0 = [&](long r) { return f.rStarDhCDt[r] * (f.Ro_surf[r] - f.R_low[r]) * f.rA[r]; };
+      auto d0 = [&](long r) {
+        if constexpr (HO) {
+          if (r == q2) return hoDhC * (f.Ro_surf[r] - f.R_low[r]) * f.rA[r];
+          if (hoStash) return r == q2 - 1 ? hoW : hoS;
+          return hoD0(r);
+        } else {
+          return f.rStarDhCDt[r] * (f.Ro_surf[r] - f.R_low[r]) * f.rA[r];
+        }
+      };
       double c = d0(q2);
       double u = ring ? 0.5 * (d0(q2 - 1) + c) : 0.0, v = ring ? 0.5 * (d0(q2 - d.nx) + c) : 0.0;
       for (int k2 = 1; k2 <= Nr; k2++) {
@@ -162,7 +220,8 @@
         double tot;
         if (rstar && p.nonlinFreeSurf >= 4) {
           const double dPhiRef = (f.Ro_surf[q2] - f.rC[k - 1]) * p.gravity;
-          tot = phC * f.rStarFacC[q2] + fmax(dPhiRef, 0.0) * (f.rStarFacC[q2] - 1.0) + 0.0;
+          if constexpr (HO) tot = phC * hoFacC + fmax(dPhiRef, 0.0) * (hoFacC - 1.0) + 0.0;
+          else tot = phC * f.rStarFacC[q2] + fmax(dPhiRef, 0.0) * (f.rStarFacC[q2] - 1.0) + 0.0;
         } else {
           tot = phC + f.Bo_surf[q2] * f.etaN[q2] + 0.0;
         }
diff --git a/mitgcm_amd/csrc/kernels_rstar.hip b/mitgcm_amd/csrc/kernels_rstar.hip
--- a/mitgcm_amd/csrc/kernels_rstar.hip
+++ b/mitgcm_amd/csrc/kernels_rstar.hip
@@ -1,70 +1,10 @@
 #include "common.h"
 #include "phys.h"
+#include "rstar.h"
 #include "ucg2d.h"
 
 namespace mgcm {
 
-__device__ __forceinline__ double eta_exch(const Dims &d, const Fields &f, const long *srcOf, long q, int fromX) {
-  const long sq = srcOf[q];
-  if (sq >= 0) return f.cg2d_b[sq];
-  const long l = q % d.n2;
-  const int i = (int)(l % d.nx) - d.OLx + 1, j = (int)(l / d.nx) - d.OLy + 1;
-  if (i >= 1 && i <= d.sNx && j >= 1 && j <= d.sNy) return f.cg2d_b[q];
-  return fromX ? f.recip_Bo[q] * f.cg2d_x[q] : f.etaN[q];
-}
-
-template <bool FUSE>
-__device__ __forceinline__ void calc_r_star_body(const Dims &d, const Params &p, const Fields &f,
-                                                 const long *__restrict__ srcOf, int lb, int fromX, int empNext = 0) {
-  const long q = (long)lb * blockDim.x + threadIdx.x;
-  if (q >= d.n2 * d.nTiles) return;
-  const int t = (int)(q / d.n2);
-  if (t < d.t0 || t >= d.t0 + d.nT) return;
-  if constexpr (FUSE) {
-    if (p.nonlinFreeSurf > 0 && p.useRealFreshWaterFlux) f.PmEpR[q] = -f.EmPmR[q];
-    if (empNext) f.EmPmR[q] = f.EmPmRnext[q];
-    const double x = eta_exch(d, f, srcOf, q, fromX);
-    f.etaHnm1[q] = f.etaH[q];
-    f.etaN[q] = x;
-    f.etaH[q] = x;
-  }
-  const long sq = srcOf[q], r = sq >= 0 ? sq : q;
-  const long l = r % d.n2;
-  const int i = (int)(l % d.nx) - d.OLx + 1, j = (int)(l / d.nx) - d.OLy + 1;
-  auto eta = [&](long qq) { return FUSE ? eta_exch(d, f, srcOf, qq, fromX) : f.etaH[qq]; };
-  const double oc = f.rStarFacC[q], ow = f.rStarFacW[q], os = f.rStarFacS[q];
-  double fc = oc, fw = ow, fs = os;
-  if (i >= 0 && i <= d.sNx + 1 && j >= 0 && j <= d.sNy + 1)
-    fc = (f.maskInC[r] != 0.0) ? (eta(r) + f.Ro_surf[r] - f.R_low[r]) * f.recip_Rcol[r] : 1.0;
-  const long rv = p.cubeCorners ? q : r;
-  const long lv = rv % d.n2;
-  const int iv = (int)(lv % d.nx) - d.OLx + 1, jv = (int)(lv / d.nx) - d.OLy + 1;
-  if (iv >= 1 && iv <= d.sNx + 1 && jv >= 1 && jv <= d.sNy) {
-    if (f.maskInW[rv] != 0.0) {
-      const double tmp = f.rSurfW[rv] - f.rLowW[rv];
-      fw = (0.5 * (eta(rv - 1) * f.rA[rv - 1] + eta(rv) * f.rA[rv]) * f.recip_rAw[rv] + tmp) / tmp;
-    } else {
-      fw = 1.0;
-    }
-  }
-  if (iv >= 1 && iv <= d.sNx && jv >= 1 && jv <= d.sNy + 1) {
-    if (f.maskInS[rv] != 0.0) {
-      const double tmp = f.rSurfS[rv] - f.rLowS[rv];
-      fs = (0.5 * (eta(rv - d.nx) * f.rA[rv - d.nx] + eta(rv) * f.rA[rv]) * f.recip_rAs[rv] + tmp) / tmp;
-    } else {
-      fs = 1.0;
-    }
-  }
-  f.rStarFacC[q] = fc;
-  f.rStarFacW[q] = fw;
-  f.rStarFacS[q] = fs;
-  f.rStarDhCDt[q] = (fc - oc) / p.deltaTFreeSurf;
-  f.rStarDhWDt[q] = (fw - ow) / p.deltaTFreeSurf;
-  f.rStarDhSDt[q] = (fs - os) / p.deltaTFreeSurf;
-  f.rStarExpC[q] = fc / oc;
-  f.rStarExpW[q] = fw / ow;
-  f.rStarExpS[q] = fs / os;
-}
 template <bool FUSE>
 __global__ void __launch_bounds__(256) k_calc_r_star(Dims d, Params p, Fields f, const long *__restrict__ srcOf, int fromX) {
   calc_r_star_body<FUSE>(d, p, f, srcOf, (int)blockIdx.x, fromX);
@@ -90,13 +30,13 @@
   exchange_mixed_body(d, u, v, nzUV, uvMap, nU, nV, x, map, nHalo, nullptr, r % nbH, (r / nbH) % nzMax, r / (nbH * nzMax));
 }
 
-template <bool SFP, bool PH>
+template <bool SFP, int PH>
 __global__ void __launch_bounds__(256) k_update_r_star_cg2d_a(Dims d, Params p, Fields f, int nc, int opIn,
                                                               const long *__restrict__ srcOf, int nbPc,
                                                               const int *iterPtr, int nbPh) {
   extern __shared__ __attribute__((aligned(16))) double lds[];
   int lb = mg_xcd_block();
-  if constexpr (PH) {
+  if constexpr (PH != 0) {
     if (lb < nbPh) { phys_hoist_body(d, p, f, iterPtr, srcOf, lb); return; }
     lb -= nbPh;
   }
@@ -111,6 +51,9 @@
   const bool inner = i >= 1 && i <= d.sNx && j >= 1 && j <= d.sNy;
   if (valid) {
     const double fc = f.rStarFacC[q], fw = f.rStarFacW[q], fs = f.rStarFacS[q];
+    if constexpr (PH == 2) {
+      if (kk == 0) { f.rStarFacCPrev[q] = fc; f.rStarFacWPrev[q] = fw; f.rStarFacSPrev[q] = fs; }
+    }
     double fwE = 0.0, fsN = 0.0;
     if (SFP && inner) { fwE = f.rStarFacW[MG_I2(d, i + 1, j, t)]; fsN = f.rStarFacS[MG_I2(d, i, j + 1, t)]; }
     MG_COLF_K(k) {
@@ -205,23 +148,26 @@
 }
 
 hipError_t launch_update_r_star_cg2d(const Dims &d, const Params &p, const Fields &f, const long *srcOf, hipStream_t s,
-                                     bool sfp, bool opEarly, bool pcHere, const int *iterPtr) {
+                                     bool sfp, bool opEarly, bool pcHere, const int *iterPtr, bool keepFac) {
   const long n = d.n2 * d.nTiles;
   const unsigned nb = (unsigned)((n + 255) / 256);
   const long ncol = (long)d.nx * d.ny * d.nT;
   const int nArr = sfp ? 6 : 2;
   const int nc = mg_colf_nc(ncol, d.Nr, nArr);
-  auto kPlain = k_update_r_star_cg2d_a<false, false>, kSfp = k_update_r_star_cg2d_a<true, false>,
-       kSfpPhys = k_update_r_star_cg2d_a<true, true>;
+  auto kPlain = k_update_r_star_cg2d_a<false, 0>, kSfp = k_update_r_star_cg2d_a<true, 0>,
+       kSfpPhys = k_update_r_star_cg2d_a<true, 1>, kSfpPhysKeep = k_update_r_star_cg2d_a<true, 2>;
   MG_ALLOW_LDS(kPlain);
   MG_ALLOW_LDS(kSfp);
   const int nbPc = (opEarly && pcHere && p.nonlinFreeSurf > 2) ? (int)nb : 0;
   if (iterPtr) {
     if (!sfp) return hipErrorInvalidValue;
     MG_ALLOW_LDS(kSfpPhys);
+    MG_ALLOW_LDS(kSfpPhysKeep);
     const int nbPh = phys_hoist_blocks(d);
-    hipLaunchKernelGGL(kSfpPhys, dim3(mg_colf_blocks(ncol, nc) + (unsigned)(nbPc + nbPh)), dim3(256),
+    hipLaunchKernelGGL(keepFac ? kSfpPhysKeep : kSfpPhys, dim3(mg_colf_blocks(ncol, nc) + (unsigned)(nbPc + nbPh)), dim3(256),
                        mg_colf_lds(d.Nr, nc, nArr), s, d, p, f, nc, opEarly ? 0 : 1, srcOf, nbPc, iterPtr, nbPh);
+  } else if (keepFac) {
+    return hipErrorInvalidValue;
   } else
     hipLaunchKernelGGL(sfp ? kSfp : kPlain, dim3(mg_colf_blocks(ncol, nc) + (unsigned)nbPc), dim3(256),
                        mg_colf_lds(d.Nr, nc, nArr), s, d, p, f, nc, opEarly ? 0 : 1, srcOf, nbPc, (const int *)nullptr, 0);
diff --git a/mitgcm_amd/csrc/kernels_step.hip b/mitgcm_amd/csrc/kernels_step.hip
--- a/mitgcm_amd/csrc/kernels_step.hip
+++ b/mitgcm_amd/csrc/kernels_step.hip
@@ -1,6 +1,7 @@
 #include "kernels_dyn.hip"
 #include "kernels_thermo.hip"
 #include "ucg2d.h"
+#include "rstar.h"
 
 namespace mgcm {
 
@@ -189,7 +190,7 @@
 }
 
 hipError_t launch_dyn_thermo(const Dims &d, const Params &p, const Fields &f, const TracerArgs &aT, const TracerArgs &aS,
-                             const int *iterPtr, hipStream_t s, const long *srcOf, bool gmHere) {
+                             const int *iterPtr, hipStream_t s, const long *srcOf, bool gmHere, bool l1Here) {
   const dim3 blk(256);
   int ncPhi, nArrPhi, nbPhi;
   phi_frame(d, p, ncPhi, nArrPhi, nbPhi);
@@ -198,7 +199,8 @@
   if (dyn_thermo_takes_gm(p)) {
     const int nbU = srcOf ? ucg2d_blocks(d) : 0;
     const int nbOp1 = 0, nbPc2 = 0, nbOp2 = nbU, nbPc3 = nbU;
-    launch_l1(d, p, f, nbDel, s, nbOp1, gmHere);
+    if (l1Here) launch_l1(d, p, f, nbDel, s, nbOp1, gmHere);
+    else if (gmHere) return hipErrorInvalidValue;
     const bool ff4 = mom_ff4_on(true);
     const int nbMom = ff4 ? mom_ff4_blocks(d) : 2 * (int)mg_plane_blocks(d.nx, d.ny, d.nT * d.Nr);
     auto l2 = ff4 ? k_dt_l2<true, true> : k_dt_l2<true, false>;
@@ -213,7 +215,7 @@
                        aS, iterPtr, ncTr, nbCd, nbImp, srcOf, nbPc3, dt_long_first());
     return hipGetLastError();
   }
-  if (srcOf || !gmHere) return hipErrorInvalidValue;
+  if (srcOf || !gmHere || !l1Here) return hipErrorInvalidValue;
   MG_ALLOW_LDS(k_dt_front<true>);
   hipLaunchKernelGGL(k_dt_front<true>, dim3((unsigned)(nbPhi + nbDel + 2 * nbTr)), blk,
                      mg_colf_lds(d.Nr, ncPhi, nArrPhi), s, d, p, f, aT, aS, iterPtr, ncPhi, nbPhi, nbDel, nbTr);
@@ -229,4 +231,46 @@
   return launch_mom_tail(d, p, f, iterPtr, s);
 }
 
-}
+__global__ void __launch_bounds__(256) k_rstar_exch_phi(Dims d, Params p, Fields f, const long *__restrict__ srcOf, int nbR,
+                                                        XFields x, const long *__restrict__ map, int nHalo, int *ctr,
+                                                        int nbX, int nzMax, int nbXall, int fromX, int empNext, int nc,
+                                                        int nbPhi) {
+  int lb = mg_xcd_block();
+  if (lb < nbPhi) { phi_hyd_body<false, true>(d, p, f, nc, lb, nullptr, srcOf, fromX); return; }
+  lb -= nbPhi;
+  if (lb < nbR) { calc_r_star_body<true>(d, p, f, srcOf, lb, fromX, empNext); return; }
+  lb -= nbR;
+  if (lb < nbXall) { exchange_multi_body(d, x, map, nHalo, ctr, lb % nbX, (lb / nbX) % nzMax, lb / (nbX * nzMax)); return; }
+  del2uv_body<true>(d, p, f, lb - nbXall, srcOf);
+}
+
+bool phi_pipe_ok(const Dims &d, const Params &p) {
+  (void)d;
+  return mg_fuse_on(MG_FUSE_PHIP) && p.nonlinFreeSurf > 0 && p.select_rStar > 0 && p.exactConserv && !p.cubeCorners &&
+         dyn_thermo_takes_gm(p) && !phi_flat_on(p);
+}
+
+hipError_t launch_phi_del2(const Dims &d, const Params &p, const Fields &f, hipStream_t s) {
+  launch_l1(d, p, f, del2_needed(p) ? (int)mg_plane_blocks(d.nx, d.ny, d.nT * d.Nr) : 0, s, 0, false);
+  return hipGetLastError();
+}
+
+hipError_t launch_rstar_exch_phi(const Dims &d, const Params &p, const Fields &f, const long *srcOf, const XFields &x,
+                                 const long *map, int nHalo, int *ctr, hipStream_t s, int fromX, int empNext) {
+  if (!phi_pipe_ok(d, p) || !srcOf || d.nT != d.nTiles) return hipErrorInvalidValue;
+  const long n = d.n2 * d.nTiles;
+  const int nbR = (int)((n + 255) / 256);
+  int nzMax = 1;
+  for (int q = 0; q < x.n; q++) nzMax = x.nz[q] > nzMax ? x.nz[q] : nzMax;
+  const int nbX = ((nHalo > 0 ? nHalo : 1) + 255) / 256;
+  const int nbXall = nbX * nzMax * (x.n > 0 ? x.n : 1);
+  int nc, nArr, nbPhi;
+  phi_frame(d, p, nc, nArr, nbPhi);
+  const int nbDel = del2_needed(p) ? (int)mg_plane_blocks(d.nx, d.ny, d.nT * d.Nr) : 0;
+  MG_ALLOW_LDS(k_rstar_exch_phi);
+  hipLaunchKernelGGL(k_rstar_exch_phi, dim3((unsigned)(nbPhi + nbR + nbXall + nbDel)), dim3(256), mg_colf_lds(d.Nr, nc, nArr),
+                     s, d, p, f, srcOf, nbR, x, map, nHalo, ctr, nbX, nzMax, nbXall, fromX, empNext, nc, nbPhi);
+  return hipGetLastError();
+}
+
+}
diff --git a/mitgcm_amd/csrc/model.hip b/mitgcm_amd/csrc/model.hip
--- a/mitgcm_amd/csrc/model.hip
+++ b/mitgcm_amd/csrc/model.hip
@@ -71,7 +71,8 @@
 hipError_t launch_rstar_exch(const Dims &, const Params &, const Fields &, const long *, bool, const XFields &, const long *,
                              int, int *, hipStream_t, int fromX = 0, int empNext = 0);
 hipError_t launch_update_r_star_cg2d(const Dims &, const Params &, const Fields &, const long *, hipStream_t, bool sfp = false,
-                                     bool opEarly = false, bool pcHere = false, const int *iterPtr = nullptr);
+                                     bool opEarly = false, bool pcHere = false, const int *iterPtr = nullptr,
+                                     bool keepFac = false);
 hipError_t launch_halo_pack(const Dims &, const XFields &, const long *, long, double *, int, hipStream_t);
 hipError_t launch_oceanic_phys(const Dims &, const Params &, const Fields &, const int *, hipStream_t, bool gm = true,
                                bool *ringDone = nullptr);
@@ -79,7 +80,11 @@
                               bool impl = true);
 bool dyn_thermo_fusable(const Dims &, const Params &, const TracerArgs &, const TracerArgs &);
 hipError_t launch_dyn_thermo(const Dims &, const Params &, const Fields &, const TracerArgs &, const TracerArgs &, const int *,
-                             hipStream_t, const long *srcOf = nullptr, bool gmHere = true);
+                             hipStream_t, const long *srcOf = nullptr, bool gmHere = true, bool l1Here = true);
+bool phi_pipe_ok(const Dims &, const Params &);
+hipError_t launch_phi_del2(const Dims &, const Params &, const Fields &, hipStream_t);
+hipError_t launch_rstar_exch_phi(const Dims &, const Params &, const Fields &, const long *, const XFields &, const long *, int,
+                                 int *, hipStream_t, int fromX, int empNext);
 bool dyn_thermo_takes_gm(const Params &);
 hipError_t launch_gm_tensor(const Dims &, const Params &, const Fields &, hipStream_t);
 hipError_t launch_hfac_snapshot(const Dims &, const Fields &, double *, hipStream_t);
@@ -1197,8 +1202,9 @@
   return launch_exchange_uv_pairs(da, us, vs, 3, m->d_uvAll[0], m->nUvUAll[0], m->nUvVAll[0], m->stream);
 }
 static hipError_t update_r_star_cg2d(mgcm_model *m, bool sfp = false, bool opEarly = false, bool pcHere = false,
-                                     const int *physNext = nullptr) {
-  return launch_update_r_star_cg2d(all_tiles(m->d), m->p, m->f, m->d_srcOf, m->stream, sfp, opEarly, pcHere, physNext);
+                                     const int *physNext = nullptr, bool keepFac = false) {
+  return launch_update_r_star_cg2d(all_tiles(m->d), m->p, m->f, m->d_srcOf, m->stream, sfp, opEarly, pcHere, physNext,
+                                   keepFac);
 }
 
 int mgcm_init(mgcm_model *m) {
@@ -1477,7 +1483,7 @@
   return 0;
 }
 
-static XFields blocking_fields(const mgcm_model *m, int tracers = 1);
+static XFields blocking_fields(const mgcm_model *m, int tracers = 1, bool totPhi = true);
 
 int mgcm_blocking_exchanges(mgcm_model *m) {
   if (check_ready(m)) return -1;
@@ -1561,11 +1567,11 @@
   return field_count(m, fd->kind);
 }
 
-static XFields blocking_fields(const mgcm_model *m, int tracers) {
+static XFields blocking_fields(const mgcm_model *m, int tracers, bool totPhi) {
   XFields x{};
   double *fl[] = {m->f.uVel, m->f.vVel, m->f.wVel, m->f.theta, m->f.salt, m->f.uVelD, m->f.vVelD, m->f.totPhiHyd};
   const bool use[] = {!m->uvMap, !m->uvMap, true, m->p.tempStepping != 0, m->p.saltStepping != 0, m->p.useCDscheme != 0,
-                      m->p.useCDscheme != 0, m->p.storePhiHyd4Phys != 0};
+                      m->p.useCDscheme != 0, m->p.storePhiHyd4Phys != 0 && totPhi};
   for (int q = 0; q < 8; q++) {
     const bool tr = q == 3 || q == 4;
     if (use[q] && (tracers == 1 || (tracers == 2) == tr)) { x.p[x.n] = fl[q]; x.nz[x.n] = m->d.Nr; x.n++; }
@@ -1593,9 +1599,13 @@
   if (p.eosType == 1 && p.selectP_inEOS_Zc == 2 && !p.storePhiHyd4Phys) return false;
   return true;
 }
+static bool step_phi_pipelinable(mgcm_model *m) {
+  return step_pipelinable(m) && phi_pipe_ok(m->d, m->p);
+}
 static int one_step(mgcm_model *m, StepMode mode = STEP_PLAIN) {
   const bool pipe = mode != STEP_PLAIN, hoist = mode == STEP_HOIST;
   if (pipe && !step_pipelinable(m)) return set_err("one_step: the pipelined step does not apply to this model");
+  const bool phiPipe = pipe && step_phi_pipelinable(m);
   const bool stagger = m->p.staggerTimeStep != 0 && m->p.momStepping;
   const bool tracers = m->p.tempStepping || m->p.saltStepping;
   const bool fork = !stagger && m->overlap && !m->timing && m->p.momStepping && tracers;
@@ -1638,7 +1648,7 @@
   m->mwg.exclusive = thermoLate ? 1 : 0;
   const bool physPhi = !stagger && m->p.momStepping && phys_phi_fusable(m->d, m->p);
   m->stepLayout = (dtFused ? 1 : 0) | (physPhi ? 2 : 0) | (forkable && !dtFused ? 4 : 0) |
-                  ((forkable && m->p.nonlinFreeSurf <= 0) || tcg ? 8 : 0) | (pipe ? 16 : 0);
+                  ((forkable && m->p.nonlinFreeSurf <= 0) || tcg ? 8 : 0) | (pipe ? 16 : 0) | (phiPipe ? 32 : 0);
   const bool gmPhi = (stagger || thermoLate) && !dtFused && !physPhi && !m->timing && gm_phi_fusable(m->d, m->p);
   bool ringPhys = false;
   const bool ringPhysOk = !ringAside && !physPhi && mom_ring_separable(m->d, m->p) && mg_fuse_on(MG_FUSE_RINGP);
@@ -1663,7 +1673,7 @@
   if (m->p.momStepping) {
     if (dtFused) {
       TIMED(K_MOM, launch_dyn_thermo(m->d, m->p, m->f, aT, aS, m->d_ctr, m->stream, opEarly ? m->d_srcOf : nullptr,
-                                     !pipe));
+                                     !pipe, !phiPipe));
       std::swap(m->f.theta, m->f.thetaNext);
       std::swap(m->f.salt, m->f.saltNext);
     } else if (physPhi) TIMED(K_MOM, launch_mom_step(m->d, m->p, m->f, m->d_ctr, m->stream, !ringAside && !ringPhys));
@@ -1675,7 +1685,7 @@
     else if (fork && !lateJoin && !dtFused) HIPCHK(hipStreamWaitEvent(m->stream, m->evJoin, 0));
     const bool sfpFused = mg_fuse_on(MG_FUSE_SFP) && m->p.nonlinFreeSurf > 0 && m->d.nT == m->d.nTiles;
     if (m->p.nonlinFreeSurf > 0)
-      TIMED(K_RSTAR, update_r_star_cg2d(m, sfpFused, opEarly, false, hoist ? m->d_ctr : nullptr));
+      TIMED(K_RSTAR, update_r_star_cg2d(m, sfpFused, opEarly, false, hoist ? m->d_ctr : nullptr, hoist && phiPipe));
     if (!sfpFused) TIMED(K_RHS, launch_sfp_rhs(m->d, m->p, m->f, m->stream));
     if (thermoLate && fork_thermo()) return -1;
     const bool etaFused = mg_fuse_on(MG_FUSE_ETA) && cg2d_fuses_eta(m);
@@ -1700,7 +1710,11 @@
       TIMED(K_ETA, launch_exch_eta(m->d, m->p, m->f, m->d_srcOf, true, 0, m->stream, etaX ? 1 : 0));
     endFused = m->p.nonlinFreeSurf > 0 && !stagger && !m->uvMap && m->d.nT == m->d.nTiles &&
                mg_hfuse(MG_FUSE_END, m->d.nx, m->d.ny, m->d.nT, m->d.Nr);
-    if (endFused)
+    if (endFused && hoist && phiPipe) {
+      if (!fuseEtaH) return set_err("one_step: the hoisted CALC_PHI_HYD needs UPDATE_ETAH in CALC_R_STAR's pass");
+      TIMED(K_RSTAR, launch_rstar_exch_phi(m->d, m->p, m->f, m->d_srcOf, blocking_fields(m, 1, false), m->d_halo, m->nHalo,
+                                           m->d_ctr, m->stream, etaX ? 1 : 0, m->p.periodicExternalForcing ? 1 : 0));
+    } else if (endFused)
       TIMED(K_RSTAR, launch_rstar_exch(m->d, m->p, m->f, m->d_srcOf, fuseEtaH, blocking_fields(m), m->d_halo, m->nHalo,
                                        m->d_ctr, m->stream, etaX ? 1 : 0,
                                        hoist && m->p.periodicExternalForcing ? 1 : 0));
@@ -1885,6 +1899,8 @@
   if (m->useGraph && !m->timing && m->ovlAuto && !m->ovlDecided && nsteps >= 2 && ovl_trial(m)) return -1;
   const bool pipe = nsteps >= MG_PIPE_MIN_STEPS && step_pipelinable(m);
   if (pipe) TIMED(K_PHYS, launch_oceanic_phys(m->d, m->p, m->f, m->d_ctr, m->stream));
+  const bool phiPipe = pipe && step_phi_pipelinable(m);
+  if (phiPipe) TIMED(K_PHI, launch_phi_del2(m->d, m->p, m->f, m->stream));
   if (m->useGraph && !m->timing) {
     for (; s + 2 <= nsteps; s += 2) {
       hipGraphExec_t ge;
@@ -1902,7 +1918,7 @@
   }
   for (; s < nsteps; s++)
     if (one_step(m, pipe ? (s == nsteps - 1 ? STEP_LAST : STEP_HOIST) : STEP_PLAIN)) return -1;
-  m->stepLayout = (m->stepLayout & ~16) | (pipe ? 16 : 0);
+  m->stepLayout = (m->stepLayout & ~48) | (pipe ? 16 : 0) | (phiPipe ? 32 : 0);
   m->lastBatch = nsteps;
   return 0;
 }
diff --git a/mitgcm_amd/csrc/rstar.h b/mitgcm_amd/csrc/rstar.h
--- /dev/null
+++ b/mitgcm_amd/csrc/rstar.h
@@ -0,0 +1,136 @@
+#pragma once
+#include "common.h"
+
+namespace mgcm {
+
+__device__ __forceinline__ double eta_exch(const Dims &d, const Fields &f, const long *srcOf, long q, int fromX) {
+  const long sq = srcOf[q];
+  if (sq >= 0) return f.cg2d_b[sq];
+  const long l = q % d.n2;
+  const int i = (int)(l % d.nx) - d.OLx + 1, j = (int)(l / d.nx) - d.OLy + 1;
+  if (i >= 1 && i <= d.sNx && j >= 1 && j <= d.sNy) return f.cg2d_b[q];
+  return fromX ? f.recip_Bo[q] * f.cg2d_x[q] : f.etaN[q];
+}
+
+template <bool NARROW>
+__device__ __forceinline__ void mg_ij_of(const Dims &d, long q, int &i, int &j) {
+  if constexpr (NARROW) {
+    const int l = (int)q % (int)d.n2;
+    i = l % d.nx - d.OLx + 1;
+    j = l / d.nx - d.OLy + 1;
+  } else {
+    const long l = q % d.n2;
+    i = (int)(l % d.nx) - d.OLx + 1;
+    j = (int)(l / d.nx) - d.OLy + 1;
+  }
+}
+
+template <bool FUSE, bool WS = true, bool SHORT = false>
+__device__ __forceinline__ void calc_r_star_fac(const Dims &d, const Params &p, const Fields &f,
+                                                const long *__restrict__ srcOf, long q, int fromX, double oc, double ow,
+                                                double os, double &fc, double &fw, double &fs) {
+  auto inner = [&](int ii, int jj) { return ii >= 1 && ii <= d.sNx && jj >= 1 && jj <= d.sNy; };
+  int i, j;
+  long r;
+  if constexpr (SHORT) {
+    mg_ij_of<true>(d, q, i, j);
+    r = q;
+    if (!inner(i, j)) {
+      const long sq = srcOf[q];
+      if (sq >= 0) { r = sq; mg_ij_of<true>(d, r, i, j); }
+    }
+  } else {
+    const long sq = srcOf[q];
+    r = sq >= 0 ? sq : q;
+    mg_ij_of<false>(d, r, i, j);
+  }
+  auto eta = [&](long qq, int ii, int jj) {
+    if constexpr (SHORT) {
+      if (inner(ii, jj)) return f.cg2d_b[qq];
+      const long sqq = srcOf[qq];
+      if (sqq >= 0) return f.cg2d_b[sqq];
+      return fromX ? f.recip_Bo[qq] * f.cg2d_x[qq] : f.etaN[qq];
+    } else {
+      return FUSE ? eta_exch(d, f, srcOf, qq, fromX) : f.etaH[qq];
+    }
+  };
+  fc = oc;
+  fw = ow;
+  fs = os;
+  if (i >= 0 && i <= d.sNx + 1 && j >= 0 && j <= d.sNy + 1)
+    fc = (f.maskInC[r] != 0.0) ? (eta(r, i, j) + f.Ro_surf[r] - f.R_low[r]) * f.recip_Rcol[r] : 1.0;
+  if constexpr (WS) {
+    const long rv = (!SHORT && p.cubeCorners) ? q : r;
+    int iv = i, jv = j;
+    if constexpr (!SHORT) mg_ij_of<false>(d, rv, iv, jv);
+    if (iv >= 1 && iv <= d.sNx + 1 && jv >= 1 && jv <= d.sNy) {
+      if (f.maskInW[rv] != 0.0) {
+        const double tmp = f.rSurfW[rv] - f.rLowW[rv];
+        fw = (0.5 * (eta(rv - 1, iv - 1, jv) * f.rA[rv - 1] + eta(rv, iv, jv) * f.rA[rv]) * f.recip_rAw[rv] + tmp) / tmp;
+      } else {
+        fw = 1.0;
+      }
+    }
+    if (iv >= 1 && iv <= d.sNx && jv >= 1 && jv <= d.sNy + 1) {
+      if (f.maskInS[rv] != 0.0) {
+        const double tmp = f.rSurfS[rv] - f.rLowS[rv];
+        fs = (0.5 * (eta(rv - d.nx, iv, jv - 1) * f.rA[rv - d.nx] + eta(rv, iv, jv) * f.rA[rv]) * f.recip_rAs[rv] + tmp) / tmp;
+      } else {
+        fs = 1.0;
+      }
+    }
+  }
+}
+
+template <bool FUSE>
+__device__ __forceinline__ void calc_r_star_body(const Dims &d, const Params &p, const Fields &f,
+                                                 const long *__restrict__ srcOf, int lb, int fromX, int empNext = 0) {
+  const long q = (long)lb * blockDim.x + threadIdx.x;
+  if (q >= d.n2 * d.nTiles) return;
+  const int t = (int)(q / d.n2);
+  if (t < d.t0 || t >= d.t0 + d.nT) return;
+  if constexpr (FUSE) {
+    if (p.nonlinFreeSurf > 0 && p.useRealFreshWaterFlux) f.PmEpR[q] = -f.EmPmR[q];
+    if (empNext) f.EmPmR[q] = f.EmPmRnext[q];
+    const double x = eta_exch(d, f, srcOf, q, fromX);
+    f.etaHnm1[q] = f.etaH[q];
+    f.etaN[q] = x;
+    f.etaH[q] = x;
+  }
+  const double oc = f.rStarFacC[q], ow = f.rStarFacW[q], os = f.rStarFacS[q];
+  double fc, fw, fs;
+  calc_r_star_fac<FUSE>(d, p, f, srcOf, q, fromX, oc, ow, os, fc, fw, fs);
+  f.rStarFacC[q] = fc;
+  f.rStarFacW[q] = fw;
+  f.rStarFacS[q] = fs;
+  f.rStarDhCDt[q] = (fc - oc) / p.deltaTFreeSurf;
+  f.rStarDhWDt[q] = (fw - ow) / p.deltaTFreeSurf;
+  f.rStarDhSDt[q] = (fs - os) / p.deltaTFreeSurf;
+  f.rStarExpC[q] = fc / oc;
+  f.rStarExpW[q] = fw / ow;
+  f.rStarExpS[q] = fs / os;
+}
+
+template <bool WS>
+__device__ __forceinline__ void r_star_next_point(const Dims &d, const Params &p, const Fields &f,
+                                                  const long *__restrict__ srcOf, long q, int fromX, double &facC,
+                                                  double &dhC, double &dhW, double &dhS) {
+  const double oc = f.rStarFacCPrev[q], ow = WS ? f.rStarFacWPrev[q] : 0.0, os = WS ? f.rStarFacSPrev[q] : 0.0;
+  double fc, fw, fs;
+  calc_r_star_fac<true, WS, true>(d, p, f, srcOf, q, fromX, oc, ow, os, fc, fw, fs);
+  facC = fc;
+  dhC = (fc - oc) / p.deltaTFreeSurf;
+  if constexpr (WS) {
+    dhW = (fw - ow) / p.deltaTFreeSurf;
+    dhS = (fs - os) / p.deltaTFreeSurf;
+  }
+}
+
+__device__ __forceinline__ long mg_at_source3(const Dims &d, const long *__restrict__ srcOf, int i, int j, int k, int t) {
+  if (i >= 1 && i <= d.sNx && j >= 1 && j <= d.sNy) return MG_I3(d, i, j, k, t);
+  const long sq = srcOf[MG_I2(d, i, j, t)];
+  if (sq < 0) return MG_I3(d, i, j, k, t);
+  return (sq / d.n2) * d.n3 + (long)(k - 1) * d.n2 + sq % d.n2;
+}
+
+}
diff --git a/mitgcm_amd/model.py b/mitgcm_amd/model.py
--- a/mitgcm_amd/model.py
+++ b/mitgcm_amd/model.py
@@ -17,6 +17,7 @@
 STATE_3D = ("uVel", "vVel", "wVel", "theta", "salt", "gU", "gV", "guNm1", "gvNm1", "gtNm1", "gsNm1", "rhoInSitu",
             "IVDConvCount", "sigmaR", "Kwx", "Kwy", "Kwz", "Kux", "Kvy", "uVelD", "vVelD", "uNM1", "vNM1",
             "totPhiHyd", "alphaRho", "del2u", "del2v", "Kuz", "Kvz", "GM_PsiX", "GM_PsiY")
+WORK_3D = ("phiHydC", "dWtC", "dWtU", "dWtV")
 STATE_2D = ("etaN", "etaH", "fu", "fv", "SST", "lambdaThetaClimRelax", "surfaceForcingT", "surfaceForcingS",
             "Qnet", "EmPmR", "SSS", "lambdaSaltClimRelax", "etaNm1", "rStarFacC", "rStarFacW", "rStarFacS",
             "rStarExpC", "rStarExpW", "rStarExpS", "rStarDhCDt", "rStarDhWDt", "rStarDhSDt", "PmEpR", "dEtaHdt")
@@ -92,7 +93,7 @@
         g = self.g
         if name in GRID_1D or name in STATE_1D:
             return (g.Nr + 1,)
-        if name in GRID_3D or name in STATE_3D:
+        if name in GRID_3D or name in STATE_3D or name in WORK_3D:
             return (g.nTiles, g.Nr, g.ny, g.nx)
         if name == "forcRec":
             n = lib().mgcm_field_count(self.h, b"forcRec")
@@ -189,7 +190,7 @@
     def step_layout(self):
         b = int(lib().mgcm_get_param(self.h, b"stepLayout"))
         return {"dyn_thermo_fused": bool(b & 1), "phys_phi_fused": bool(b & 2), "thermo_second_stream": bool(b & 4),
-                "late_join": bool(b & 8), "pipelined": bool(b & 16)}
+                "late_join": bool(b & 8), "pipelined": bool(b & 16), "phi_pipelined": bool(b & 32)}
 
     def cg2d_fma(self):
         return lib().mgcm_get_param(self.h, b"cg2dFMA") != 0.0
```

New measurement: 3951 model-days/s, median of 6. 1.01x the previous value.
